# joyecnu/STTODE

Hardware: AMD Instinct MI355X
Metric: predicted-trajectories/sec (20-sample best-of-K) (higher is better)
Workload: dtype f32

## Files before the change

include/sttode_hip.h:

```cpp
#ifndef STTODE_HIP_H
#define STTODE_HIP_H
#ifdef __cplusplus
extern "C" {
#endif

#define STTODE_ABI_VERSION 14
int sttode_abi_version(void);
const char* sttode_last_error(void);

int sttode_rotate_scene(float* past, float* fut, int n, int Tp, int Tf, float c, float s, void* stream);

int sttode_frontend_scenes(const float* past, const int* scene_ptr, int n, int S, int Tp, int TPX, int vel_from_norm,
                           float* scene_orig, int* agent_scene, float* xpad, float* enc_in, float* cur, float* orig,
                           int* last_flag, void* stream);

int sttode_frontend_nba(const float* past, int n, int N, int Tp, int TPX, float* xpad, float* enc_in, float* cur, float* orig,
                        int* last_flag, void* stream);

int sttode_frontend_future(const float* future, const float* past_last, int n, int Tf, int mode, int nba_N,
                           const float* scene_orig, const int* agent_scene, const int* scene_ptr, float* enc_in, void* stream);

int sttode_embed_qkv(const float* fc1P, const float* fc1b, const float* posP, const float* peb, const float* fc2P,
                     const float* fc2b, const float* fc3P, const float* fc3b, const float* fc3last, const float* inP,
                     const float* inb, const float* enc_in, const int* last_flag, float* g, float* qkv, int n, int Tlen,
// ... 162 lines not shown
} SttodeOdeCombine;
int sttode_ode_combine(const void* jobs, int count, int width, void* stream);
typedef struct SttodeOdeProgram {
    int stages;
    int steps;
    float h;
    float a[16];
    float b[4];
} SttodeOdeProgram;
int sttode_ttrunk_ode_fwd(const void* const* ptrs, int count, int trunks, const int* n, const int* T, const long* ld_feat, float* const* ys,
                          float* const* yT, const void* prog, void* stream);
typedef struct SttodeOdeStageBwd {
    const float* w[16];
    const float* y;
    SttodeOdeCombine kb;
    float* dy;
    SttodeOdeCombine next;
    float* attn;
    float* ao;
    float* h;
    float* f1;
    float* dsum2;
    float* df1;
    float* du;
    float* dv;
    float* dao;
    float* dattn;
    float* ln;
    int n;
} SttodeOdeStageBwd;
int sttode_ode_stage_bwd(const void* jobs, int count, void* stream);

int sttode_loss_objective(const float* pred, const float* rec, const float* fut, const float* past, const float* qzp,
                          const int* scene_ptr, const int* agent_scene, int S, int n, int K1, int D, int Dp, int zd, float scale_mse,
                          float scale_rec, float kl_denom, float min_clip, float* out, float* dpred, float* drec, float* dqzp,
                          float* scratch, long scratch_floats, void* stream);
int sttode_loss_objective_live(const float* pred, const float* rec, const float* fut, const float* past, const float* qzp,
                               const int* scene_ptr, const int* agent_scene, int S, int n, int K1, int D, int Dp, int zd, float scale_mse,
                               float scale_rec, float kl_denom, float min_clip, float* out, float* dpred2, float* drec2, float* dqzp,
                               int* best, float* scratch, long scratch_floats, void* stream);
int sttode_live_rows_gather(const void* items, int count, const int* best, int n, int K1, void* stream);
int sttode_publish_values(const float* vals, int n, float* host_vals, unsigned* dev_seq, unsigned* host_seq, void* stream);
int sttode_wait_value(const unsigned* host_seq, long want, double timeout_s);

int sttode_pmath_rowop(int op, const float* x, const float* y, float* out, float* out2, int rows, int d, float c, void* stream);
int sttode_pmath_scalar(int which, const float* x, float* out, long n, void* stream);
int sttode_pmath_riemannian_grad(const float* x, const float* g, float* out, int rows, int d, float c, void* stream);
int sttode_pmath_matvec(const float* m, const float* x, float* mx_ws, float* xnorm_ws, float* out, int rows, int d, int O, float c,
                        void* stream);
int sttode_pmath_pair(int which, const float* x, const float* y, const float* A, float* out, int P, int R, int d, float c,
                      void* stream);
int sttode_pmath_mean(const float* x, float* yl_ws, float* lam_ws, float* out, int rows, int d, float c, void* stream);
int sttode_pmath_rowop_bwd(int op, const float* x, const float* y, const float* g, float* gx, float* gy, int rows, int d, float c, void* stream);
int sttode_pmath_matvec_bwd(const float* m, const float* x, const float* g, float* mx_ws, float* gmx_ws, float* gxn_ws, float* gx, float* gm,
                            int rows, int d, int O, float c, void* stream);
int sttode_pmath_dist_matrix_bwd(const float* x, const float* y, const float* g, float* gx, float* gy, int P, int R, int d, float c,
                                 void* stream);
int sttode_pmath_hsoftmax_bwd(const float* X, const float* A, const float* P, const float* g, double* coef_ws, float* gX, float* gA, float* gP,
                              int B, int C, int d, float c, void* stream);
int sttode_pmath_clip(const float* x, float* out, int rows, int d, float r, void* stream);
int sttode_pmath_clip_bwd(const float* x, const float* g, float* gx, int rows, int d, float r, void* stream);
int sttode_oblique_dist(const float* p1, const float* p2, float* out, int nb, int n1, int n2, int d, void* stream);

int sttode_delta_dist(const float* X, int rows, int d, const int* idx, int T, int n, float* dist, long dist_floats, float* diam, void* stream);
int sttode_delta_workspace(int T, int n, long* floats);
int sttode_delta_hyp(const float* dist, int T, int n, long dist_floats, int symmetric, float* ws, long ws_floats, float* delta, void* stream);

int sttode_reduce_samples(const float* pred, int n, int R, int K_in, int Tf, int K, int iters, int from_frame, int init_mode,
                          const float* init, float* centroids, int* labels, int* counts, void* stream);

typedef struct SttodeModel SttodeModel;

enum SttodeWeight {
    STT_W_FC1P, STT_W_FC1B, STT_W_POSP, STT_W_PEB, STT_W_FC2P, STT_W_FC2B, STT_W_FC3P, STT_W_FC3B, STT_W_FC3LAST, STT_W_INP,
    STT_W_INB, STT_W_OUTP, STT_W_OUTB, STT_W_INFOP, STT_W_INFOB, STT_W_GATEP, STT_W_GATEB, STT_W_LN1W, STT_W_LN1B, STT_W_L1P,
    STT_W_L1B, STT_W_L2P, STT_W_L2B, STT_W_LN2W, STT_W_LN2B,
    STT_W_B0_CONVP, STT_W_B0_CONVB, STT_W_B0_WIHP, STT_W_B0_WHHP, STT_W_B0_GBIAS, STT_W_B0_XWA, STT_W_B0_XB1, STT_W_B0_YWA,
    STT_W_B0_YB1, STT_W_B0_STREAM,
    STT_W_B1_CONVP, STT_W_B1_CONVB, STT_W_B1_WIHP, STT_W_B1_WHHP, STT_W_B1_GBIAS, STT_W_B1_YWA, STT_W_B1_YB1, STT_W_B1_STREAM,
    STT_W_CHAIN_POOL, STT_W_CHAIN_PROG, STT_W_CHAIN_CONSTS, STT_W_G0_POOL, STT_W_G0_PROG, STT_W_G0_CONSTS,
    STT_W_CHAINB3_POOL, STT_W_CHAINB3_PROG,
    STT_W_ROLE32_POOL, STT_W_ROLE32_PROG_SCENES, STT_W_ROLE32_PROG_NBA, STT_W_ROLE32_CONSTS_SCENES,
    STT_W_ROLE32_CONSTS_NBA,
    STT_W_COUNT
};

enum SttodeBuffer {
    STT_B_SCENE_ORIG, STT_B_AGENT_SCENE, STT_B_XPAD, STT_B_ENC_IN, STT_B_CUR, STT_B_ORIG, STT_B_LAST, STT_B_G, STT_B_QKV,
    STT_B_ATTN, STT_B_PF, STT_B_STATE0, STT_B_A0X, STT_B_A0Y, STT_B_A1Y, STT_B_DBUF, STT_B_YBUF, STT_B_STATE1, STT_B_QUEUE, STT_B_FLAGS ,
    STT_B_ODE , STT_B_COUNT
};

enum SttodeStage {
    STT_STAGE_FRONTEND, STT_STAGE_EMBED, STT_STAGE_ATTN, STT_STAGE_POST, STT_STAGE_GRU0, STT_STAGE_LINEAR, STT_STAGE_MLP0,
    STT_STAGE_GRU1, STT_STAGE_MLP1, STT_STAGE_CHAIN, STT_STAGE_AGENTS ,
    STT_STAGE_FUSED , STT_STAGE_COUNT
};

int sttode_model_create(SttodeModel** out, const void* const* weights, int count, int Tp, int Tf, int K, int n_chunks0,
                        int n_chunks1);
int sttode_model_set_weight(SttodeModel* m, int index, const void* ptr);
int sttode_model_destroy(SttodeModel* m);
int sttode_workspace_layout(const SttodeModel* m, int n, int S, long* offsets , long* total_floats);
int sttode_workspace_init(SttodeModel* m, float* workspace, int n, int S, void* stream);
int sttode_set_chain(SttodeModel* m, int mode);
int sttode_set_fused(SttodeModel* m, int mode);
int sttode_set_mfma_mode(SttodeModel* m, int mode);
int sttode_debug_drop_role_flag(SttodeModel* m, int tile);
int sttode_stage_scene(const float* pre, const float* fut, int N, int Tp, int Tf, float* dev, void* stream);
int sttode_stage_rows(const float* a, long na, const float* b, long nb, float* dev, void* stream);
int sttode_async_next_stream(SttodeModel* m, int n, void** stream);
int sttode_async_best_of_k(SttodeModel* m, int slot, const float* pred, const float* gt, int n, int K, int Tf, float scale, float* ade,
                           float* fde);
int sttode_set_scene_launch(SttodeModel* m, int max_tiles);
int sttode_fused_block_of(long block, long tiles, long groups, long K, long lead);
int sttode_set_ode(SttodeModel* m, int method, int steps);
int sttode_timing_enable(SttodeModel* m, int every);
int sttode_timing_read(SttodeModel* m, double* total_ms , int* launches ,
                       double* busy_ms );

int sttode_inference_scenes(SttodeModel* m, const float* past, const int* scene_ptr, int n, int S, const float* z,
                            float* workspace, float* pred, void* stream);
int sttode_inference_nba(SttodeModel* m, const float* past, int B, int N, const float* z, float* workspace, float* pred,
                         void* stream);
int sttode_inference_nba_groups(SttodeModel* m, const float* past, int G, int B, int N, const float* z, float* workspace, float* pred,
                                void* stream);

int sttode_set_lagged(SttodeModel* m, int streams );
typedef struct SttodeSamplerPlan {
    const float* pool;
    const int* prog;
    int prog_len;
    const float* biases;
    int K;
    int nz;
    int h1;
    int h2;
    int eps_mode;
    const float* eps;
} SttodeSamplerPlan;
typedef struct SttodeAsyncOpts {
    int device_latents;
    unsigned long long zkey;
    const float* metrics_gt;
    float* ade;
    float* fde;
    float metrics_scale;
    int nba_groups;
    const SttodeSamplerPlan* sampler;
} SttodeAsyncOpts;
int sttode_sampler_qnet(const SttodeSamplerPlan* plan, const float* pf, int n, float* z, void* stream);
int sttode_clock_probe(long long* out, void* stream);
int sttode_copy_to_host(void* dst, const void* src, long bytes, int wgs, void* stream);
int sttode_async_enqueue(SttodeModel* m, int slot);
int sttode_async_flush(SttodeModel* m);
int sttode_inference_scenes_async(SttodeModel* m, const float* past, const int* scene_ptr, int n, int S, const float* z,
                                  float* workspace, float* pred, int slot, const SttodeAsyncOpts* opts, void* stream);
int sttode_inference_nba_async(SttodeModel* m, const float* past, int B, int N, const float* z, float* workspace, float* pred,
                               int slot, const SttodeAsyncOpts* opts, void* stream);
int sttode_async_horizon_metrics(SttodeModel* m, int slot, const float* pred, const float* gt, int n, int K, int Tf, float scale, float* out);
int sttode_async_best_of_k_select(SttodeModel* m, int slot, const float* pred, const float* gt, int n, int K, int Tf, float scale,
                                  float miss_threshold, const int* seg_ptr, int S, float* ade, float* fde, int* best_ade_idx, int* best_fde_idx,
                                  unsigned char* miss, float* best, float* seg_ade, float* seg_fde, int* seg_miss);
int sttode_async_joint_select(SttodeModel* m, int slot, const float* pred, const float* gt, int n, int K, int Tf, float scale,
                              const int* seg_ptr, int S, float radius, float* seg_jade, float* seg_jfde, int* seg_jade_idx, int* seg_jfde_idx,
                              int* seg_col, int* seg_gt_col);
int sttode_async_kde_nll(SttodeModel* m, int slot, const float* pred, const float* gt, int n, int K, int Tf, float scale, double* nll);
int sttode_async_sample_spread(SttodeModel* m, int slot, const float* pred, const float* gt, int n, int K, int Tf, float scale,
                               double div_scale, double* apd, double* fpd, double* pade, double* dlow, double* es_ade, double* es_fde,
                               float* ade_at_k, float* fde_at_k);
int sttode_wait(SttodeModel* m, int slot, void* stream);
int sttode_async_is_lagged(SttodeModel* m, int n);
int sttode_wait_host(SttodeModel* m, int slot);
int sttode_timeout_word(SttodeModel* m, const unsigned** word);
int sttode_timeout_clear(SttodeModel* m);
int sttode_check(SttodeModel* m, const float* workspace, int n, int S, void* stream);

#ifdef __cplusplus
}
#endif
#endif
```

sttode_amd/capi.py:

```python
import ctypes
import os

_LIB = None
LIB_PATH = os.environ.get('STTODE_HIP_LIB') or os.path.join(os.path.dirname(os.path.abspath(__file__)), 'lib', 'libsttode_hip.so')

_P, _I, _L, _F, _D = ctypes.c_void_p, ctypes.c_int, ctypes.c_long, ctypes.c_float, ctypes.c_double
ABI_VERSION = 14

SIGNATURES = {
    'sttode_abi_version': [],
    'sttode_rotate_scene': [_P, _P, _I, _I, _I, _F, _F, _P],
    'sttode_frontend_scenes': [_P, _P, _I, _I, _I, _I, _I, _P, _P, _P, _P, _P, _P, _P, _P],
    'sttode_frontend_nba': [_P, _I, _I, _I, _I, _P, _P, _P, _P, _P, _P],
    'sttode_frontend_future': [_P, _P, _I, _I, _I, _I, _P, _P, _P, _P, _P],
    'sttode_embed_qkv': [_P] * 11 + [_P, _P, _P, _P, _I, _I, _P],
    'sttode_mhgsa_attn': [_P, _P, _P, _P, _P, _P, _I, _I, _I] + [_L] * 8 + [_F, _F, _P],
    'sttode_mhgsa_attn_groups': [_P, _P, _P, _P, _I, _L, _L, _L, _L, _I, _I, _I] + [_L] * 8 + [_F, _F, _I, _P],
    'sttode_post_attn': [_P] * 14 + [_P, _P, _I, _P, _I, _F, _P],
    'sttode_post_attn_ode': [_P] * 16 + [_P, _P, _I, _F, _I, _I, _P],
    'sttode_post_attn_rhs': [_P] * 14 + [_P, _P, _I, _P, _I, _P],
    'sttode_ode_state_to_pf': [_P, _P, _P, _I, _P],
    'sttode_gru_cols': [_P, _P, _P, _P, _P, _P, _P, _I, _I, _I, _P],
    'sttode_set_latency_tiles': [_I, _I, _I],
    'sttode_linear_cols': [_P, _I, _I, _P, _I, _I, _P, _P, _P, _I, _I, _I, _I, _P],
    'sttode_agent_preact': [_P] * 11 + [_I, _P],
    'sttode_mlp_block0': [_P, _P, _P, _I, _P, _P, _P, _P, _I, _I, _I, _I, _P],
    'sttode_mlp_block1': [_P, _P, _I, _P, _P, _P, _P, _P, _P, _I, _I, _I, _I, _P],
    'sttode_mlp_cols': [_P, _P, _I, _P, _P, _P, _I, _I, _I, _P],
    'sttode_traj_chain': [_P, _P, _P, _P, _P, _I, _P, _P, _P, _I, _P, _P, _P, _P, _I, _I, _I, _I, _I, _P],
    'sttode_chain_prog_len': [_I, _I],
    'sttode_gru_cols32': [_P, _I, _P, _P, _I, _P, _P, _I, _I, _P],
    'sttode_best_of_k': [_P, _P, _I, _I, _I, _F, _P, _P, _P],
    'sttode_horizon_metrics': [_P, _P, _I, _I, _I, _F, _P, _P],
    'sttode_best_of_k_select': [_P, _P, _I, _I, _I, _F, _F, _P, _I] + [_P] * 10,
    'sttode_joint_select': [_P, _P, _I, _I, _I, _F, _P, _I, _F] + [_P] * 7,
    'sttode_kde_nll': [_P, _P, _I, _I, _I, _F, _P, _P],
    'sttode_sample_spread': [_P, _P, _I, _I, _I, _F, _D] + [_P] * 9,
    'sttode_sampler_latent': [_P, _P, _P, _I, _P, _P, _I, _I, _I, _P],
    'sttode_sampler_loss': [_P, _P, _P, _P, _P, _I, _I, _I, _I, _F, _P, _P, _P],
    'sttode_sampler_loss_bwd': [_P, _P, _P, _P, _P, _P, _P, _I, _I, _I, _I, _F, _P, _P, _P, _P],
    'sttode_sampler_qnet': [_P, _P, _I, _P, _P],
    'sttode_tlinear': [_P, _L, _I, _P, _L, _I, _P, _P, _L, _P, _L, _I, _I, _I, _I, _I, _P],
    'sttode_tlinear_tab': [_P, _L, _P, _L, _P, _P, _L, _I, _P, _L, _I, _I, _I, _I, _P],
    'sttode_twgrad': [_P, _L, _P, _L, _I, _P, _L, _P, _I, _I, _I, _P, _L, _P],
    'sttode_twgrad_defer': [_I, _P, _L],
    'sttode_twgrad_flush': [],
    'sttode_tgemm_group': [_I],
    'sttode_tlinear_bwd': [_P, _L, _P, _L, _P, _L, _P, _L, _I, _I, _P, _L, _I, _P, _L, _P, _I, _I, _I, _P, _L, _P],
    'sttode_decoder_inputs': [_P, _P, _L, _P, _L, _P, _P, _I, _I, _I, _I, _P],
    'sttode_rows_copy': [_P, _L, _P, _L, _I, _I, _I, _I, _P],
    'sttode_rows_reduce': [_P, _L, _P, _L, _I, _I, _I, _I, _P],
    'sttode_train_ewise': [_I, _P, _P, _P, _P, _P, _L, _I, _F, _P],
    'sttode_add_ln_fwd': [_P, _P, _P, _P, _P, _P, _P, _I, _I, _P],
    'sttode_ln_bwd': [_P, _P, _P, _P, _P, _P, _P, _I, _I, _P, _L, _P],
    'sttode_gru_cell_fwd': [_P, _L, _P, _P, _P, _P, _I, _P],
    'sttode_gru_cell_bwd': [_P, _P, _P, _P, _L, _P, _P, _I, _P],
    'sttode_gru_seq_fwd': [_P, _P, _P, _P, _P, _P, _L, _I, _I, _P],
    'sttode_gru_seq_bwd': [_P, _L, _P, _P, _P, _P, _P, _I, _I, _P],
    'sttode_conv_fwd': [_P, _I, _P, _P, _P, _P, _P, _I, _I, _P],
    'sttode_conv_bwd': [_P, _P, _P, _P, _P, _P, _I, _I, _P, _L, _P],
    'sttode_mhgsa_attn_bwd': [_P, _P, _P, _I, _I, _I, _P],
    'sttode_mhgsa_attn_rc_bwd': [_P] * 7 + [_I, _I, _I] + [_L] * 8 + [_F, _F, _P],
    'sttode_adam_step': [_P, _I, _L, _P, _D, _D, _D, _D, _D, _L, _P],
    'sttode_grad_norm': [_P, _I, _P, _L, _D, _I, _P, _P],
    'sttode_adam_step_guarded': [_P, _I, _L, _P, _D, _D, _D, _D, _P, _I, _P],
    'sttode_grad_scale': [_P, _I, _L, _P, _P, _P],
    'sttode_loss_sqerr': [_P, _P, _L, _F, _P, _P, _P],
    'sttode_loss_kl': [_P, _P, _I, _I, _I, _F, _F, _P, _P, _P, _P],
    'sttode_loss_diverse': [_P, _P, _P, _P, _I, _I, _I, _P, _P, _P, _P],
    'sttode_ttrunk_fwd': [_P, _I, _I, _I, _L, _F, _I, _P],
    'sttode_ode_combine': [_P, _I, _I, _P],
    'sttode_ttrunk_ode_fwd': [_P, _I, _I, _P, _P, _P, _P, _P, _P, _P],
    'sttode_ode_stage_bwd': [_P, _I, _P],
    'sttode_loss_objective': [_P, _P, _P, _P, _P, _P, _P, _I, _I, _I, _I, _I, _I, _F, _F, _F, _F, _P, _P, _P, _P, _P, _L, _P],
    'sttode_pmath_rowop': [_I, _P, _P, _P, _P, _I, _I, _F, _P],
    'sttode_pmath_scalar': [_I, _P, _P, _L, _P],
    'sttode_pmath_riemannian_grad': [_P, _P, _P, _I, _I, _F, _P],
    'sttode_pmath_matvec': [_P, _P, _P, _P, _P, _I, _I, _I, _F, _P],
    'sttode_pmath_pair': [_I, _P, _P, _P, _P, _I, _I, _I, _F, _P],
    'sttode_pmath_mean': [_P, _P, _P, _P, _I, _I, _F, _P],
    'sttode_oblique_dist': [_P, _P, _P, _I, _I, _I, _I, _P],
    'sttode_pmath_rowop_bwd': [_I, _P, _P, _P, _P, _P, _I, _I, _F, _P],
    'sttode_pmath_matvec_bwd': [_P, _P, _P, _P, _P, _P, _P, _P, _I, _I, _I, _F, _P],
    'sttode_pmath_dist_matrix_bwd': [_P, _P, _P, _P, _P, _I, _I, _I, _F, _P],
    'sttode_pmath_hsoftmax_bwd': [_P, _P, _P, _P, _P, _P, _P, _P, _I, _I, _I, _F, _P],
    'sttode_pmath_clip': [_P, _P, _I, _I, _F, _P],
    'sttode_pmath_clip_bwd': [_P, _P, _P, _I, _I, _F, _P],
    'sttode_delta_dist': [_P, _I, _I, _P, _I, _I, _P, _L, _P, _P],
    'sttode_delta_workspace': [_I, _I, ctypes.POINTER(ctypes.c_long)],
    'sttode_delta_hyp': [_P, _I, _I, _L, _I, _P, _L, _P, _P],
    'sttode_reduce_samples': [_P, _I, _I, _I, _I, _I, _I, _I, _I, _P, _P, _P, _P, _P],
    'sttode_attn_core': [_P, _P, _P, _P, _L, _P, _P, _P, _P, _I, _I, _I] + [_L] * 8 + [_F, _F, _I, _P],
    'sttode_attn_core_bwd': [_P, _P, _P, _P, _L, _P, _P, _P, _P, _I, _I, _I] + [_L] * 8 + [_F, _F, _I, _P],
    'sttode_model_create': [ctypes.POINTER(ctypes.c_void_p), ctypes.POINTER(ctypes.c_void_p), _I, _I, _I, _I, _I, _I],
    'sttode_model_destroy': [_P],
    'sttode_model_set_weight': [_P, _I, _P],
    'sttode_workspace_layout': [_P, _I, _I, ctypes.POINTER(ctypes.c_long), ctypes.POINTER(ctypes.c_long)],
    'sttode_workspace_init': [_P, _P, _I, _I, _P],
    'sttode_timeout_word': [_P, ctypes.POINTER(ctypes.c_void_p)],
    'sttode_timeout_clear': [_P],
    'sttode_set_chain': [_P, _I],
    'sttode_set_fused': [_P, _I],
    'sttode_set_mfma_mode': [_P, _I],
    'sttode_debug_drop_role_flag': [_P, _I],
    'sttode_set_scene_launch': [_P, _I],
    'sttode_stage_scene': [_P, _P, _I, _I, _I, _P, _P],
    'sttode_stage_rows': [_P, _L, _P, _L, _P, _P],
    'sttode_loss_objective_live': [_P, _P, _P, _P, _P, _P, _P, _I, _I, _I, _I, _I, _I, _F, _F, _F, _F, _P, _P, _P, _P, _P, _P, _L, _P],
    'sttode_live_rows_gather': [_P, _I, _P, _I, _I, _P],
    'sttode_publish_values': [_P, _I, _P, _P, _P, _P],
    'sttode_wait_value': [_P, _L, _D],
    'sttode_async_next_stream': [_P, _I, _P],
    'sttode_async_best_of_k': [_P, _I, _P, _P, _I, _I, _I, _F, _P, _P],
    'sttode_fused_block_of': [_L, _L, _L, _L, _L],
    'sttode_set_ode': [_P, _I, _I],
    'sttode_timing_enable': [_P, _I],
    'sttode_timing_read': [_P, ctypes.POINTER(ctypes.c_double), ctypes.POINTER(ctypes.c_int), ctypes.POINTER(ctypes.c_double)],
    'sttode_inference_scenes': [_P, _P, _P, _I, _I, _P, _P, _P, _P],
    'sttode_inference_nba': [_P, _P, _I, _I, _P, _P, _P, _P],
    'sttode_inference_nba_groups': [_P, _P, _I, _I, _I, _P, _P, _P, _P],
    'sttode_inference_scenes_async': [_P, _P, _P, _I, _I, _P, _P, _P, _I, _P, _P],
    'sttode_inference_nba_async': [_P, _P, _I, _I, _P, _P, _P, _I, _P, _P],
    'sttode_async_horizon_metrics': [_P, _I, _P, _P, _I, _I, _I, _F, _P],
    'sttode_async_best_of_k_select': [_P, _I, _P, _P, _I, _I, _I, _F, _F, _P, _I] + [_P] * 9,
    'sttode_async_joint_select': [_P, _I, _P, _P, _I, _I, _I, _F, _P, _I, _F] + [_P] * 6,
    'sttode_async_kde_nll': [_P, _I, _P, _P, _I, _I, _I, _F, _P],
    'sttode_async_sample_spread': [_P, _I, _P, _P, _I, _I, _I, _F, _D] + [_P] * 8,
    'sttode_wait': [_P, _I, _P],
    'sttode_async_is_lagged': [_P, _I],
    'sttode_wait_host': [_P, _I],
    'sttode_set_lagged': [_P, _I],
    'sttode_async_flush': [_P],
    'sttode_clock_probe': [_P, _P],
    'sttode_copy_to_host': [_P, _P, _L, _I, _P],
    'sttode_async_enqueue': [_P, _I],
    'sttode_check': [_P, _P, _I, _I, _P],
}

WEIGHT_ORDER = ([('past', k) for k in ('fc1P', 'fc1b', 'posP', 'peb', 'fc2P', 'fc2b', 'fc3P', 'fc3b', 'fc3last', 'inP', 'inb', 'outP',
                                       'outb', 'infoP', 'infob', 'gateP', 'gateb', 'ln1w', 'ln1b', 'l1P', 'l1b', 'l2P', 'l2b', 'ln2w',
                                       'ln2b')]
                + [('blk0', k) for k in ('convP', 'convB', 'wihP', 'whhP', 'gbias', 'x_WA', 'x_b1', 'y_WA', 'y_b1', 'stream')]
                + [('blk1', k) for k in ('convP', 'convB', 'wihP', 'whhP', 'gbias', 'y_WA', 'y_b1', 'stream')]
                + [('chain', k) for k in ('pool', 'prog', 'consts')] + [('gru0s', k) for k in ('pool', 'prog', 'consts')]
                + [('chain_b3', k) for k in ('pool', 'prog')]
                + [('role32', k) for k in ('pool', 'prog_scenes', 'prog_nba', 'consts_scenes', 'consts_nba')])
TRUNK_PTRS = ('fc1_w', 'fc1_b', 'pos_w', 'pos_b', 'fc2_w', 'fc2_b', 'fc3_w', 'fc3_b', 'inproj_w', 'inproj_b', 'out_w', 'out_b', 'info_w', 'info_b',
              'gate_w', 'gate_b', 'ln1_w', 'ln1_b', 'l1_w', 'l1_b', 'l2_w', 'l2_b', 'ln2_w', 'ln2_b', 'enc_in', 'last', 'pe', 'drop', 'posin', 'tp',
              'h3in', 'feat', 'xc', 'qkv', 'ao', 'tt', 'ss', 'h', 'xh1', 'rs1', 'f1', 'xh2', 'rs2', 'ode', 'attn')
BUFFERS = ('scene_orig', 'agent_scene', 'xpad', 'enc_in', 'cur', 'orig', 'last', 'g', 'qkv', 'attn', 'pf', 'state0', 'A0x', 'A0y',
           'A1y', 'dbuf', 'ybuf', 'state1', 'queue', 'flags', 'ode')
STAGES = ('frontend', 'embed_qkv', 'mhgsa_attn', 'post_attn', 'gru_cols[block0,agents]', 'agent_preact', 'mlp_block0',
          'gru_cols[block1,trajectories]', 'mlp_block1', 'trajectory_chain', 'agents_fused[encoder+block0 GRU]', 'agents+trajectory_chain[fused launch]')


class AsyncOpts(ctypes.Structure):
    _fields_ = [('device_latents', ctypes.c_int), ('zkey', ctypes.c_ulonglong), ('metrics_gt', ctypes.c_void_p), ('ade', ctypes.c_void_p),
                ('fde', ctypes.c_void_p), ('metrics_scale', ctypes.c_float), ('nba_groups', ctypes.c_int), ('sampler', ctypes.c_void_p)]


class GradGroup(ctypes.Structure):
    _fields_ = [('items', ctypes.c_void_p), ('n', ctypes.c_int), ('chunks', ctypes.c_long), ('gbase', ctypes.c_void_p),
                ('lr', ctypes.c_double), ('beta1', ctypes.c_double), ('beta2', ctypes.c_double), ('step', ctypes.c_long)]


GRAD_MAX_GROUPS = 16
GRAD_STATE_WORDS = 40


class SamplerPlan(ctypes.Structure):
    _fields_ = [('pool', ctypes.c_void_p), ('prog', ctypes.c_void_p), ('prog_len', ctypes.c_int), ('biases', ctypes.c_void_p),
                ('K', ctypes.c_int), ('nz', ctypes.c_int), ('h1', ctypes.c_int), ('h2', ctypes.c_int), ('eps_mode', ctypes.c_int),
                ('eps', ctypes.c_void_p)]


class NativeModel:

    def __init__(self, packed, Tp, Tf, K):
        self.packed = packed
        tbl = (ctypes.c_void_p * len(WEIGHT_ORDER))(*[(packed[g][k].data_ptr() if g in packed else None) for g, k in WEIGHT_ORDER])
        h = ctypes.c_void_p()
        rc = lib().sttode_model_create(ctypes.byref(h), tbl, len(WEIGHT_ORDER), Tp, Tf, K, int(packed['blk0']['n_chunks']),
                                       int(packed['blk1']['n_chunks']))
        if rc != 0:
            raise SttodeError('sttode_model_create failed: ' + lib().sttode_last_error().decode())
        self.h = h
        self._layouts = {}
        w = ctypes.c_void_p()
        if lib().sttode_timeout_word(h, ctypes.byref(w)) != 0 or not w.value:
            raise SttodeError('sttode_timeout_word failed: ' + lib().sttode_last_error().decode())
        self.timeout_word = ctypes.c_uint.from_address(w.value)

    def raise_if_timed_out(self):
        v = self.timeout_word.value
        if v:
            lib().sttode_timeout_clear(self.h)
            raise SttodeError('a trajectory group of an earlier launch gave up waiting for its per-agent role (time-out word %d): the '
                              'predictions of that call are NaN-poisoned, not valid' % v if v != 2 else
                              'an earlier launch ran on a workspace that was never initialised (sttode_workspace_init): its predictions are NaN')

    def init_workspace(self, buf, n, S):
        call('sttode_workspace_init', self.h, buf, int(n), int(S), stream_ptr())

    def layout(self, n, S):
        key = (n, S)
        if key not in self._layouts:
            off = (ctypes.c_long * len(BUFFERS))()
            tot = ctypes.c_long()
            rc = lib().sttode_workspace_layout(self.h, n, S, off, ctypes.byref(tot))
            if rc != 0:
                raise SttodeError('sttode_workspace_layout failed: ' + lib().sttode_last_error().decode())
            self._layouts[key] = (dict(zip(BUFFERS, list(off))), int(tot.value))
        return self._layouts[key]

    def set_chain(self, mode):
        if lib().sttode_set_chain(self.h, int(mode)) != 0:
            raise SttodeError('sttode_set_chain failed: ' + lib().sttode_last_error().decode())

    def set_scene_launch(self, max_tiles):
        call('sttode_set_scene_launch', self.h, int(max_tiles))

    def set_fused(self, mode):
        if lib().sttode_set_fused(self.h, int(mode)) != 0:
            raise SttodeError('sttode_set_fused failed: ' + lib().sttode_last_error().decode())

    def set_lagged(self, streams):
        call('sttode_set_lagged', self.h, int(streams))
        self._lagged = int(streams)

    def check(self, workspace, n, S):
        call('sttode_check', self.h, workspace, int(n), int(S), stream_ptr())

    def set_weights(self, group, tensors):
        self.packed[group] = tensors
        for i, (g, k) in enumerate(WEIGHT_ORDER):
            if g == group:
                call('sttode_model_set_weight', self.h, i, tensors[k])

    def set_mfma_mode(self, mode):
        if lib().sttode_set_mfma_mode(self.h, int(mode)) != 0:
            raise SttodeError('sttode_set_mfma_mode failed: ' + lib().sttode_last_error().decode())

    def set_ode(self, method, steps):
        if lib().sttode_set_ode(self.h, int(method), int(steps)) != 0:
            raise SttodeError('sttode_set_ode failed: ' + lib().sttode_last_error().decode())

    def timing(self, every):
        lib().sttode_timing_enable(self.h, int(every))

    def read_timing(self):
        ms = (ctypes.c_double * len(STAGES))()
        cnt = (ctypes.c_int * len(STAGES))()
        busy = (ctypes.c_double * len(STAGES))()
        rc = lib().sttode_timing_read(self.h, ms, cnt, busy)
        if rc != 0:
            raise SttodeError('sttode_timing_read failed: ' + lib().sttode_last_error().decode())
        self.busy_ms = {STAGES[i]: busy[i] for i in range(len(STAGES)) if cnt[i]}
        return {STAGES[i]: (ms[i], cnt[i]) for i in range(len(STAGES)) if cnt[i]}

    def __del__(self):
        try:
            if self.h:
                lib().sttode_model_destroy(self.h)
                self.h = None
        except Exception:
            pass



class SttodeError(RuntimeError):
    pass


def lib():
    global _LIB
    if _LIB is None:
        if not os.path.exists(LIB_PATH):
            raise SttodeError(f'{LIB_PATH} not found: build it with `python -c "import __graft_entry__ as g; g.build()"` '
                              f'or `make -C sttode_amd/csrc`. There is no CPU fallback.')
        L = ctypes.CDLL(LIB_PATH)
        L.sttode_last_error.restype = ctypes.c_char_p
        L.sttode_last_error.argtypes = []
        try:
            got = int(L.sttode_abi_version())
        except AttributeError:
            got = None
        if got != ABI_VERSION:
            raise SttodeError(f'{LIB_PATH}: ABI version {got}, this binding needs {ABI_VERSION}; rebuild with `make -C sttode_amd/csrc`')
# ... 40 lines not shown
```

sttode_amd/csrc/api_util.hpp:

```cpp
#pragma once
#include <hip/hip_runtime.h>
#include <cstdio>

void stt_set_error(const char* msg);
int stt_gru_cols_form(const float* xin, const float* convP, const float* convB, const float* wihP, const float* whhP, const float* gbias,
                      float* state, int ncols, int Tp, int TPX, int lat_max_tiles, void* stream);
int stt_agents_fused(const float* const* W, const float* enc_in, const int* last, float* g, float* qkv, float* pf, const float* xpad,
                     float* state0, int n, int Tp, int TPX, float ode_time, void* stream);
bool stt_agents_fused_covers(int Tp, int TPX);
int stt_chain_fused(const float* const* W, float* ws, const long* off, int n, int K, int Tp, int Tf, int prog_len, const float* z, float* pred,
                    float ode_time, const float* attn, int ld_attn, const float* past, const int* scene_ptr, int S, int wgs_per_cu, int b3, int lead, int drop_tile,
                    unsigned* tmo_host, void* stream);
bool stt_chain_fused_covers(int Tp);
int stt_scene_lat(const float* const* W, float* ws, const long* off, int n, int K, int Tp, int Tf, int TPX, int NOY, int n_chunks0, int n_chunks1,
                  const float* z, float* pred, float ode_time, const float* past, const int* scene_ptr, int S, int drop_tile, unsigned* tmo_host,
                  void* stream);
static inline int stt_scene_flags_offset(int n) { return 5 * ((n + 15) / 16) + 4; }
int stt_scene_flags_init(float* ws, const long* off, int n, int K, void* stream);
bool stt_scene_lat_covers(int Tp, int TPX, int NOY);
int stt_traj_chain_b3(const float* A0x, const float* A0y, const float* A1y, const float* pool, const int* prog, int prog_len,
                      const float* consts, const float* z, const float* xpad, int ldx, const float* cur, const float* orig,
                      float* pred, int* counter, int ncols, int K, int Tp, int Tf, int wgs_per_cu, void* stream);
int stt_gru_lat_tiles();
int stt_enc_lat_tiles();

#define STT_REQUIRE(cond, msg)      \
    do {                            \
        if (!(cond)) {              \
            stt_set_error(msg);     \
            return 1;               \
        }                           \
    } while (0)

#define STT_HIP(expr)                                                                       \
    do {                                                                                    \
        hipError_t _e = (expr);                                                             \
        if (_e != hipSuccess) {                                                             \
            char _b[512];                                                                   \
            snprintf(_b, sizeof(_b), "%s failed: %s (%s:%d)", #expr, hipGetErrorString(_e), __FILE__, __LINE__); \
            stt_set_error(_b);                                                              \
            return 2;                                                                       \
        }                                                                                   \
    } while (0)

#define STT_ATTR_DEVICES 64
#define STT_SET_LDS_ONCE(kernel, bytes)                                                                         \
    do {                                                                                                        \
        static bool _done[STT_ATTR_DEVICES] = {};                                                               \
        int _dev = 0;                                                                                           \
        STT_HIP(hipGetDevice(&_dev));                                                                           \
        if (_dev < 0 || _dev >= STT_ATTR_DEVICES || !_done[_dev]) {                                             \
            STT_HIP(hipFuncSetAttribute((const void*)(kernel), hipFuncAttributeMaxDynamicSharedMemorySize, (bytes))); \
            if (_dev >= 0 && _dev < STT_ATTR_DEVICES) _done[_dev] = true;                                       \
        }                                                                                                       \
    } while (0)

struct LagRoles {
    float* ws; const long* off; int n;
    const float* attn; int ld_attn; float ode_time;
    float* zgen; unsigned long long zkey;
    const float* past; const int* scene_ptr; int S;
    float* ade; float* fde;
};
struct LagGroups {
    float* ws; const long* off; int n; const float* z; float* pred;
    const float* gt; float* ade; float* fde; float scale;
    int workers;
};
int stt_chain_lagged(const float* const* W, const LagRoles& r, const LagGroups& g, int K, int Tp, int Tf, int prog_len, int b3, void* stream);
bool stt_chain_lagged_covers(int Tp);
struct SttodeSamplerPlan;
const char* stt_sampler_plan_check(const SttodeSamplerPlan* plan, int K);
int stt_sampler_qnet(const SttodeSamplerPlan* plan, const float* pf, int n, float* z, void* stream);
int stt_joint_check(const char* who, const float* pred, const float* gt, int n, int K, int Tf, const int* seg_ptr, int S, float radius,
                    const float* seg_jade, const float* seg_jfde, const int* seg_jade_idx, const int* seg_jfde_idx, const int* seg_col,
                    const int* seg_gt_col);
int stt_kde_check(const char* who, const float* pred, const float* gt, int n, int K, int Tf, const double* nll);
int stt_spread_check(const char* who, const float* pred, const float* gt, int n, int K, int Tf, double div_scale, const double* apd,
                     const double* fpd, const double* pade, const double* dlow, const double* es_ade, const double* es_fde,
                     const float* ade_at_k, const float* fde_at_k);
```

sttode_amd/csrc/chain32.hip:

```cpp
#include "chain.hpp"
#include "latency_bodies.hpp"
#include "frontend_body.hpp"
#include "api_util.hpp"
#include "../../include/sttode_hip.h"
#include <cstdlib>
#include <cstddef>

#ifdef C32_DIAG_TRACE
__shared__ long long g_tr_ph[4];
#define C32_TRACE_BEGIN() long long _tr_t0 = 0, _tr_c0 = 0; if (threadIdx.x == 0 && A.dbg) { _tr_t0 = __builtin_amdgcn_s_memrealtime(); _tr_c0 = __builtin_amdgcn_s_memtime(); }
#define C32_TRACE_END(kind) do { if (threadIdx.x == 0 && A.dbg) { \
        const long long _t1 = __builtin_amdgcn_s_memrealtime(); unsigned _hw, _xcc; \
        asm volatile("s_getreg_b32 %0, hwreg(HW_REG_HW_ID)" : "=s"(_hw)); asm volatile("s_getreg_b32 %0, hwreg(HW_REG_XCC_ID)" : "=s"(_xcc)); \
        const unsigned long long _r = atomicAdd((unsigned long long*)A.dbg, 1ull); if ((long long)_r >= A.dbg[1]) break;  \
        long long* _p = A.dbg + 8 + _r * 12; _p[0] = A.trace_tag; _p[1] = blockIdx.x; _p[2] = (kind); _p[3] = _tr_t0; _p[4] = _t1; _p[5] = _hw; _p[6] = _xcc; \
        _p[8] = g_tr_ph[0]; _p[9] = g_tr_ph[1]; _p[10] = g_tr_ph[2]; _p[7] = __builtin_amdgcn_s_memtime() - _tr_c0; _p[11] = g_tr_ph[3]; } } while (0)
#define C32_TRACE_PHASE(i) do { if (threadIdx.x == 0) g_tr_ph[i] = __builtin_amdgcn_s_memrealtime(); } while (0)
#else
#define C32_TRACE_PHASE(i) do { } while (0)
#define C32_TRACE_BEGIN() do { } while (0)
#define C32_TRACE_END(kind) do { } while (0)
#endif

#include "role_body.hpp"

typedef float f32x16 __attribute__((ext_vector_type(16)));

#ifdef C32_DIAG_NOGATES
#define C32_SIG(x) ((x) * 1e-3f)
#define C32_TANH(x) ((x) * 1e-3f)
#else
#define C32_SIG(x) sigmoid_prescaled(x)
#define C32_TANH(x) tanh_prescaled(x)
#endif

#define C32_TILE 256
#define C32_CMAX 3
#define C32_RING (2 * C32_CMAX * C32_TILE)
#define C32_SLOT 256

struct Role32Args {
    const f32x4* pool; const int2* prog; int prog_len; const float* consts;
    const float* enc_in; const int* last;
    const float* g_in; const float* attn; int ld_attn;
    const float* xpad; int ldx;
    float* pf; float* state0; float* A0x; float* A0y; float* A1y;
    int n, Tp, kte, nwg;
    float ode_time;
    int prio;
    int* counter;
    float* zgen; unsigned zkey0, zkey1; int K;
    const float* past; const int* scene_ptr; int S; float* scene_orig; int* agent_scene;
    float* enc_in_w; float* xpad_w; float* cur_w; float* orig_w; int* last_w;
    float* m_ade; float* m_fde;
};

struct ChainArgs {
    const float* A0x; const float* A0y; const float* A1y;
    const f32x4* pool;
    const int2* prog; int prog_len;
    const float* consts;
    const float* z;
    const float* xpad; int ldx;
    const float* cur; const float* orig;
    float* pred;
    float* park;
    int* counter;
    int ncols, K, Tp, Tf2;
    int persistent;
    const float* m_gt; float* m_ade; float* m_fde; float m_scale;
    int nworkers;
    long long* dbg;
    int trace_tag;
    int xcd_map;
    RoleArgs R;
    Role32Args R32;
};

template <int NY> struct C32Const {
    static constexpr int b2x = 0, b3x = 256, b2y = 288, b3y = 544, gb = 544 + 32 * NY, cb = gb + 384, b2m = cb + 32,
                         b3m = b2m + 256, total = b3m + 32 * NY;
};

__device__ __forceinline__ f32x16 splat16(float v) {
    f32x16 r;
#pragma unroll
    for (int e = 0; e < 16; ++e) r[e] = v;
    return r;
}
__device__ __forceinline__ f32x16 relu16(f32x16 v) {
#pragma unroll
    for (int e = 0; e < 16; ++e) v[e] = fmaxf(v[e], 0.f);
    return v;
}
__device__ __forceinline__ f32x16 ldrows(const float* p, int h) {
    f32x16 r;
#pragma unroll
    for (int a = 0; a < 4; ++a) {
        const f32x4 v = ld4(p + 8 * a + 4 * h);
        r[4 * a + 0] = v[0]; r[4 * a + 1] = v[1]; r[4 * a + 2] = v[2]; r[4 * a + 3] = v[3];
    }
    return r;
}

typedef const __attribute__((address_space(4))) int KProg;

template <int BUF, bool GEN, bool DYN = false>
struct ChainStreamT {
    static constexpr int kBuf = BUF;
    static constexpr int kPieces = (BUF / 64 + 3) / 4, kPairs = (kPieces + 1) / 2;
    const char* pool; KProg* prog; f32x4* ring;
    unsigned ring_addr, loff;
    unsigned qoff, qend;
    int par, lane, wave;
    int2 ld_v, ld_w;
    bool fetched;
    int cnt;
    const char* nsrc[kPairs]; unsigned nm0[kPairs]; int ncnt, npc;
#ifdef C32_DIAG_STAMPS
    long long t_bar, gap_cyc, gap_n, gap_cal;
#endif
    __device__ __forceinline__ int2 entry_at(unsigned off) const {
        const KProg* e = reinterpret_cast<const KProg*>(reinterpret_cast<const __attribute__((address_space(4))) char*>(prog) + off);
        return make_int2(e[0], e[1]);
    }
    __device__ __forceinline__ unsigned next_off(unsigned off) const { return off + 8 >= qend ? 0u : off + 8; }
    __device__ __forceinline__ void stage(int2 ev, int buf) {
        ncnt = __builtin_amdgcn_readfirstlane(ev.y);
        npc = GEN ? (ncnt - wave + 3) >> 2 : ncnt;
        const size_t src = (size_t)(unsigned)__builtin_amdgcn_readfirstlane(ev.x) * (GEN ? 16u : C32_TILE * 16u) + (unsigned)wave * 1024u;
        const unsigned dst = __builtin_amdgcn_readfirstlane(ring_addr + (unsigned)buf * (BUF * 16) + (unsigned)wave * 1024u);
#pragma unroll
        for (int k = 0; k < kPairs; ++k) {
            nsrc[k] = pool + (src + 4096u * (2 * k + 1));
            nm0[k] = dst + 4096u * (2 * k + 1);
            asm volatile("" : "+s"(nsrc[k]), "+s"(nm0[k]));
        }
        asm volatile("" : "+s"(npc));
    }
    __device__ __forceinline__ void issue(int N) {
#ifndef C32_DIAG_NODMA
#pragma unroll
        for (int k = 0; k < kPairs; ++k) {
            if (N > 0 ? 2 * k < N : 2 * k < npc) {
                glds16_sv<-4096>(nsrc[k], loff, nm0[k] - 4096u);
                if (2 * k + 1 < kPieces && (N > 0 ? 2 * k + 1 < N : 2 * k + 1 < npc)) glds16_m0<0>(nsrc[k], loff);
            }
        }
#endif
    }
    __device__ __forceinline__ void init(const f32x4* pool_, const int2* prog_, int len_, f32x4* ring_) {
        pool = reinterpret_cast<const char*>(pool_); prog = (KProg*)prog_; ring = ring_;
        ring_addr = __builtin_amdgcn_readfirstlane(lds_addr(ring_));
        lane = threadIdx.x & 63;
        loff = (unsigned)lane * 16;
        wave = __builtin_amdgcn_readfirstlane(threadIdx.x >> 6);
        par = 0;
        qend = (unsigned)len_ * 8u;
        const int2 e0 = entry_at(0);
        stage(e0, 0);
        issue(0);
        cnt = e0.y;
        qoff = next_off(0);
        stage(entry_at(qoff), 1);
        qoff = next_off(qoff);
        fetched = false;
#ifdef C32_DIAG_STAMPS
        gap_cyc = 0; gap_n = 0;
        const long long c0 = __builtin_amdgcn_s_memtime();
        asm volatile("s_waitcnt lgkmcnt(0)" ::: "memory");
        gap_cal = __builtin_amdgcn_s_memtime() - c0;
        t_bar = 0;
#endif
    }
    __device__ __forceinline__ void fetch() { ld_v = entry_at(qoff); qoff = next_off(qoff); fetched = true; }
    __device__ __forceinline__ void fetch_more() { ld_w = entry_at(qoff); qoff = next_off(qoff); }
    __device__ __forceinline__ void take_prefetched() { ld_v = ld_w; fetched = true; }
    __device__ __forceinline__ void stamp_gap() {
#ifdef C32_DIAG_STAMPS
        asm volatile("s_waitcnt lgkmcnt(0)" ::: "memory");
        const long long c1 = __builtin_amdgcn_s_memtime();
        asm volatile("s_waitcnt lgkmcnt(0)" ::: "memory");
        if (t_bar) { gap_cyc += c1 - t_bar; ++gap_n; }
#endif
    }
    __device__ __forceinline__ void begin(int N = 0) {
        __builtin_amdgcn_sched_barrier(0);
#ifdef C32_DIAG_CHECK
        if (!GEN && N > 0 && ncnt != N) __builtin_trap();
#endif
        cnt = ncnt;
        issue(GEN || DYN ? 0 : N);
        stamp_gap();
        __builtin_amdgcn_sched_barrier(0);
    }
    __device__ __forceinline__ const f32x4* cur() const { return ring + par * BUF + lane; }
    __device__ __forceinline__ void end(bool has_entry = false) {
        __builtin_amdgcn_sched_barrier(0);
#ifdef C32_DIAG_CHECK
        if (has_entry && !fetched) __builtin_trap();
#endif
        if (!has_entry && !fetched) fetch();
        stage(ld_v, par);
        __builtin_amdgcn_sched_barrier(0);
#ifndef C32_DIAG_NOBARRIER
        asm volatile("s_waitcnt vmcnt(0)" ::: "memory");
        __syncthreads();
#endif
#ifdef C32_DIAG_STAMPS
        t_bar = __builtin_amdgcn_s_memtime();
        asm volatile("s_waitcnt lgkmcnt(0)" ::: "memory");
#endif
        par ^= 1;
        fetched = false;
        __builtin_amdgcn_sched_barrier(0);
    }
};
typedef ChainStreamT<C32_CMAX * C32_TILE, false> ChainStream;

__device__ __forceinline__ void tile_mma(f32x16& acc, const f32x4* __restrict__ t, const f32x16& B) {
#pragma unroll
    for (int g = 0; g < 4; ++g) {
        const f32x4 a = t[g * 64];
#pragma unroll
        for (int r = 0; r < 4; ++r) acc = __builtin_amdgcn_mfma_f32_32x32x2f32(a[r], B[4 * g + r], acc, 0, 0, 0);
    }
}

__device__ __forceinline__ void gather_rows(const void* base, unsigned voff, unsigned slot_addr) {
// ... 366 lines not shown
    f32x16 e = ldrows(cb, h);
    Frag fa, fb;
    if (ZS) {
        const int k0 = 2 * t - 2, k1 = 2 * t + 3;
        const int g0 = (k0 > 0 ? k0 : 0) >> 3, g1 = (k1 < 2 * Tp - 1 ? k1 : 2 * Tp - 1) >> 3;
        const f32x4* tc = st.cur();
#pragma unroll
        for (int g = 0; g < 4; ++g)
            if (g >= g0 && g <= g1) fa.a[g] = tc[g * 64];
        st.begin(3);
#pragma unroll
        for (int g = 0; g < 4; ++g)
            if (g >= g0 && g <= g1)
#pragma unroll
                for (int r = 0; r < 4; ++r) e = __builtin_amdgcn_mfma_f32_32x32x2f32(fa.a[g][r], d[4 * g + r], e, 0, 0, 0);
        __builtin_amdgcn_sched_barrier(0);
        if (pre) st.take_prefetched();
        else st.fetch();
    } else {
        ldfrag(fa, st.cur());
        st.begin(3);
        tile_mma2f(st, e, fa, d, fb, nullptr, pre ? 0 : 1);
        if (pre) st.take_prefetched();
    }
    e = relu16(e);
    st.end();
    return e;
}

template <bool ZS, class ST>
__device__ __forceinline__ void gru32_steps(ST& st, const float* gb, const float* cb, const f32x16& d, f32x16 (&hs)[3], int Tp, int h) {
    if (ZS) {
        const f32x16 e = gru32_conv<ZS>(st, cb, d, 0, Tp, h, false);
        Frag fa, fb;
#pragma unroll
        for (int j = 0; j < 3; ++j) {
            STT_FENCE();
            f32x16 ar = ldrows(gb + 0 * 96 + 32 * j, h);
            ldfrag(fa, st.cur()); st.begin(3);
            tile_mma2f(st, ar, fa, e, fb, nullptr);
            st.end(); ldfrag(fa, st.cur() + 1 * C32_TILE); st.begin(3);
#pragma unroll
            for (int r = 0; r < 16; ++r) ar[r] = C32_SIG(ar[r]);
            STT_FENCE();
            f32x16 az = ldrows(gb + 1 * 96 + 32 * j, h);
            tile_mma2f(st, az, fa, e, fb, nullptr, 2);
            st.end(); st.begin(3);
            st.take_prefetched();
#pragma unroll
            for (int r = 0; r < 16; ++r) az[r] = C32_SIG(az[r]);
            STT_FENCE();
            f32x16 an = ldrows(gb + 3 * 96 + 32 * j, h);
            {
                const f32x16 bi = ldrows(gb + 2 * 96 + 32 * j, h);
#pragma unroll
                for (int r = 0; r < 16; ++r) an[r] = fmaf(ar[r], an[r], bi[r]);
            }
            st.end(); ldfrag(fa, st.cur() + 2 * C32_TILE);
            if (j < 2) st.begin(3); else st.begin();
            STT_FENCE();
            tile_mma2f(st, an, fa, e, fb, nullptr, (j == 2 && 1 < Tp) ? 2 : 1);
            st.end();
#pragma unroll
            for (int r = 0; r < 16; ++r) {
                const float ng = C32_TANH(an[r]);
                hs[j][r] = fmaf(az[r], 0.f - ng, ng);
            }
        }
    }
#pragma unroll 1
    for (int t = ZS ? 1 : 0; t < Tp; ++t) {
        const f32x16 e = gru32_conv<ZS>(st, cb, d, t, Tp, h, ZS);
        Frag fa, fb;
        f32x16 hn[3];
#pragma unroll
        for (int j = 0; j < 3; ++j) {
            STT_FENCE();
            f32x16 ar = ldrows(gb + 0 * 96 + 32 * j, h);
            ldfrag(fa, st.cur()); st.begin(3);
            tile_mma2f(st, ar, fa, e, fb, st.cur() + 1 * C32_TILE);
            tile_mma2(ar, fb, hs[0], fa, st.cur() + 2 * C32_TILE);
            tile_mma2(ar, fa, hs[1], fb, nullptr);
            st.end(); ldfrag(fa, st.cur()); st.begin(3);
            tile_mma2f(st, ar, fa, hs[2], fb, st.cur() + 1 * C32_TILE);
#pragma unroll
            for (int r = 0; r < 16; ++r) ar[r] = C32_SIG(ar[r]);
            STT_FENCE();
            f32x16 az = ldrows(gb + 1 * 96 + 32 * j, h);
            tile_mma2(az, fb, e, fa, st.cur() + 2 * C32_TILE);
            tile_mma2(az, fa, hs[0], fb, nullptr);
            st.end(); ldfrag(fa, st.cur()); st.begin(3);
            tile_mma2f(st, az, fa, hs[1], fb, st.cur() + 1 * C32_TILE);
            tile_mma2(az, fb, hs[2], fa, st.cur() + 2 * C32_TILE);
#pragma unroll
            for (int r = 0; r < 16; ++r) az[r] = C32_SIG(az[r]);
            STT_FENCE();
            f32x16 an = ldrows(gb + 3 * 96 + 32 * j, h);
            tile_mma2(an, fa, hs[0], fb, nullptr);
            st.end(); ldfrag(fa, st.cur());
            if (j < 2) st.begin(3); else st.begin();
            tile_mma2f(st, an, fa, hs[1], fb, st.cur() + 1 * C32_TILE, (ZS && j == 2 && t + 1 < Tp) ? 2 : 1);
            tile_mma2(an, fb, hs[2], fa, st.cur() + 2 * C32_TILE);
            {
                const f32x16 bi = ldrows(gb + 2 * 96 + 32 * j, h);
#pragma unroll
                for (int r = 0; r < 16; ++r) an[r] = fmaf(ar[r], an[r], bi[r]);
            }
            STT_FENCE();
            tile_mma2(an, fa, e, fb, nullptr);
            st.end();
#pragma unroll
            for (int r = 0; r < 16; ++r) {
                const float ng = C32_TANH(an[r]);
                hn[j][r] = fmaf(az[r], hs[j][r] - ng, ng);
            }
        }
#pragma unroll
        for (int j = 0; j < 3; ++j) hs[j] = hn[j];
    }

}

#include "role32.hpp"

__device__ __forceinline__ int opaque(int v) { asm volatile("" : "+v"(v)); return v; }

#ifdef C32_DIAG_STAMPS
#define C32_STAMP(k) do { if (threadIdx.x == 0 && A.dbg && gi < 4) { A.dbg[((size_t)blockIdx.x * 4 + gi) * 16 + 2 * (k)] = __builtin_amdgcn_s_memtime(); \
                                                                    A.dbg[((size_t)blockIdx.x * 4 + gi) * 16 + 2 * (k) + 1] = __builtin_amdgcn_s_memrealtime(); } } while (0)
#else
#define C32_STAMP(k) do { } while (0)
#endif

__host__ __device__ __forceinline__ int fused_block_of(long b, long T, long G, long K, long lead) {
    auto roles_upto = [&](long x) { const long c = (8 * (x + lead + 1) + K - 1) / K; return c < T ? c : T; };
    long lo = -1, hi = G - 1;
    while (lo < hi) {
        const long mid = (lo + hi + 1) >> 1;
        if (mid + roles_upto(mid) <= b) lo = mid; else hi = mid - 1;
    }
    if (lo >= 0 && lo + roles_upto(lo) == b) return (int)lo;
    return -1 - (int)(b - (lo + 1));
}

__host__ __device__ __forceinline__ int xcd_group(int b, int G) {
    const int x = b & 7, i = b >> 3, q = G >> 3, r = G & 7;
    return x * q + (x < r ? x : r) + i;
}

template <int NY, int FUSE, bool B3M, bool ZS>
__global__ __launch_bounds__(256, 2) void traj_chain_kernel(ChainArgs A) {
    constexpr bool kDynCount = !B3M && ((NY == 1 && FUSE == 2 && !ZS) || (NY == 2 && FUSE == 1 && ZS));
    typedef ChainStreamT<B3M ? C32_BUF_B3 : C32_CMAX * C32_TILE, B3M, kDynCount> Stream;
    extern __shared__ __attribute__((aligned(16))) char smem[];
    f32x4* ring = reinterpret_cast<f32x4*>(smem);
    f32x4* slots = ring + 2 * Stream::kBuf;
    f32x4* zslots = slots + 4 * C32_SLOT;
    float* cst = reinterpret_cast<float*>(zslots + 4 * C32_SLOT);
    int* sq = reinterpret_cast<int*>(cst + C32Const<NY>::total);
    typedef C32Const<NY> CO;

    const int lane = threadIdx.x & 63, c = lane & 31, h = lane >> 5;
    const int wave = __builtin_amdgcn_readfirstlane(threadIdx.x >> 6);
    const f32x4* slot = slots + wave * C32_SLOT;
    const f32x4* zslot = zslots + wave * C32_SLOT;
    const unsigned slot_addr = __builtin_amdgcn_readfirstlane(lds_addr(slot));
    const unsigned zslot_addr = __builtin_amdgcn_readfirstlane(lds_addr(zslot));
    const int ngroups = (A.ncols + 127) >> 7;

    C32_TRACE_BEGIN();
    if (FUSE == 2 && (int)blockIdx.x < A.R32.nwg) {
        role32_body<ZS>(*(KRole32Args*)((const __attribute__((address_space(4))) char*)__builtin_amdgcn_kernarg_segment_ptr() + offsetof(ChainArgs, R32)),
                    blockIdx.x, smem);
        C32_TRACE_END(1);
        return;
    }
    if (FUSE == 1 && A.R.split && (int)blockIdx.x < 5 * A.R.ntiles) {
        split_role(A.R, (A.ncols + A.K - 1) / A.K, A.Tp, A.ldx, A.xpad, blockIdx.x, smem);
        C32_TRACE_END(1);
        return;
    }
    int fb = FUSE == 0 ? (int)blockIdx.x : FUSE == 2 ? (int)blockIdx.x - A.R32.nwg : A.R.split ? (int)blockIdx.x - 5 * A.R.ntiles
                                                : fused_block_of(blockIdx.x, A.R.ntiles, ngroups, A.K, A.R.lead);
    if (FUSE && A.xcd_map && fb >= 0) fb = xcd_group(fb, ngroups);
    if (FUSE == 1 && fb < 0) {
        agent_role(A.R, (A.ncols + A.K - 1) / A.K, A.Tp, A.ldx, A.xpad, -1 - fb, smem);
        C32_TRACE_END(1);
        return;
    }
    for (int i = threadIdx.x; i < CO::total; i += blockDim.x) cst[i] = A.consts[i];
    if (threadIdx.x == 0) sq[0] = FUSE == 2 ? fb : (FUSE == 0 && A.persistent) ? atomicAdd(A.counter, 1) : FUSE ? fb : (int)blockIdx.x;
    if (FUSE == 1) {
        const int g0 = fb;
        const int c_lo = g0 * 128, c_hi = (c_lo + 127 < A.ncols ? c_lo + 127 : A.ncols - 1);
        const int t_lo = (c_lo / A.K) >> 4, t_hi = (c_hi / A.K) >> 4;
        if (wave == 0) {
            const bool ok = A.R.split ? wait_tiles(A.R.pflags, 3 * t_lo, 3 * t_hi + 2, A.R.flags + A.R.ntiles, lane, A.R.tmo_host)
                                      : wait_tiles(A.R.flags, t_lo, t_hi, A.R.flags + A.R.ntiles, lane, A.R.tmo_host);
            if (!ok && lane == 0) sq[0] = -1;
        }
    }
    __syncthreads();
    C32_TRACE_PHASE(3);
    int g = sq[0];
    if (FUSE == 1 && g < 0) {
        for (int i = threadIdx.x; i < 128 * A.Tf2; i += blockDim.x) {
            const size_t o = (size_t)fb * 128 * A.Tf2 + i;
            if (o < (size_t)A.ncols * A.Tf2) A.pred[o] = __builtin_nanf("");
        }
        return;
    }
    if (g >= ngroups) return;
    Stream st;
    st.init(A.pool, A.prog, A.prog_len, ring);

    auto col_of = [&](int gg) { int col = gg * 128 + wave * 32 + c; return col < A.ncols ? col : A.ncols - 1; };
    {
        const int c0 = col_of(g);
        gather_rows(A.A0x, row_off(c0 / A.K, 512, h), slot_addr);
        gather_rows(A.z, row_off(c0, 32, h), zslot_addr);
    }
    asm volatile("s_waitcnt vmcnt(0)" ::: "memory");
    __syncthreads();

    int gi = 0;
    (void)gi;
    while (true) {
        C32_STAMP(0);
        const int col = g * 128 + wave * 32 + c;
        int colc = col < A.ncols ? col : A.ncols - 1;
        int agent = colc / A.K;
        const bool live = col < A.ncols;
        __syncthreads();
        if (threadIdx.x == 0)
            sq[1] = (FUSE == 2 && A.persistent && ngroups > A.nworkers) ? A.nworkers + atomicAdd(A.counter, 1)
                    : (FUSE == 0 && A.persistent) ? atomicAdd(A.counter, 1) : ngroups;

        f32x16 acc2[8];
        f32x16 d;
        {
            agent = opaque(agent);
            f32x16 xo[1];
            const unsigned ao = row_off(agent, 512, h);
            if (B3M) {
                mlp_l12_b3<0, true>(st, slot, zslot, nullptr, A.A0x, ao, A.A0y, ao, acc2, lane);
                mlp_l3_b3<1>(st, acc2, cst + CO::b2x, cst + CO::b3x, xo, h);
            } else {
                mlp_l12<0>(st, slot, zslot, nullptr, A.A0x, ao, A.A0y, ao, acc2, lane);
                mlp_l3<1, 3>(st, acc2, cst + CO::b2x, cst + CO::b3x, xo, h);
            }
            agent = opaque(agent);
            const float* xp = A.xpad + (size_t)agent * A.ldx;
#pragma unroll
            for (int a = 0; a < 4; ++a) {
                f32x4 v = splat4(0.f);
                if (8 * a + 4 * h < A.ldx) v = ld4(xp + 8 * a + 4 * h);
#pragma unroll
                for (int b = 0; b < 4; ++b) d[4 * a + b] = v[b] - xo[0][4 * a + b];
            }
        }
        STT_FENCE();
        C32_STAMP(1);
        {
            agent = opaque(agent);
            f32x16 yo[NY];
            const unsigned ao = row_off(agent, 512, h);
            if (B3M) {
                mlp_l12_b3<0, true>(st, slot, zslot, nullptr, A.A0y, ao, A.A1y, ao, acc2, lane);
                mlp_l3_b3<NY>(st, acc2, cst + CO::b2y, cst + CO::b3y, yo, h);
            } else {
                mlp_l12<0>(st, slot, zslot, nullptr, A.A0y, ao, A.A1y, ao, acc2, lane);
                mlp_l3<NY, 1>(st, acc2, cst + CO::b2y, cst + CO::b3y, yo, h);
            }
            if (live) {
                float* prow = A.park + (size_t)opaque(col) * A.Tf2;
#pragma unroll
                for (int o = 0; o < NY; ++o)
#pragma unroll
                    for (int a = 0; a < 4; ++a) {
                        const int row0 = 32 * o + 8 * a + 4 * h;
                        float* p = prow + row0;
                        if (row0 + 3 < A.Tf2 && (A.Tf2 & 3) == 0) {
                            f32x4 v = {yo[o][4 * a], yo[o][4 * a + 1], yo[o][4 * a + 2], yo[o][4 * a + 3]};
                            st4(p, v);
                        } else {
#pragma unroll
                            for (int b = 0; b < 4; ++b)
                                if (row0 + b < A.Tf2) p[b] = yo[o][4 * a + b];
                        }
                    }
            }
        }
        STT_FENCE();
        C32_STAMP(2);
        f32x16 hs[3];
        {
#pragma unroll
            for (int j = 0; j < 3; ++j) hs[j] = splat16(0.f);
            if (B3M) gru32_steps_b3(st, cst + CO::gb, cst + CO::cb, d, hs, A.Tp, h);
            else gru32_steps<ZS>(st, cst + CO::gb, cst + CO::cb, d, hs, A.Tp, h);
        }
        STT_FENCE();
        C32_STAMP(3);
        const int gnext = sq[1];
        {
            agent = opaque(agent);
            const int cnx = col_of(gnext < ngroups ? gnext : g);
            const unsigned ao = row_off(agent, 512, h), an = row_off(cnx / A.K, 512, h);
            if (B3M) mlp_l12_b3<3, false>(st, slot, zslot, hs, A.A1y, ao, A.A0x, an, acc2, lane);
            else mlp_l12<3>(st, slot, zslot, hs, A.A1y, ao, A.A0x, an, acc2, lane);
            gather_rows(A.z, row_off(opaque(cnx), 32, h), zslot_addr);
            f32x16 yo[NY];
            if (B3M) mlp_l3_b3<NY>(st, acc2, cst + CO::b2m, cst + CO::b3m, yo, h);
            else mlp_l3<NY, 3>(st, acc2, cst + CO::b2m, cst + CO::b3m, yo, h);
            {
                agent = opaque(agent);
                const float cx = A.cur[2 * agent], cy = A.cur[2 * agent + 1];
                const float ox = A.orig[2 * agent], oy = A.orig[2 * agent + 1];
                const bool vec = (A.Tf2 & 3) == 0;
                const float* yrow = A.park + (size_t)opaque(colc) * A.Tf2;
                float* prow = A.pred + (size_t)opaque(col) * A.Tf2;
                const float* grow = FUSE == 2 && A.m_gt ? A.m_gt + (size_t)agent * A.Tf2 : nullptr;
                float dd[NY][4][2];
#pragma unroll
                for (int o = 0; o < NY; ++o)
#pragma unroll
                    for (int a = 0; a < 4; ++a) {
                        const int row0 = 32 * o + 8 * a + 4 * h;
                        const bool whole = vec && row0 + 3 < A.Tf2;
                        f32x4 y0 = splat4(0.f);
                        if (whole) y0 = ld4(yrow + row0);
                        else {
#pragma unroll
                            for (int b = 0; b < 4; ++b)
                                if (row0 + b < A.Tf2) y0[b] = yrow[row0 + b];
                        }
                        f32x4 v;
                        v[0] = ((y0[0] + yo[o][4 * a + 0]) + cx) + ox;
                        v[1] = ((y0[1] + yo[o][4 * a + 1]) + cy) + oy;
                        v[2] = ((y0[2] + yo[o][4 * a + 2]) + cx) + ox;
                        v[3] = ((y0[3] + yo[o][4 * a + 3]) + cy) + oy;
                        if (live) {
                            if (whole) st4(prow + row0, v);
                            else {
#pragma unroll
                                for (int b = 0; b < 4; ++b)
                                    if (row0 + b < A.Tf2) prow[row0 + b] = v[b];
                            }
                        }
                        dd[o][a][0] = dd[o][a][1] = 0.f;
                        if (FUSE == 2 && grow) {
                            if (row0 < A.Tf2) { const float2 g = *reinterpret_cast<const float2*>(grow + row0); dd[o][a][0] = bok_dist(v[0], v[1], g.x, g.y, A.m_scale); }
                            if (row0 + 2 < A.Tf2) { const float2 g = *reinterpret_cast<const float2*>(grow + row0 + 2); dd[o][a][1] = bok_dist(v[2], v[3], g.x, g.y, A.m_scale); }
                        }
                    }
                if (FUSE == 2 && grow) {
                    const int Tf = A.Tf2 >> 1;
                    float acc = 0.f, fdl = -1.f;
#pragma unroll
                    for (int o = 0; o < NY; ++o)
#pragma unroll
                        for (int a = 0; a < 4; ++a) {
                            const int t0 = (32 * o + 8 * a + 4 * h) >> 1;
                            float mine = acc;
                            if (h == 0) { if (t0 < Tf) mine += dd[o][a][0]; if (t0 + 1 < Tf) mine += dd[o][a][1]; }
                            float mine1 = __shfl(mine, c, 64);
                            if (h == 1) { if (t0 < Tf) mine1 += dd[o][a][0]; if (t0 + 1 < Tf) mine1 += dd[o][a][1]; }
                            acc = __shfl(mine1, c + 32, 64);
                            if (t0 == Tf - 1) fdl = dd[o][a][0];
                            if (t0 + 1 == Tf - 1) fdl = dd[o][a][1];
                        }
                    fdl = fmaxf(fdl, __shfl_xor(fdl, 32, 64));
                    const float adev = acc / (float)Tf;
                    if (live && h == 0) {
                        atomicMin(reinterpret_cast<unsigned*>(A.m_ade) + agent, __float_as_uint(adev));
                        atomicMin(reinterpret_cast<unsigned*>(A.m_fde) + agent, __float_as_uint(fdl));
                    }
                }
            }
        }
        C32_STAMP(4);
#ifdef C32_DIAG_STAMPS
        if (threadIdx.x == 0 && A.dbg && gi < 4) {
            long long* o = A.dbg + ((size_t)blockIdx.x * 4 + gi) * 16 + 10;
            o[0] = st.gap_cyc; o[1] = st.gap_n; o[2] = st.gap_cal;
        }
        st.gap_cyc = 0; st.gap_n = 0;
#endif
        ++gi;
        g = gnext;
        if (g >= ngroups) break;
    }
    C32_TRACE_END(0);
}

struct Gru32Args {
    const float* xin; int ldx;
    const f32x4* pool; const int2* prog; int prog_len;
    const float* consts;
    float* state;
    int ncols, Tp;
};
template <bool ZS>
__global__ __launch_bounds__(256, 2) void gru32_kernel(Gru32Args A) {
    extern __shared__ __attribute__((aligned(16))) char smem[];
    f32x4* ring = reinterpret_cast<f32x4*>(smem);
    float* cst = reinterpret_cast<float*>(ring + C32_RING);
    const int lane = threadIdx.x & 63, c = lane & 31, h = lane >> 5;
    const int wave = __builtin_amdgcn_readfirstlane(threadIdx.x >> 6);
    for (int i = threadIdx.x; i < 416; i += blockDim.x) cst[i] = A.consts[i];
    __syncthreads();
    ChainStream st;
    st.init(A.pool, A.prog, A.prog_len, ring);
    const int col = blockIdx.x * 128 + wave * 32 + c;
    const int colc = col < A.ncols ? col : A.ncols - 1;
    f32x16 d;
    {
        const float* xp = A.xin + (size_t)colc * A.ldx;
#pragma unroll
        for (int a = 0; a < 4; ++a) {
            f32x4 v = splat4(0.f);
            if (8 * a + 4 * h < A.ldx) v = ld4(xp + 8 * a + 4 * h);
#pragma unroll
            for (int b = 0; b < 4; ++b) d[4 * a + b] = v[b];
        }
    }
    asm volatile("s_waitcnt vmcnt(0)" ::: "memory");
    __syncthreads();
    f32x16 hs[3];
#pragma unroll
    for (int j = 0; j < 3; ++j) hs[j] = splat16(0.f);
    gru32_steps<ZS>(st, cst, cst + 384, d, hs, A.Tp, h);
    if (col < A.ncols) {
#pragma unroll
        for (int j = 0; j < 3; ++j)
#pragma unroll
            for (int a = 0; a < 4; ++a) {
                const f32x4 v = {hs[j][4 * a], hs[j][4 * a + 1], hs[j][4 * a + 2], hs[j][4 * a + 3]};
                st4(A.state + (size_t)col * 96 + 32 * j + 8 * a + 4 * h, v);
            }
    }
}

static int chain_cus() {
    static int n = 0;
    if (!n) {
        int dev = 0;
        hipDeviceProp_t p;
        if (hipGetDevice(&dev) == hipSuccess && hipGetDeviceProperties(&p, dev) == hipSuccess) n = p.multiProcessorCount;
        if (n <= 0) n = 256;
    }
    return n;
}
static int gru_zero_skip() {
    static const int v = getenv("STTODE_GRU_ZERO_SKIP") ? atoi(getenv("STTODE_GRU_ZERO_SKIP")) != 0 : 1;
    return v;
}
static int chain_lds(int NY, bool b3 = false) { return ((b3 ? 2 * C32_BUF_B3 : C32_RING) + 8 * C32_SLOT) * 16 + (1216 + 64 * NY) * 4 + 16; }

static int role_lds(int Tp) {
    const int e = (Tp * 256 + 512) * 16, g = (2 * 6 * 64 + 2 * 24 * 64 + 2 * 4 * 64) * 16;
    return e > g ? e : g;
}

static int role32_lds() { return C32_RING * 16 + R32C::total * 4; }

template <int NY, int FUSE, bool B3M = false> static int chain_launch(ChainArgs a, int wgs_per_cu, hipStream_t s) {
    void (*kern)(ChainArgs) = gru_zero_skip() ? traj_chain_kernel<NY, FUSE, B3M, true> : traj_chain_kernel<NY, FUSE, B3M, false>;
    STT_SET_LDS_ONCE(kern, 96 * 1024);
    const int ngroups = (a.ncols + 127) / 128;
    int grid = ngroups;
    if (FUSE == 1) grid = (a.R.split ? 5 : 1) * a.R.ntiles + ngroups;
    else if (FUSE == 2) {
        int workers = ngroups;
        if (a.persistent && workers > 2 * chain_cus()) workers = 2 * chain_cus();
        grid = a.R32.nwg + (a.ncols > 0 ? workers : 0);
        a.nworkers = workers;
        if (workers < ngroups) a.xcd_map = 0;
    }
    int lds = chain_lds(NY, B3M);
    if (FUSE == 1 && lds < role_lds(a.Tp)) lds = role_lds(a.Tp);
    if (FUSE == 2 && a.R32.nwg > 0 && lds < role32_lds()) lds = role32_lds();
    if (wgs_per_cu == 1 && lds < 84 * 1024) lds = 84 * 1024;
    STT_REQUIRE(lds <= 96 * 1024, "sttode_traj_chain: dynamic LDS beyond the 96 KiB the kernel is registered for");
    STT_REQUIRE((long)a.ncols * 128 <= 0xffffffffL && (long)((a.ncols + a.K - 1) / a.K) * 2048 <= 0xffffffffL,
                "sttode_traj_chain: z / per-agent table rows beyond the 32-bit byte offsets of the gathers");
    if (FUSE == 1) STT_HIP(hipMemsetAsync(a.R.flags, 0, (((size_t)(a.R.split ? 5 : 1) * a.R.ntiles + 1) * 4 + 15) / 16 * 16, s));
    hipLaunchKernelGGL(kern, dim3(grid), dim3(256), lds, s, a);
    STT_HIP(hipGetLastError());
    return 0;
}

extern "C" int sttode_gru_cols32(const float* xin, int ldx, const float* pool, const int* prog, int prog_len, const float* consts,
                                 float* state, int ncols, int Tp, void* stream) {
    STT_REQUIRE(xin && pool && prog && consts && state, "sttode_gru_cols32: null pointer");
    STT_REQUIRE(ncols > 0 && Tp >= 1 && (ldx == 16 || ldx == 32) && 2 * Tp <= ldx, "sttode_gru_cols32: bad ncols/Tp/ldx");
    STT_REQUIRE(prog_len == 13 * Tp, "sttode_gru_cols32: chunk program must hold 13 entries per step");
    Gru32Args a;
    a.xin = xin; a.ldx = ldx; a.pool = (const f32x4*)pool; a.prog = (const int2*)prog; a.prog_len = prog_len; a.consts = consts;
    a.state = state; a.ncols = ncols; a.Tp = Tp;
    const int lds = C32_RING * 16 + 416 * 4;
    hipLaunchKernelGGL(gru_zero_skip() ? gru32_kernel<true> : gru32_kernel<false>, dim3((ncols + 127) / 128), dim3(256), lds, (hipStream_t)stream, a);
    STT_HIP(hipGetLastError());
    return 0;
}

__global__ __launch_bounds__(256, 2) void sampler_qnet32_kernel(QNet32Args Q) {
    extern __shared__ __attribute__((aligned(16))) char smem[];
    f32x4* ring = reinterpret_cast<f32x4*>(smem);
    const int lane = threadIdx.x & 63, c = lane & 31, h = lane >> 5;
    const int wave = __builtin_amdgcn_readfirstlane(threadIdx.x >> 6);
    ChainStream st;
    st.init(Q.pool, Q.prog, Q.prog_len, ring);
    const int col = blockIdx.x * 128 + wave * 32 + c;
    const bool live = col < Q.n;
    const int colc = live ? col : Q.n - 1;
    f32x16 P[4];
#pragma unroll
    for (int kt = 0; kt < 4; ++kt) P[kt] = ldrows(Q.pf + (size_t)colc * 128 + 32 * kt, h);
    asm volatile("s_waitcnt vmcnt(0)" ::: "memory");
    __syncthreads();
    TileFeed<ChainStream> fd(st);
    fd.open();
    qnet32(fd, Q, P, col, colc, live, h);
    fd.close();
}

static long sampler_tiles(const SttodeSamplerPlan* p) {
    const long h1t = p->h1 / 32, h2t = p->h2 / 32;
    return 8 + h1t * (2 + h2t) + (long)p->K * h2t * (p->eps_mode ? 2 : 1);
}
const char* stt_sampler_plan_check(const SttodeSamplerPlan* p, int K) {
    if (!p || !p->pool || !p->prog || !p->biases) return "sampler plan: null pool / program / biases";
    if (p->nz != 32) return "sampler plan: nz must be 32 (one MFMA tile of rows per sample)";
    if (p->K <= 0 || (K > 0 && p->K != K)) return "sampler plan: K must be positive and equal the model's sample_k";
    if (p->h1 <= 0 || p->h1 % 32 || p->h2 <= 0 || p->h2 % 32 || p->h2 > 256) return "sampler plan: hidden widths must be multiples of 32, h2 <= 256";
    if (p->eps_mode < 0 || p->eps_mode > 2 || (p->eps_mode != 0 && !p->eps)) return "sampler plan: eps_mode 0 (mean) | 1 (shared [nz]) | 2 (per agent [n][nz]); eps required unless 0";
    if (p->prog_len <= 0 || p->prog_len > 4096) return "sampler plan: prog_len must be in [1, 4096]";
    if (3L * p->prog_len < sampler_tiles(p)) return "sampler plan: chunk program too short for the widths (<= 3 tiles per chunk)";
    return nullptr;
}
int stt_sampler_qnet(const SttodeSamplerPlan* p, const float* pf, int n, float* z, void* stream) {
    QNet32Args q;
    q.pool = (const f32x4*)p->pool; q.prog = (const int2*)p->prog; q.prog_len = p->prog_len; q.bias = p->biases;
    q.pf = pf; q.z = z; q.eps = p->eps; q.n = n; q.K = p->K; q.h1t = p->h1 / 32; q.h2t = p->h2 / 32; q.eps_mode = p->eps_mode;
    const int lds = C32_RING * 16;
    hipLaunchKernelGGL(sampler_qnet32_kernel, dim3((n + 127) / 128), dim3(256), lds, (hipStream_t)stream, q);
    STT_HIP(hipGetLastError());
    return 0;
}
extern "C" int sttode_sampler_qnet(const SttodeSamplerPlan* plan, const float* pf, int n, float* z, void* stream) {
    STT_REQUIRE(plan && pf && z, "sttode_sampler_qnet: null pointer");
    STT_REQUIRE(n > 0 && (long)n * plan->K <= 0x7fffffffL / 32, "sttode_sampler_qnet: n must be positive (and n K 32 within int range)");
    if (const char* why = stt_sampler_plan_check(plan, 0)) {
        char b[256];
        snprintf(b, sizeof(b), "sttode_sampler_qnet: %s", why);
        stt_set_error(b);
        return 1;
    }
    return stt_sampler_qnet(plan, pf, n, z, stream);
}

#if defined(C32_DIAG_STAMPS) || defined(C32_DIAG_TRACE)
static long long* g_chain_dbg = nullptr;
static int g_trace_tag = 0;
extern "C" int sttode_chain_debug_buffer(void* p) { g_chain_dbg = (long long*)p; return 0; }
#endif

extern "C" int sttode_fused_block_of(long block, long tiles, long groups, long K, long lead) {
    return fused_block_of(block, tiles, groups, K, lead);
}

extern "C" int sttode_chain_prog_len(int Tp, int Tf) {
    const int NY = (2 * Tf + 31) / 32;
    const int l3y = (8 * NY + 2) / 3;
    return (48 + 3) + (48 + l3y) + 13 * Tp + (64 + l3y);
}

static int traj_chain_impl(const float* A0x, const float* A0y, const float* A1y, const float* pool, const int* prog, int prog_len,
                           const float* consts, const float* z, const float* xpad, int ldx, const float* cur, const float* orig,
                           float* pred, int* counter, int ncols, int K, int Tp, int Tf, int wgs_per_cu, bool b3, void* stream) {
    STT_REQUIRE(A0x && A0y && A1y && pool && prog && consts && z && xpad && cur && orig && pred && counter, "sttode_traj_chain: null pointer");
    STT_REQUIRE(ncols > 0 && K > 0 && Tp >= 1 && 2 * Tp <= 32 && Tf >= 1, "sttode_traj_chain: bad ncols/K/Tp/Tf");
    STT_REQUIRE(ldx == 16 || ldx == 32, "sttode_traj_chain: ldx must be 16 or 32");
    STT_REQUIRE(wgs_per_cu == 1 || wgs_per_cu == 2, "sttode_traj_chain: wgs_per_cu must be 1 or 2");
    STT_REQUIRE(2 * Tp <= ldx, "sttode_traj_chain: xpad rows shorter than 2*Tp");
    STT_REQUIRE(prog_len == sttode_chain_prog_len(Tp, Tf), "sttode_traj_chain: chunk program length does not match (Tp, Tf)");
    ChainArgs a;
    a.A0x = A0x; a.A0y = A0y; a.A1y = A1y; a.pool = (const f32x4*)pool; a.prog = (const int2*)prog; a.prog_len = prog_len;
    a.consts = consts; a.z = z; a.xpad = xpad; a.ldx = ldx; a.cur = cur; a.orig = orig; a.pred = pred; a.park = pred; a.counter = counter;
    a.ncols = ncols; a.K = K; a.Tp = Tp; a.Tf2 = 2 * Tf;
    a.dbg = nullptr; a.trace_tag = 0; a.xcd_map = 0; a.nworkers = 0; a.m_gt = nullptr; a.m_ade = a.m_fde = nullptr; a.m_scale = 1.0f;
    a.R = RoleArgs();
    a.persistent = 0;
#if defined(C32_DIAG_STAMPS) || defined(C32_DIAG_TRACE)
    a.dbg = g_chain_dbg;
    a.trace_tag = g_trace_tag++;
#endif
    const int NY = (2 * Tf + 31) / 32;
    hipStream_t s = (hipStream_t)stream;
    if (b3) {
        switch (NY) {
            case 1: return chain_launch<1, 0, true>(a, wgs_per_cu, s);
            case 2: return chain_launch<2, 0, true>(a, wgs_per_cu, s);
            case 3: return chain_launch<3, 0, true>(a, wgs_per_cu, s);
            default: STT_REQUIRE(false, "sttode_traj_chain: future length beyond the built instantiations (2*Tf <= 96)");
        }
    }
    switch (NY) {
        case 1: return chain_launch<1, 0>(a, wgs_per_cu, s);
        case 2: return chain_launch<2, 0>(a, wgs_per_cu, s);
        case 3: return chain_launch<3, 0>(a, wgs_per_cu, s);
        default: STT_REQUIRE(false, "sttode_traj_chain: future length beyond the built instantiations (2*Tf <= 96)");
    }
    return 0;
}
extern "C" int sttode_traj_chain(const float* A0x, const float* A0y, const float* A1y, const float* pool, const int* prog, int prog_len,
                                 const float* consts, const float* z, const float* xpad, int ldx, const float* cur, const float* orig,
                                 float* pred, int* counter, int ncols, int K, int Tp, int Tf, int wgs_per_cu, void* stream) {
    return traj_chain_impl(A0x, A0y, A1y, pool, prog, prog_len, consts, z, xpad, ldx, cur, orig, pred, counter, ncols, K, Tp, Tf, wgs_per_cu, false, stream);
}
int stt_traj_chain_b3(const float* A0x, const float* A0y, const float* A1y, const float* pool, const int* prog, int prog_len,
                      const float* consts, const float* z, const float* xpad, int ldx, const float* cur, const float* orig,
                      float* pred, int* counter, int ncols, int K, int Tp, int Tf, int wgs_per_cu, void* stream) {
    return traj_chain_impl(A0x, A0y, A1y, pool, prog, prog_len, consts, z, xpad, ldx, cur, orig, pred, counter, ncols, K, Tp, Tf, wgs_per_cu, true, stream);
}

bool stt_chain_fused_covers(int Tp) { return Tp >= 2 && 2 * Tp <= 32 && role_lds(Tp) <= 80 * 1024; }
int stt_chain_fused(const float* const* W, float* ws, const long* off, int n, int K, int Tp, int Tf, int prog_len, const float* z, float* pred,
                    float ode_time, const float* attn, int ld_attn, const float* past, const int* scene_ptr, int S, int wgs_per_cu, int b3,
                    int lead, int drop_tile, unsigned* tmo_host, void* stream) {
    STT_REQUIRE(W && ws && off && z && pred, "stt_chain_fused: null pointer");
    STT_REQUIRE(n > 0 && K > 0 && stt_chain_fused_covers(Tp) && Tf >= 1, "stt_chain_fused: shape outside the fused launch");
    STT_REQUIRE(!attn || (ld_attn >= 64 && ld_attn % 4 == 0), "stt_chain_fused: bad attention leading dimension");
    STT_REQUIRE(prog_len == sttode_chain_prog_len(Tp, Tf), "stt_chain_fused: chunk program length does not match (Tp, Tf)");
    STT_REQUIRE((long)n * K <= 0x7fffffffL, "stt_chain_fused: too many trajectories");
    ChainArgs a;
    a.A0x = ws + off[STT_B_A0X]; a.A0y = ws + off[STT_B_A0Y]; a.A1y = ws + off[STT_B_A1Y];
    a.pool = (const f32x4*)W[b3 ? STT_W_CHAINB3_POOL : STT_W_CHAIN_POOL]; a.prog = (const int2*)W[b3 ? STT_W_CHAINB3_PROG : STT_W_CHAIN_PROG];
    a.prog_len = prog_len;
    a.consts = W[STT_W_CHAIN_CONSTS]; a.z = z; a.xpad = ws + off[STT_B_XPAD]; a.ldx = 2 * Tp <= 16 ? 16 : 32; a.cur = ws + off[STT_B_CUR];
    a.orig = ws + off[STT_B_ORIG]; a.pred = pred; a.park = pred; a.counter = (int*)(ws + off[STT_B_QUEUE]);
    a.ncols = n * K; a.K = K; a.Tp = Tp; a.Tf2 = 2 * Tf; a.persistent = 0; a.dbg = nullptr; a.trace_tag = 0; a.xcd_map = 0; a.nworkers = 0;
    a.m_gt = nullptr; a.m_ade = a.m_fde = nullptr; a.m_scale = 1.0f;
#if defined(C32_DIAG_STAMPS) || defined(C32_DIAG_TRACE)
    a.dbg = g_chain_dbg;
    a.trace_tag = g_trace_tag++;
#endif
    RoleArgs& r = a.R;
    role_args_fill(r, W, ws, off);
    r.attn = attn; r.ld_attn = ld_attn;
    STT_REQUIRE(!past || (scene_ptr && S > 0 && !attn), "stt_chain_fused: the in-role front-end needs scene_ptr, S > 0 and attention length 1");
    r.past = past; r.scene_ptr = scene_ptr; r.S = S;
    r.flags = (unsigned*)(ws + off[STT_B_FLAGS]); r.ntiles = (n + 15) / 16; r.ode_time = ode_time;
    r.tmo_host = tmo_host;
    r.lead = lead < 0 ? (1 << 28) : lead;
    a.xcd_map = lead < 0;
    r.split = lead == -2;
    r.gflags = r.flags + r.ntiles + 1; r.pflags = r.gflags + r.ntiles;
    r.drop_tile = drop_tile;
    const int NY = (2 * Tf + 31) / 32;
    hipStream_t s = (hipStream_t)stream;
    switch (NY) {
        case 1: return b3 ? chain_launch<1, 1, true>(a, wgs_per_cu, s) : chain_launch<1, 1>(a, wgs_per_cu, s);
        case 2: return b3 ? chain_launch<2, 1, true>(a, wgs_per_cu, s) : chain_launch<2, 1>(a, wgs_per_cu, s);
        case 3: return b3 ? chain_launch<3, 1, true>(a, wgs_per_cu, s) : chain_launch<3, 1>(a, wgs_per_cu, s);
        default: STT_REQUIRE(false, "stt_chain_fused: future length beyond the built instantiations (2*Tf <= 96)");
    }
    return 0;
}

bool stt_chain_lagged_covers(int Tp) { return Tp >= 2 && 2 * Tp <= 32; }
int stt_chain_lagged(const float* const* W, const LagRoles& lr, const LagGroups& lg, int K, int Tp, int Tf, int prog_len, int b3, void* stream) {
    float* ws_r = lr.ws; const long* off_r = lr.off; const int n_r = lr.n; const float* attn = lr.attn; const int ld_attn = lr.ld_attn;
    const float ode_time = lr.ode_time; float* zgen = lr.zgen; const unsigned long long zkey = lr.zkey; const float* past = lr.past;
    const int* scene_ptr = lr.scene_ptr; const int S = lr.S; float* r_ade = lr.ade; float* r_fde = lr.fde;
    float* ws_g = lg.ws; const long* off_g = lg.off; const int n_g = lg.n; const float* z = lg.z; float* pred = lg.pred;
    const float* g_gt = lg.gt; float* g_ade = lg.ade; float* g_fde = lg.fde; const float g_scale = lg.scale; const int lag_workers_ok = lg.workers;
    STT_REQUIRE(W && (ws_r || ws_g), "stt_chain_lagged: nothing to launch");
    STT_REQUIRE(K > 0 && stt_chain_lagged_covers(Tp) && Tf >= 1, "stt_chain_lagged: shape outside the lagged launch");
    ChainArgs a;
    a.R = RoleArgs();
    a.R32 = Role32Args();
    a.dbg = nullptr; a.trace_tag = 0; a.xcd_map = 0; a.persistent = 0; a.counter = nullptr; a.nworkers = 0;
    a.K = K; a.Tp = Tp; a.Tf2 = 2 * Tf; a.ldx = 2 * Tp <= 16 ? 16 : 32; a.ncols = 0;
    a.pool = (const f32x4*)W[b3 ? STT_W_CHAINB3_POOL : STT_W_CHAIN_POOL]; a.prog = (const int2*)W[b3 ? STT_W_CHAINB3_PROG : STT_W_CHAIN_PROG];
    a.prog_len = prog_len; a.consts = W[STT_W_CHAIN_CONSTS];
    a.A0x = a.A0y = a.A1y = nullptr; a.z = nullptr; a.xpad = nullptr; a.cur = a.orig = nullptr; a.pred = nullptr; a.park = nullptr;
    a.m_gt = nullptr; a.m_ade = a.m_fde = nullptr; a.m_scale = 1.0f;
    if (ws_g && g_gt) {
        STT_REQUIRE(g_ade && g_fde, "stt_chain_lagged: fused metrics need ade and fde");
        a.m_gt = g_gt; a.m_ade = g_ade; a.m_fde = g_fde; a.m_scale = g_scale;
    }
    if (ws_g) {
        STT_REQUIRE(off_g && z && pred && n_g > 0 && (long)n_g * K <= 0x7fffffffL, "stt_chain_lagged: bad group arguments");
        STT_REQUIRE(prog_len == sttode_chain_prog_len(Tp, Tf), "stt_chain_lagged: chunk program length does not match (Tp, Tf)");
        a.A0x = ws_g + off_g[STT_B_A0X]; a.A0y = ws_g + off_g[STT_B_A0Y]; a.A1y = ws_g + off_g[STT_B_A1Y];
        a.z = z; a.xpad = ws_g + off_g[STT_B_XPAD]; a.cur = ws_g + off_g[STT_B_CUR]; a.orig = ws_g + off_g[STT_B_ORIG]; a.pred = pred;
        a.park = ws_g + off_g[STT_B_YBUF];
        a.ncols = n_g * K;
        a.persistent = lag_workers_ok ? 1 : 0;
        a.counter = (int*)(ws_g + off_g[STT_B_QUEUE]);
        a.xcd_map = 1;
    }
    if (ws_r) {
        STT_REQUIRE(off_r && n_r > 0, "stt_chain_lagged: bad role arguments");
        STT_REQUIRE(!attn || (ld_attn >= 64 && ld_attn % 4 == 0), "stt_chain_lagged: bad attention leading dimension");
        Role32Args& r = a.R32;
        r.pool = (const f32x4*)W[STT_W_ROLE32_POOL];
        r.prog = (const int2*)W[attn ? STT_W_ROLE32_PROG_NBA : STT_W_ROLE32_PROG_SCENES];
        r.consts = W[attn ? STT_W_ROLE32_CONSTS_NBA : STT_W_ROLE32_CONSTS_SCENES];
        r.kte = (4 * Tp + 31) / 32;
        const int e = attn ? 8 : 2 * r.kte + 8;
        r.prog_len = attn ? 13 * Tp + (e + 2) / 3 + (128 + 288 + 2) / 3 : 13 * Tp + (e + 128 + 288 + 2) / 3;
        r.enc_in = ws_r + off_r[STT_B_ENC_IN]; r.last = (const int*)(ws_r + off_r[STT_B_LAST]);
        r.g_in = ws_r + off_r[STT_B_G]; r.attn = attn; r.ld_attn = ld_attn;
        r.xpad = ws_r + off_r[STT_B_XPAD]; r.ldx = a.ldx;
        r.pf = ws_r + off_r[STT_B_PF]; r.state0 = ws_r + off_r[STT_B_STATE0];
        r.A0x = ws_r + off_r[STT_B_A0X]; r.A0y = ws_r + off_r[STT_B_A0Y]; r.A1y = ws_r + off_r[STT_B_A1Y];
        r.n = n_r; r.Tp = Tp; r.nwg = (n_r + 127) / 128; r.ode_time = ode_time;
        r.prio = 3;
        r.counter = (int*)(ws_r + off_r[STT_B_QUEUE]);
        r.zgen = zgen; r.zkey0 = (unsigned)zkey; r.zkey1 = (unsigned)(zkey >> 32); r.K = K;
        STT_REQUIRE(!past || (scene_ptr && S > 0 && !attn), "stt_chain_lagged: the in-role front-end needs scene_ptr, S > 0 and attention length 1");
        r.past = past; r.scene_ptr = scene_ptr; r.S = S;
        r.scene_orig = ws_r + off_r[STT_B_SCENE_ORIG]; r.agent_scene = (int*)(ws_r + off_r[STT_B_AGENT_SCENE]);
        r.enc_in_w = ws_r + off_r[STT_B_ENC_IN]; r.xpad_w = ws_r + off_r[STT_B_XPAD]; r.cur_w = ws_r + off_r[STT_B_CUR];
        r.orig_w = ws_r + off_r[STT_B_ORIG]; r.last_w = (int*)(ws_r + off_r[STT_B_LAST]);
        r.m_ade = r_ade; r.m_fde = r_fde;
    }
#if defined(C32_DIAG_STAMPS) || defined(C32_DIAG_TRACE)
    a.dbg = g_chain_dbg;
    a.trace_tag = g_trace_tag++;
#endif
    const int NY = (2 * Tf + 31) / 32;
    hipStream_t s = (hipStream_t)stream;
    switch (NY) {
        case 1: return b3 ? chain_launch<1, 2, true>(a, 2, s) : chain_launch<1, 2>(a, 2, s);
        case 2: return b3 ? chain_launch<2, 2, true>(a, 2, s) : chain_launch<2, 2>(a, 2, s);
        case 3: return b3 ? chain_launch<3, 2, true>(a, 2, s) : chain_launch<3, 2>(a, 2, s);
        default: STT_REQUIRE(false, "stt_chain_lagged: future length beyond the built instantiations (2*Tf <= 96)");
    }
    return 0;
}
```

sttode_amd/csrc/pipeline.hip:

```cpp
#include "api_util.hpp"
#include "../../include/sttode_hip.h"
#include <vector>
#include <algorithm>
#include <utility>
#include <cstring>
#include <mutex>
#include <cstdlib>

#define STT_MAX_DEVICES 64
#define STT_MAX_SLOTS 8
#define STT_GRU0_LAT_TILES 4096
struct TimRec { int stage; hipEvent_t e0, e1; };

struct LagPending { bool valid; float* ws; long off[STT_B_COUNT]; int n; const float* z; float* pred; hipStream_t s; int si;
                    const float* gt; float* ade; float* fde; float scale;
                    int one_launch; };

struct SttodeModel {
    int Tp, Tf, TPX, NOY, K;
    const float* w[STT_W_COUNT];
    int n_chunks0, n_chunks1;
    hipStream_t side;
    hipEvent_t ev_fork, ev_join;
    int chain_mode;
    int fused_mode;
    int role_lead;
    hipStream_t slot_stream[STT_MAX_SLOTS];
    int scene_launch;
    int drop_tile;
    int b3;
    bool fe_in_role;
    int ode_method, ode_steps;
    int prog_len;
    hipStream_t sA, sB, sB2;
    std::mutex mu;
    unsigned* tmo_host;
    int lag_streams;
    long lag_calls;
    LagPending lag[STT_MAX_SLOTS];
    int lag_q[4][STT_MAX_SLOTS]; int lag_qn[4];
    hipStream_t sLag4;
    long acalls;
    hipEvent_t ev_call, evA_done[STT_MAX_SLOTS], evB_done[STT_MAX_SLOTS];
    bool timing;
    int timing_every;
    long calls;
    std::vector<TimRec> recs;
    std::vector<hipEvent_t> pool;
};

bool stt_embed_qkv_fe_covers(int n, int Tlen);
int stt_embed_qkv_fe(const float* const* W, const float* past, int n, int N, int Tlen, int TPX, float* xpad, float* enc_in, float* cur,
                     float* orig, int* last, float* g, float* qkv, void* stream);

int stt_post_attn_stage(const float* const* W, const float* state, const float* attn, int ld_attn, const float* base, const float* kA, float cA,
                        const float* kB, float cB, const float* kC, float cC, float cN, float* kout, float* out, float* qkv, const float* g,
                        float* pf, int n, void* stream);

static std::mutex g_stream_mu;

#define STT_TMO_WORDS 4096
static unsigned* g_tmo_pool = nullptr;
static std::vector<int> g_tmo_free;
static unsigned* tmo_word_take() {
    std::lock_guard<std::mutex> lk(g_stream_mu);
    if (!g_tmo_pool) {
        if (hipHostMalloc((void**)&g_tmo_pool, STT_TMO_WORDS * sizeof(unsigned), hipHostMallocDefault) != hipSuccess) { g_tmo_pool = nullptr; return nullptr; }
        memset(g_tmo_pool, 0, STT_TMO_WORDS * sizeof(unsigned));
        for (int i = STT_TMO_WORDS - 1; i >= 0; --i) g_tmo_free.push_back(i);
    }
    if (g_tmo_free.empty()) return nullptr;
    const int i = g_tmo_free.back();
    g_tmo_free.pop_back();
    g_tmo_pool[i] = 0u;
    return g_tmo_pool + i;
}
static void tmo_word_give(unsigned* w) {
    if (!w || !g_tmo_pool) return;
    std::lock_guard<std::mutex> lk(g_stream_mu);
    g_tmo_free.push_back((int)(w - g_tmo_pool));
}

static inline size_t al(size_t x) { return (x + 63) & ~(size_t)63; }

extern "C" int sttode_model_create(SttodeModel** out, const void* const* weights, int count, int Tp, int Tf, int K,
                                   int n_chunks0, int n_chunks1) {
    STT_REQUIRE(out && weights, "sttode_model_create: null pointer");
    STT_REQUIRE(count == STT_W_COUNT, "sttode_model_create: weight table must have STT_W_COUNT entries");
    STT_REQUIRE(Tp >= 2 && 2 * Tp <= 32 && Tf >= 1 && K >= 1, "sttode_model_create: bad Tp/Tf/K");
    for (int i = 0; i < count; ++i)
        STT_REQUIRE(weights[i] != nullptr || i == STT_W_CHAINB3_POOL || i == STT_W_CHAINB3_PROG, "sttode_model_create: null weight pointer");
    SttodeModel* m = new SttodeModel();
    m->Tp = Tp; m->Tf = Tf; m->K = K;
    m->TPX = (2 * Tp <= 16) ? 1 : 2;
    m->NOY = (2 * Tf + 15) / 16;
    for (int i = 0; i < count; ++i) m->w[i] = (const float*)weights[i];
    m->n_chunks0 = n_chunks0; m->n_chunks1 = n_chunks1;
    m->timing = false;
    m->timing_every = 0;
    m->calls = 0;
    m->acalls = 0;
    m->chain_mode = -1;
    m->ode_method = 0; m->ode_steps = 1;
    m->fused_mode = 1;
    m->b3 = 0;
    m->role_lead = -1;
    m->drop_tile = -1;
    for (int p = 0; p < STT_MAX_SLOTS; ++p) { m->slot_stream[p] = nullptr; m->lag[p].valid = false; }
    m->lag_streams = 3;
    m->lag_calls = 0;
    m->tmo_host = nullptr;
    for (int i = 0; i < 4; ++i) m->lag_qn[i] = 0;
    if (const char* e = getenv("STTODE_LAGGED")) m->lag_streams = atoi(e) >= 2 && atoi(e) <= 4 ? atoi(e) : 0;
    m->scene_launch = 128;
    m->fe_in_role = false;
    m->prog_len = sttode_chain_prog_len(Tp, Tf);
    m->side = nullptr;
    bool ok = hipEventCreateWithFlags(&m->ev_fork, hipEventDisableTiming) == hipSuccess &&
              hipEventCreateWithFlags(&m->ev_join, hipEventDisableTiming) == hipSuccess;
    static hipStream_t g_sA[STT_MAX_DEVICES] = {}, g_sB[STT_MAX_DEVICES] = {}, g_sB2[STT_MAX_DEVICES] = {};
    static hipStream_t g_sLag4[STT_MAX_DEVICES] = {};
    int dev = 0;
    ok = ok && hipGetDevice(&dev) == hipSuccess && dev >= 0 && dev < STT_MAX_DEVICES;
    if (ok) {
        std::lock_guard<std::mutex> lk(g_stream_mu);
        if (!g_sA[dev]) {
            ok = hipStreamCreateWithFlags(&g_sA[dev], hipStreamNonBlocking) == hipSuccess &&
                 hipStreamCreateWithFlags(&g_sB[dev], hipStreamNonBlocking) == hipSuccess &&
                 hipStreamCreateWithFlags(&g_sB2[dev], hipStreamNonBlocking) == hipSuccess;
            if (!ok) g_sA[dev] = nullptr;
        }
        if (ok) { m->sA = g_sA[dev]; m->sB = g_sB[dev]; m->sB2 = g_sB2[dev]; }
        if (ok && !g_sLag4[dev]) ok = hipStreamCreateWithFlags(&g_sLag4[dev], hipStreamNonBlocking) == hipSuccess;
        m->sLag4 = g_sLag4[dev];
    }
    ok = ok && hipEventCreateWithFlags(&m->ev_call, hipEventDisableTiming) == hipSuccess;
    if (ok) { m->tmo_host = tmo_word_take(); ok = m->tmo_host != nullptr; }
    for (int p = 0; p < STT_MAX_SLOTS && ok; ++p)
        ok = hipEventCreateWithFlags(&m->evA_done[p], hipEventDisableTiming) == hipSuccess &&
             hipEventCreateWithFlags(&m->evB_done[p], hipEventDisableTiming) == hipSuccess;
    if (!ok) {
        tmo_word_give(m->tmo_host);
        delete m;
        stt_set_error("sttode_model_create: could not create streams / events");
        return 2;
    }
    *out = m;
    return 0;
}

extern "C" int sttode_model_set_weight(SttodeModel* m, int index, const void* ptr) {
    STT_REQUIRE(m && ptr && index >= 0 && index < STT_W_COUNT, "sttode_model_set_weight: bad arguments");
    m->w[index] = (const float*)ptr;
    return 0;
}

extern "C" int sttode_model_destroy(SttodeModel* m) {
    if (!m) return 0;
    hipStreamCaptureMode mode = hipStreamCaptureModeRelaxed;
    const bool exchanged = hipThreadExchangeStreamCaptureMode(&mode) == hipSuccess;
    if (!exchanged) (void)hipGetLastError();
    for (auto& r : m->recs) { (void)hipEventDestroy(r.e0); (void)hipEventDestroy(r.e1); }
    for (auto e : m->pool) (void)hipEventDestroy(e);
    (void)hipEventDestroy(m->ev_fork); (void)hipEventDestroy(m->ev_join);
    (void)hipEventDestroy(m->ev_call);
    for (int p = 0; p < STT_MAX_SLOTS; ++p) { (void)hipEventDestroy(m->evA_done[p]); (void)hipEventDestroy(m->evB_done[p]); }
    tmo_word_give(m->tmo_host);
    delete m;
    if (exchanged) (void)hipThreadExchangeStreamCaptureMode(&mode);
    return 0;
}

extern "C" int sttode_workspace_layout(const SttodeModel* m, int n, int S, long* offsets, long* total_floats) {
    STT_REQUIRE(m && offsets && total_floats, "sttode_workspace_layout: null pointer");
    STT_REQUIRE(n > 0 && S >= 0, "sttode_workspace_layout: bad n/S");
    const size_t mm = (size_t)n * m->K;
    size_t o = 0;
    auto put = [&](int id, size_t cnt) { offsets[id] = (long)o; o += al(cnt); };
    put(STT_B_SCENE_ORIG, (size_t)(S > 0 ? S : 1) * 2);
    put(STT_B_AGENT_SCENE, n);
    put(STT_B_XPAD, (size_t)n * 16 * m->TPX);
    put(STT_B_ENC_IN, (size_t)n * m->Tp * 4);
    put(STT_B_CUR, (size_t)n * 2);
    put(STT_B_ORIG, (size_t)n * 2);
    put(STT_B_LAST, n);
    put(STT_B_G, (size_t)n * 64);
    put(STT_B_QKV, (size_t)n * 192);
    put(STT_B_ATTN, (size_t)n * 64);
    put(STT_B_PF, (size_t)n * 128);
    put(STT_B_STATE0, (size_t)n * 96);
    put(STT_B_A0X, (size_t)n * 512);
    put(STT_B_A0Y, (size_t)n * 512);
    put(STT_B_A1Y, (size_t)n * 512);
    put(STT_B_DBUF, mm * 16 * m->TPX);
    put(STT_B_YBUF, mm * 16 * m->NOY);
    put(STT_B_STATE1, mm * 96);
    put(STT_B_QUEUE, 64);
    put(STT_B_FLAGS, (size_t)8 * ((n + 15) / 16) + 8 + (mm + 15) / 16);
    put(STT_B_ODE, (size_t)6 * n * 64);
    *total_floats = (long)o;
    return 0;
}

extern "C" int sttode_set_chain(SttodeModel* m, int mode) {
    STT_REQUIRE(m, "sttode_set_chain: null model");
    STT_REQUIRE(mode >= -1 && mode <= 1, "sttode_set_chain: mode must be -1 (auto), 0 or 1");
    m->chain_mode = mode;
    return 0;
}

extern "C" int sttode_set_fused(SttodeModel* m, int mode) {
    STT_REQUIRE(m, "sttode_set_fused: null model");
    STT_REQUIRE(mode >= 0 && mode <= 4, "sttode_set_fused: mode must be 0 .. 4");
    m->fused_mode = mode ? 1 : 0;
    m->fe_in_role = mode == 2;
    m->role_lead = mode == 3 ? 160 : mode == 4 ? -2 : -1;
    return 0;
}

static int lag_flush_all(SttodeModel* m);
extern "C" int sttode_set_lagged(SttodeModel* m, int streams) {
    STT_REQUIRE(m, "sttode_set_lagged: null model");
    STT_REQUIRE(streams == 0 || (streams >= 2 && streams <= 4), "sttode_set_lagged: streams must be 0 (off), 2, 3 or 4");
    std::lock_guard<std::mutex> lk(m->mu);
    if (int rc = lag_flush_all(m)) return rc;
    m->lag_streams = streams;
    m->lag_calls = 0;
    return 0;
}

extern "C" int sttode_debug_drop_role_flag(SttodeModel* m, int tile) {
    STT_REQUIRE(m && tile >= -1, "sttode_debug_drop_role_flag: bad arguments");
    m->drop_tile = tile;
    return 0;
}

extern "C" int sttode_set_scene_launch(SttodeModel* m, int max_tiles) {
    STT_REQUIRE(m, "sttode_set_scene_launch: null model");
    STT_REQUIRE(max_tiles >= -1, "sttode_set_scene_launch: max_tiles must be -1 (default), 0 (off) or a tile count");
    m->scene_launch = max_tiles < 0 ? 128 : max_tiles;
    return 0;
}

extern "C" int sttode_set_mfma_mode(SttodeModel* m, int mode) {
    STT_REQUIRE(m, "sttode_set_mfma_mode: null model");
    STT_REQUIRE(mode == 0 || mode == 1, "sttode_set_mfma_mode: mode must be 0 (fp32) or 1 (three-way bf16 split, exploratory)");
    STT_REQUIRE(mode == 0 || (m->w[STT_W_CHAINB3_POOL] && m->w[STT_W_CHAINB3_PROG]),
                "sttode_set_mfma_mode: the bf16-split weight stream has not been handed over (sttode_model_set_weight)");
    m->b3 = mode;
    return 0;
}

extern "C" int sttode_set_ode(SttodeModel* m, int method, int steps) {
    STT_REQUIRE(m, "sttode_set_ode: null model");
    STT_REQUIRE(method >= 0 && method <= 2 && steps >= 1 && steps <= 1024, "sttode_set_ode: method in {0,1,2}, 1 <= steps <= 1024");
    m->ode_method = method; m->ode_steps = steps;
    return 0;
}

extern "C" int sttode_timing_enable(SttodeModel* m, int every) {
    STT_REQUIRE(m && every >= 0, "sttode_timing_enable: bad arguments");
    m->timing_every = every;
    m->timing = false;
    m->calls = 0;
    return 0;
}

static hipEvent_t get_event(SttodeModel* m) {
    if (!m->pool.empty()) { hipEvent_t e = m->pool.back(); m->pool.pop_back(); return e; }
    hipEvent_t e = nullptr;
    (void)hipEventCreate(&e);
    return e;
}

extern "C" int sttode_timing_read(SttodeModel* m, double* total_ms, int* launches, double* busy_ms) {
    STT_REQUIRE(m && total_ms && launches, "sttode_timing_read: null pointer");
    for (int i = 0; i < STT_STAGE_COUNT; ++i) { total_ms[i] = 0.0; launches[i] = 0; if (busy_ms) busy_ms[i] = 0.0; }
    std::vector<std::pair<double, double>> iv[STT_STAGE_COUNT];
    hipEvent_t ref = m->recs.empty() ? nullptr : m->recs.front().e0;
    for (auto& r : m->recs) {
        STT_HIP(hipEventSynchronize(r.e1));
        float ms = 0.f, t0 = 0.f;
        STT_HIP(hipEventElapsedTime(&ms, r.e0, r.e1));
        total_ms[r.stage] += ms;
        launches[r.stage] += 1;
        if (busy_ms && r.e0 != ref) {
            STT_HIP(hipEventSynchronize(r.e0));
            STT_HIP(hipEventElapsedTime(&t0, ref, r.e0));
        }
        iv[r.stage].push_back({(double)t0, (double)t0 + (double)ms});
    }
    if (busy_ms)
        for (int st = 0; st < STT_STAGE_COUNT; ++st) {
            std::sort(iv[st].begin(), iv[st].end());
            double cur0 = 0, cur1 = 0;
            bool open = false;
            for (auto& p : iv[st]) {
                if (!open) { cur0 = p.first; cur1 = p.second; open = true; }
                else if (p.first <= cur1) { if (p.second > cur1) cur1 = p.second; }
                else { busy_ms[st] += cur1 - cur0; cur0 = p.first; cur1 = p.second; }
            }
            if (open) busy_ms[st] += cur1 - cur0;
        }
    for (auto& r : m->recs) { m->pool.push_back(r.e0); m->pool.push_back(r.e1); }
    m->recs.clear();
    return 0;
}

struct StageTimer {
    SttodeModel* m; int stage; hipStream_t s; hipEvent_t e0 = nullptr, e1 = nullptr; bool on = false;
    StageTimer(SttodeModel* m_, int st, hipStream_t s_) : m(m_), stage(st), s(s_) {
        on = m->timing || (m->timing_every > 0 && ((stage >= STT_STAGE_MLP0 && stage <= STT_STAGE_CHAIN) || stage == STT_STAGE_FUSED));
        if (on) { e0 = get_event(m); e1 = get_event(m); (void)hipEventRecord(e0, s); }
    }
    ~StageTimer() {
        if (on) { (void)hipEventRecord(e1, s); m->recs.push_back({stage, e0, e1}); }
    }
};

// ... 83 lines not shown
            return last ? 0 : attention_of_state();
        };
#define ODE_DO(call) do { if (int _rc = (call)) return _rc; } while (0)
        const double h = 12.0 / (double)m->ode_steps;
        for (int st = 0; st < m->ode_steps; ++st) {
            const bool fin = st + 1 == m->ode_steps;
            const float* y0 = st == 0 ? g : y;
            if (m->ode_method == 0) { ODE_DO(stage(y0, y0, nullptr, 0, nullptr, 0, nullptr, 0, h, nullptr, y, fin)); continue; }
            if (m->ode_method == 1) {
                ODE_DO(stage(y0, y0, nullptr, 0, nullptr, 0, nullptr, 0, h / 3, k1, t, false));
                ODE_DO(stage(t, y0, k1, -h / 3, nullptr, 0, nullptr, 0, h, k2, t, false));
                ODE_DO(stage(t, y0, k1, h, k2, -h, nullptr, 0, h, k3, t, false));
                ODE_DO(stage(t, y0, k1, h / 8, k2, 3 * h / 8, k3, 3 * h / 8, h / 8, nullptr, y, fin));
            } else {
                ODE_DO(stage(y0, y0, nullptr, 0, nullptr, 0, nullptr, 0, h / 2, k1, t, false));
                ODE_DO(stage(t, y0, nullptr, 0, nullptr, 0, nullptr, 0, h / 2, k2, t, false));
                ODE_DO(stage(t, y0, nullptr, 0, nullptr, 0, nullptr, 0, h, k3, t, false));
                ODE_DO(stage(t, y0, k1, h / 6, k2, h / 3, k3, h / 3, h / 6, nullptr, y, fin));
            }
        }
#undef ODE_DO
    } else if (m->ode_method != 0 || m->ode_steps != 1) {
        RUN(STT_STAGE_POST, s,
            sttode_post_attn_ode(W[STT_W_OUTP], W[STT_W_OUTB], W[STT_W_INFOP], W[STT_W_INFOB], W[STT_W_GATEP], W[STT_W_GATEB], W[STT_W_LN1W],
                                 W[STT_W_LN1B], W[STT_W_L1P], W[STT_W_L1B], W[STT_W_L2P], W[STT_W_L2B], W[STT_W_LN2W], W[STT_W_LN2B],
                                 W[STT_W_INP], W[STT_W_INB], g, pf, n, 12.0f, m->ode_method, m->ode_steps, s));
    } else
    RUN(STT_STAGE_POST, s,
        sttode_post_attn(W[STT_W_OUTP], W[STT_W_OUTB], W[STT_W_INFOP], W[STT_W_INFOB], W[STT_W_GATEP], W[STT_W_GATEB], W[STT_W_LN1W],
                         W[STT_W_LN1B], W[STT_W_L1P], W[STT_W_L1B], W[STT_W_L2P], W[STT_W_L2B], W[STT_W_LN2W], W[STT_W_LN2B], g,
                         attn_src, ld_attn, pf, n, 12.0f, s));
    if (use_side) STT_HIP(hipStreamWaitEvent(s, m->ev_join, 0));
    RUN(STT_STAGE_LINEAR, s,
        sttode_agent_preact(pf, state0, W[STT_W_B0_XWA], W[STT_W_B0_XB1], W[STT_W_B0_YWA], W[STT_W_B0_YB1], W[STT_W_B1_YWA], W[STT_W_B1_YB1],
                            A0x, A0y, A1y, n, s));
    return 0;
}

static int stage_trajectories(SttodeModel* m, float* ws, const long* off, int n, const float* z, float* pred, hipStream_t s, bool pipelined) {
    const float* const* W = m->w;
    const int K = m->K, Tp = m->Tp, Tf = m->Tf, TPX = m->TPX, NOY = m->NOY;
    const float* xpad = ws + off[STT_B_XPAD];
    const float *A0x = ws + off[STT_B_A0X], *A0y = ws + off[STT_B_A0Y], *A1y = ws + off[STT_B_A1Y];
    float *dbuf = ws + off[STT_B_DBUF], *ybuf = ws + off[STT_B_YBUF], *state1 = ws + off[STT_B_STATE1];
    const long ncols_all = (long)n * K;
    const bool fused = m->chain_mode == 1 || (m->chain_mode < 0 && ncols_all >= 16384);
    if (fused) {
        if (m->b3) {
            RUN(STT_STAGE_CHAIN, s,
                stt_traj_chain_b3(A0x, A0y, A1y, W[STT_W_CHAINB3_POOL], (const int*)W[STT_W_CHAINB3_PROG], m->prog_len, W[STT_W_CHAIN_CONSTS], z,
                                  xpad, 16 * TPX, ws + off[STT_B_CUR], ws + off[STT_B_ORIG], pred, (int*)(ws + off[STT_B_QUEUE]), (int)ncols_all, K,
                                  Tp, Tf, pipelined ? 1 : 2, s));
            return 0;
        }
        RUN(STT_STAGE_CHAIN, s,
            sttode_traj_chain(A0x, A0y, A1y, W[STT_W_CHAIN_POOL], (const int*)W[STT_W_CHAIN_PROG], m->prog_len, W[STT_W_CHAIN_CONSTS], z,
                              xpad, 16 * TPX, ws + off[STT_B_CUR], ws + off[STT_B_ORIG], pred, (int*)(ws + off[STT_B_QUEUE]), (int)ncols_all, K,
                              Tp, Tf, pipelined ? 1 : 2, s));
        return 0;
    }
    const int nc = (int)ncols_all;
    RUN(STT_STAGE_MLP0, s,
        sttode_mlp_block0(A0x, A0y, W[STT_W_B0_STREAM], m->n_chunks0, z, xpad, dbuf, ybuf, nc, K, TPX, NOY, s));
    RUN(STT_STAGE_GRU1, s,
        sttode_gru_cols(dbuf, W[STT_W_B1_CONVP], W[STT_W_B1_CONVB], W[STT_W_B1_WIHP], W[STT_W_B1_WHHP], W[STT_W_B1_GBIAS], state1, nc, Tp, TPX, s));
    RUN(STT_STAGE_MLP1, s,
        sttode_mlp_block1(A1y, W[STT_W_B1_STREAM], m->n_chunks1, z, state1, ybuf, ws + off[STT_B_CUR], ws + off[STT_B_ORIG], pred, nc, K, Tf,
                          NOY, s));
    return 0;
}

static int frontend(SttodeModel* m, float* ws, const long* off, const float* past, const int* scene_ptr, int n, int S, int nbaN,
                    hipStream_t s) {
    if (scene_ptr) {
        RUN(STT_STAGE_FRONTEND, s,
            sttode_frontend_scenes(past, scene_ptr, n, S, m->Tp, m->TPX, 1, ws + off[STT_B_SCENE_ORIG],
                                   (int*)(ws + off[STT_B_AGENT_SCENE]), ws + off[STT_B_XPAD], ws + off[STT_B_ENC_IN], ws + off[STT_B_CUR],
                                   ws + off[STT_B_ORIG], (int*)(ws + off[STT_B_LAST]), s));
    } else {
        RUN(STT_STAGE_FRONTEND, s,
            sttode_frontend_nba(past, n, nbaN, m->Tp, m->TPX, ws + off[STT_B_XPAD], ws + off[STT_B_ENC_IN], ws + off[STT_B_CUR],
                                ws + off[STT_B_ORIG], (int*)(ws + off[STT_B_LAST]), s));
    }
    return 0;
}

static bool use_fused(const SttodeModel* m, int n) {
    const long ncols_all = (long)n * m->K;
    const bool chain = m->chain_mode == 1 || (m->chain_mode < 0 && ncols_all >= 16384);
    return m->fused_mode == 1 && chain && m->ode_method == 0 && m->ode_steps == 1 && stt_chain_fused_covers(m->Tp);
}
static bool use_scene_launch(const SttodeModel* m, int n, const int* scene_ptr) {
    const long ncols_all = (long)n * m->K;
    const bool chain = m->chain_mode == 1 || (m->chain_mode < 0 && ncols_all >= 16384);
    return scene_ptr != nullptr && !chain && m->scene_launch > 0 && (ncols_all + 15) / 16 <= m->scene_launch && m->ode_method == 0 &&
           m->ode_steps == 1 && stt_scene_lat_covers(m->Tp, m->TPX, m->NOY);
}
static int stage_fused(SttodeModel* m, float* ws, const long* off, int n, int groups, int attn_len, int attn_slots, const float* z, float* pred,
                       const float* past, const int* scene_ptr, int S, hipStream_t s) {
    const float* const* W = m->w;
    const float* attn = nullptr;
    if (attn_len > 1) {
        float* qkv = ws + off[STT_B_QKV];
        RUN(STT_STAGE_EMBED, s,
            sttode_embed_qkv(W[STT_W_FC1P], W[STT_W_FC1B], W[STT_W_POSP], W[STT_W_PEB], W[STT_W_FC2P], W[STT_W_FC2B], W[STT_W_FC3P],
                             W[STT_W_FC3B], W[STT_W_FC3LAST], W[STT_W_INP], W[STT_W_INB], ws + off[STT_B_ENC_IN],
                             (const int*)(ws + off[STT_B_LAST]), ws + off[STT_B_G], qkv, n, m->Tp, s));
        RUN(STT_STAGE_ATTN, s, attention(qkv, ws + off[STT_B_ATTN], groups, attn_len, attn_slots, s));
        attn = ws + off[STT_B_ATTN];
    }
    RUN(STT_STAGE_FUSED, s, stt_chain_fused(W, ws, off, n, m->K, m->Tp, m->Tf, m->prog_len, z, pred, 12.0f, attn, 64, past, scene_ptr, S, 2, m->b3, m->role_lead, m->drop_tile,
                                            m->tmo_host, s));
    return 0;
}

static inline void arm_timing(SttodeModel* m) {
    m->timing = m->timing_every > 0 && (m->calls % m->timing_every) == 0;
    ++m->calls;
}

static int run_serial(SttodeModel* m, const float* past, const int* scene_ptr, int n, int S, int G, int B, int N, const float* z, float* ws,
                      float* pred, hipStream_t s) {
    arm_timing(m);
    long off[STT_B_COUNT], tot;
    if (int rc = sttode_workspace_layout(m, n, S, off, &tot)) return rc;
    if (use_scene_launch(m, n, scene_ptr)) {
        RUN(STT_STAGE_FUSED, s,
            stt_scene_lat(m->w, ws, off, n, m->K, m->Tp, m->Tf, m->TPX, m->NOY, m->n_chunks0, m->n_chunks1, z, pred, 12.0f, past, scene_ptr, S,
                          m->drop_tile, m->tmo_host, s));
        return 0;
    }
    const bool fe_in_role = use_fused(m, n) && scene_ptr != nullptr && m->fe_in_role;
    if (!fe_in_role)
        if (int rc = frontend(m, ws, off, past, scene_ptr, n, S, N, s)) return rc;
    if (use_fused(m, n))
        return stage_fused(m, ws, off, n, G, scene_ptr ? 1 : B, scene_ptr ? 1 : N, z, pred, fe_in_role ? past : nullptr, scene_ptr, S, s);
    if (int rc = stage_agents(m, ws, off, n, G, scene_ptr ? 1 : B, scene_ptr ? 1 : N, s, true)) return rc;
    return stage_trajectories(m, ws, off, n, z, pred, s, false);
}

static bool use_lagged(const SttodeModel* m, int n) {
    const long ncols_all = (long)n * m->K;
    const bool chain = m->chain_mode == 1 || (m->chain_mode < 0 && ncols_all >= 16384);
    return m->lag_streams > 0 && m->fused_mode == 1 && chain && m->ode_method == 0 && m->ode_steps == 1 && stt_chain_lagged_covers(m->Tp);
}
static hipStream_t lag_stream(const SttodeModel* m, int si) { return si == 0 ? m->sB : si == 1 ? m->sB2 : si == 2 ? m->sA : m->sLag4; }
static void lag_unqueue(SttodeModel* m, int slot) {
    const int si = m->lag[slot].si;
    int w = 0;
    for (int i = 0; i < m->lag_qn[si]; ++i)
        if (m->lag_q[si][i] != slot) m->lag_q[si][w++] = m->lag_q[si][i];
    m->lag_qn[si] = w;
}
static int lag_flush(SttodeModel* m, int slot) {
    LagPending& p = m->lag[slot];
    if (!p.valid) return 0;
    lag_unqueue(m, slot);
    p.valid = false;
    LagRoles none = {};
    LagGroups lg = {p.ws, p.off, p.n, p.z, p.pred, p.gt, p.ade, p.fde, p.scale, p.one_launch};
    RUN(STT_STAGE_FUSED, p.s, stt_chain_lagged(m->w, none, lg, m->K, m->Tp, m->Tf, m->prog_len, m->b3, p.s));
    STT_HIP(hipEventRecord(m->evB_done[slot], p.s));
    return 0;
}
static int lag_flush_all(SttodeModel* m) {
    for (int p = 0; p < STT_MAX_SLOTS; ++p)
        if (int rc = lag_flush(m, p)) return rc;
    return 0;
}
static int run_lagged(SttodeModel* m, const float* past, const int* scene_ptr, int n, int S, int G, int B, int N, const float* z, float* ws,
                      float* pred, int slot, const long* off, const SttodeAsyncOpts& o, hipStream_t s) {
    const float* const* W = m->w;
    const int si = (int)(m->lag_calls % m->lag_streams);
    hipStream_t sf = lag_stream(m, si);
    ++m->lag_calls;
    STT_HIP(hipStreamWaitEvent(sf, m->ev_call, 0));
    STT_HIP(hipStreamWaitEvent(sf, m->evB_done[slot], 0));
    const bool fe_role = scene_ptr != nullptr;
    const bool fe_embed = !scene_ptr && B > 1 && stt_embed_qkv_fe_covers(n, m->Tp);
    if (!fe_role && !fe_embed)
        if (int rc = frontend(m, ws, off, past, scene_ptr, n, S, N, sf)) return rc;
    const float* attn = nullptr;
    if (!scene_ptr && B > 1) {
        float* qkv = ws + off[STT_B_QKV];
        if (fe_embed) {
            RUN(STT_STAGE_EMBED, sf,
                stt_embed_qkv_fe(W, past, n, N, m->Tp, m->TPX, ws + off[STT_B_XPAD], ws + off[STT_B_ENC_IN], ws + off[STT_B_CUR], ws + off[STT_B_ORIG],
                                 (int*)(ws + off[STT_B_LAST]), ws + off[STT_B_G], qkv, sf));
        } else
        RUN(STT_STAGE_EMBED, sf,
            sttode_embed_qkv(W[STT_W_FC1P], W[STT_W_FC1B], W[STT_W_POSP], W[STT_W_PEB], W[STT_W_FC2P], W[STT_W_FC2B], W[STT_W_FC3P],
                             W[STT_W_FC3B], W[STT_W_FC3LAST], W[STT_W_INP], W[STT_W_INB], ws + off[STT_B_ENC_IN],
                             (const int*)(ws + off[STT_B_LAST]), ws + off[STT_B_G], qkv, n, m->Tp, sf));
        RUN(STT_STAGE_ATTN, sf, attention(qkv, ws + off[STT_B_ATTN], G, B, N, sf));
        attn = ws + off[STT_B_ATTN];
    }
    const int gs = m->lag_qn[si] > 0 ? m->lag_q[si][0] : -1;
    LagPending* g = gs >= 0 ? &m->lag[gs] : nullptr;
    float* zgen = o.device_latents ? const_cast<float*>(z) : nullptr;
    const bool met = o.metrics_gt != nullptr;
    LagRoles lr = {ws, off, n, attn, 64, 12.0f, zgen, o.zkey, fe_role ? past : nullptr, fe_role ? scene_ptr : nullptr, fe_role ? S : 0,
                   met ? o.ade : nullptr, met ? o.fde : nullptr};
    LagGroups lg = {};
    if (g) lg = LagGroups{g->ws, g->off, g->n, g->z, g->pred, g->gt, g->ade, g->fde, g->scale, fe_role && g->one_launch};
    RUN(STT_STAGE_FUSED, sf, stt_chain_lagged(W, lr, lg, m->K, m->Tp, m->Tf, m->prog_len, m->b3, sf));
    if (g) {
        lag_unqueue(m, gs);
        g->valid = false;
        STT_HIP(hipEventRecord(m->evB_done[gs], sf));
    }
    if (o.sampler)
        if (int rc = stt_sampler_qnet(o.sampler, ws + off[STT_B_PF], n, const_cast<float*>(z), sf)) return rc;
    LagPending& p = m->lag[slot];
    p.valid = true; p.ws = ws; p.n = n; p.z = z; p.pred = pred; p.s = sf; p.si = si;
    p.one_launch = fe_role;
    p.gt = met ? o.metrics_gt : nullptr; p.ade = met ? o.ade : nullptr; p.fde = met ? o.fde : nullptr; p.scale = met ? o.metrics_scale : 1.0f;
    memcpy(p.off, off, sizeof(p.off));
    m->lag_q[si][m->lag_qn[si]++] = slot;
    m->slot_stream[slot] = sf;
    return 0;
}

static int run_async(SttodeModel* m, const float* past, const int* scene_ptr, int n, int S, int G, int B, int N, const float* z, float* ws,
                     float* pred, int slot, const SttodeAsyncOpts* opts, hipStream_t s) {
    STT_REQUIRE(slot >= 0 && slot < STT_MAX_SLOTS, "sttode_inference_*_async: slot must be in [0, 8)");
    std::lock_guard<std::mutex> lk(m->mu);
    SttodeAsyncOpts o = {};
    if (opts) o = *opts;
    if (o.device_latents || o.metrics_gt) {
        STT_REQUIRE(use_lagged(m, n), "sttode_inference_*_async: device latents / fused metrics need the lagged form (sttode_async_is_lagged)");
        STT_REQUIRE(!o.metrics_gt || (o.ade && o.fde), "sttode_inference_*_async: fused metrics need the ade / fde outputs");
    }
    if (o.sampler) {
        STT_REQUIRE(!o.device_latents, "sttode_inference_*_async: a sampler plan and device_latents both ask to fill z: pass one of them");
        STT_REQUIRE(use_lagged(m, n), "sttode_inference_*_async: a sampler plan needs the lagged form (sttode_async_is_lagged)");
        if (const char* why = stt_sampler_plan_check(o.sampler, m->K)) {
            char b[256];
            snprintf(b, sizeof(b), "sttode_inference_*_async: %s", why);
            stt_set_error(b);
            return 1;
        }
    }
    arm_timing(m);
    long off[STT_B_COUNT], tot;
    if (int rc = sttode_workspace_layout(m, n, S, off, &tot)) return rc;
    if (int rc = lag_flush(m, slot)) return rc;
    STT_HIP(hipEventRecord(m->ev_call, s));
    if (use_lagged(m, n)) return run_lagged(m, past, scene_ptr, n, S, G, B, N, z, ws, pred, slot, off, o, s);
    if (use_fused(m, n)) {
        hipStream_t sf = m->sB;
        ++m->acalls;
        STT_HIP(hipStreamWaitEvent(sf, m->ev_call, 0));
        STT_HIP(hipStreamWaitEvent(sf, m->evB_done[slot], 0));
        const bool fe_in_role = scene_ptr != nullptr && m->fe_in_role;
        if (!fe_in_role)
            if (int rc = frontend(m, ws, off, past, scene_ptr, n, S, N, sf)) return rc;
        if (int rc = stage_fused(m, ws, off, n, G, scene_ptr ? 1 : B, scene_ptr ? 1 : N, z, pred, fe_in_role ? past : nullptr, scene_ptr, S, sf)) return rc;
        STT_HIP(hipEventRecord(m->evB_done[slot], sf));
        m->slot_stream[slot] = sf;
        return 0;
    }
    STT_HIP(hipStreamWaitEvent(m->sA, m->ev_call, 0));
    STT_HIP(hipStreamWaitEvent(m->sA, m->evB_done[slot], 0));
    if (int rc = frontend(m, ws, off, past, scene_ptr, n, S, N, m->sA)) return rc;
    if (int rc = stage_agents(m, ws, off, n, G, scene_ptr ? 1 : B, scene_ptr ? 1 : N, m->sA, false)) return rc;
    STT_HIP(hipEventRecord(m->evA_done[slot], m->sA));
    hipStream_t sb = (m->acalls++ & 1) ? m->sB2 : m->sB;
    STT_HIP(hipStreamWaitEvent(sb, m->ev_call, 0));
    STT_HIP(hipStreamWaitEvent(sb, m->evA_done[slot], 0));
    if (int rc = stage_trajectories(m, ws, off, n, z, pred, sb, true)) return rc;
    STT_HIP(hipEventRecord(m->evB_done[slot], sb));
    m->slot_stream[slot] = sb;
    return 0;
}

extern "C" int sttode_inference_scenes(SttodeModel* m, const float* past, const int* scene_ptr, int n, int S, const float* z,
                                       float* workspace, float* pred, void* stream) {
    STT_REQUIRE(m && past && scene_ptr && z && workspace && pred, "sttode_inference_scenes: null pointer");
    STT_REQUIRE(n > 0 && S > 0, "sttode_inference_scenes: n and S must be positive");
    return run_serial(m, past, scene_ptr, n, S, 1, 1, 1, z, workspace, pred, (hipStream_t)stream);
}

extern "C" int sttode_inference_nba(SttodeModel* m, const float* past, int B, int N, const float* z, float* workspace, float* pred,
                                    void* stream) {
    STT_REQUIRE(m && past && z && workspace && pred, "sttode_inference_nba: null pointer");
    STT_REQUIRE(B > 0 && N > 0, "sttode_inference_nba: B and N must be positive");
    return run_serial(m, past, nullptr, B * N, 0, 1, B, N, z, workspace, pred, (hipStream_t)stream);
}

extern "C" int sttode_inference_nba_groups(SttodeModel* m, const float* past, int G, int B, int N, const float* z, float* workspace,
                                           float* pred, void* stream) {
    STT_REQUIRE(m && past && z && workspace && pred, "sttode_inference_nba_groups: null pointer");
    STT_REQUIRE(G > 0 && B > 0 && N > 0 && (long)G * B * N <= 0x7fffffffL / 64, "sttode_inference_nba_groups: G, B and N must be positive (and G B N small enough)");
    return run_serial(m, past, nullptr, G * B * N, 0, G, B, N, z, workspace, pred, (hipStream_t)stream);
}

extern "C" int sttode_inference_scenes_async(SttodeModel* m, const float* past, const int* scene_ptr, int n, int S, const float* z,
                                             float* workspace, float* pred, int slot, const SttodeAsyncOpts* opts, void* stream) {
    STT_REQUIRE(m && past && scene_ptr && z && workspace && pred, "sttode_inference_scenes_async: null pointer");
    STT_REQUIRE(n > 0 && S > 0, "sttode_inference_scenes_async: n and S must be positive");
    return run_async(m, past, scene_ptr, n, S, 1, 1, 1, z, workspace, pred, slot, opts, (hipStream_t)stream);
}

extern "C" int sttode_inference_nba_async(SttodeModel* m, const float* past, int B, int N, const float* z, float* workspace,
                                          float* pred, int slot, const SttodeAsyncOpts* opts, void* stream) {
    STT_REQUIRE(m && past && z && workspace && pred, "sttode_inference_nba_async: null pointer");
    const int G = opts && opts->nba_groups > 1 ? opts->nba_groups : 1;
    STT_REQUIRE(B > 0 && N > 0 && (long)G * B * N <= 0x7fffffffL / 64, "sttode_inference_nba_async: B and N must be positive (and groups x B x N small enough)");
    return run_async(m, past, nullptr, G * B * N, 0, G, B, N, z, workspace, pred, slot, opts, (hipStream_t)stream);
}

extern "C" int sttode_async_best_of_k(SttodeModel* m, int slot, const float* pred, const float* gt, int n, int K, int Tf, float scale,
                                      float* ade, float* fde) {
    STT_REQUIRE(m && slot >= 0 && slot < STT_MAX_SLOTS, "sttode_async_best_of_k: bad model / slot");
    std::lock_guard<std::mutex> lk(m->mu);
    STT_REQUIRE(m->slot_stream[slot] != nullptr, "sttode_async_best_of_k: no asynchronous call has used this slot");
    if (int rc = lag_flush(m, slot)) return rc;
    if (int rc = sttode_best_of_k(pred, gt, n, K, Tf, scale, ade, fde, m->slot_stream[slot])) return rc;
    STT_HIP(hipEventRecord(m->evB_done[slot], m->slot_stream[slot]));
    return 0;
}

extern "C" int sttode_async_best_of_k_select(SttodeModel* m, int slot, const float* pred, const float* gt, int n, int K, int Tf, float scale,
                                             float miss_threshold, const int* seg_ptr, int S, float* ade, float* fde, int* best_ade_idx,
                                             int* best_fde_idx, unsigned char* miss, float* best, float* seg_ade, float* seg_fde,
                                             int* seg_miss) {
    STT_REQUIRE(m && slot >= 0 && slot < STT_MAX_SLOTS, "sttode_async_best_of_k_select: bad model / slot");
    std::lock_guard<std::mutex> lk(m->mu);
    STT_REQUIRE(m->slot_stream[slot] != nullptr, "sttode_async_best_of_k_select: no asynchronous call has used this slot");
    if (int rc = lag_flush(m, slot)) return rc;
    if (int rc = sttode_best_of_k_select(pred, gt, n, K, Tf, scale, miss_threshold, seg_ptr, S, ade, fde, best_ade_idx, best_fde_idx, miss,
                                         best, seg_ade, seg_fde, seg_miss, m->slot_stream[slot]))
        return rc;
    STT_HIP(hipEventRecord(m->evB_done[slot], m->slot_stream[slot]));
    return 0;
}

extern "C" int sttode_async_joint_select(SttodeModel* m, int slot, const float* pred, const float* gt, int n, int K, int Tf, float scale,
                                         const int* seg_ptr, int S, float radius, float* seg_jade, float* seg_jfde, int* seg_jade_idx,
                                         int* seg_jfde_idx, int* seg_col, int* seg_gt_col) {
    STT_REQUIRE(m && slot >= 0 && slot < STT_MAX_SLOTS, "sttode_async_joint_select: bad model / slot");
    if (stt_joint_check("sttode_async_joint_select", pred, gt, n, K, Tf, seg_ptr, S, radius, seg_jade, seg_jfde, seg_jade_idx, seg_jfde_idx,
                        seg_col, seg_gt_col))
        return 1;
    std::lock_guard<std::mutex> lk(m->mu);
    STT_REQUIRE(m->slot_stream[slot] != nullptr, "sttode_async_joint_select: no asynchronous call has used this slot");
    if (int rc = lag_flush(m, slot)) return rc;
    if (int rc = sttode_joint_select(pred, gt, n, K, Tf, scale, seg_ptr, S, radius, seg_jade, seg_jfde, seg_jade_idx, seg_jfde_idx, seg_col,
                                     seg_gt_col, m->slot_stream[slot]))
        return rc;
    STT_HIP(hipEventRecord(m->evB_done[slot], m->slot_stream[slot]));
    return 0;
}

extern "C" int sttode_async_kde_nll(SttodeModel* m, int slot, const float* pred, const float* gt, int n, int K, int Tf, float scale, double* nll) {
    STT_REQUIRE(m && slot >= 0 && slot < STT_MAX_SLOTS, "sttode_async_kde_nll: bad model / slot");
    if (stt_kde_check("sttode_async_kde_nll", pred, gt, n, K, Tf, nll)) return 1;
    std::lock_guard<std::mutex> lk(m->mu);
    STT_REQUIRE(m->slot_stream[slot] != nullptr, "sttode_async_kde_nll: no asynchronous call has used this slot");
    if (int rc = lag_flush(m, slot)) return rc;
    if (int rc = sttode_kde_nll(pred, gt, n, K, Tf, scale, nll, m->slot_stream[slot])) return rc;
    STT_HIP(hipEventRecord(m->evB_done[slot], m->slot_stream[slot]));
    return 0;
}

extern "C" int sttode_async_sample_spread(SttodeModel* m, int slot, const float* pred, const float* gt, int n, int K, int Tf, float scale,
                                          double div_scale, double* apd, double* fpd, double* pade, double* dlow, double* es_ade,
                                          double* es_fde, float* ade_at_k, float* fde_at_k) {
    STT_REQUIRE(m && slot >= 0 && slot < STT_MAX_SLOTS, "sttode_async_sample_spread: bad model / slot");
    if (stt_spread_check("sttode_async_sample_spread", pred, gt, n, K, Tf, div_scale, apd, fpd, pade, dlow, es_ade, es_fde, ade_at_k, fde_at_k))
        return 1;
    std::lock_guard<std::mutex> lk(m->mu);
    STT_REQUIRE(m->slot_stream[slot] != nullptr, "sttode_async_sample_spread: no asynchronous call has used this slot");
    if (int rc = lag_flush(m, slot)) return rc;
    if (int rc = sttode_sample_spread(pred, gt, n, K, Tf, scale, div_scale, apd, fpd, pade, dlow, es_ade, es_fde, ade_at_k, fde_at_k,
                                      m->slot_stream[slot]))
        return rc;
    STT_HIP(hipEventRecord(m->evB_done[slot], m->slot_stream[slot]));
    return 0;
}

extern "C" int sttode_async_horizon_metrics(SttodeModel* m, int slot, const float* pred, const float* gt, int n, int K, int Tf, float scale,
                                            float* out) {
    STT_REQUIRE(m && slot >= 0 && slot < STT_MAX_SLOTS, "sttode_async_horizon_metrics: bad model / slot");
    std::lock_guard<std::mutex> lk(m->mu);
    STT_REQUIRE(m->slot_stream[slot] != nullptr, "sttode_async_horizon_metrics: no asynchronous call has used this slot");
    if (int rc = lag_flush(m, slot)) return rc;
    if (int rc = sttode_horizon_metrics(pred, gt, n, K, Tf, scale, out, m->slot_stream[slot])) return rc;
    STT_HIP(hipEventRecord(m->evB_done[slot], m->slot_stream[slot]));
    return 0;
}

extern "C" int sttode_async_next_stream(SttodeModel* m, int n, void** stream) {
    STT_REQUIRE(m && stream && n > 0, "sttode_async_next_stream: bad arguments");
    std::lock_guard<std::mutex> lk(m->mu);
    *stream = nullptr;
    if (use_lagged(m, n)) { *stream = lag_stream(m, (int)(m->lag_calls % m->lag_streams)); return 0; }
    if (use_fused(m, n)) *stream = m->sB;
    return 0;
}

extern "C" int sttode_async_is_lagged(SttodeModel* m, int n) { return m && n > 0 && use_lagged(m, n) ? 1 : 0; }

extern "C" int sttode_wait_host(SttodeModel* m, int slot) {
    STT_REQUIRE(m && slot >= 0 && slot < STT_MAX_SLOTS, "sttode_wait_host: bad arguments");
    hipEvent_t ev;
    {
        std::lock_guard<std::mutex> lk(m->mu);
        if (int rc = lag_flush(m, slot)) return rc;
        ev = m->evB_done[slot];
    }
    STT_HIP(hipEventSynchronize(ev));
    return 0;
}

extern "C" int sttode_wait(SttodeModel* m, int slot, void* stream) {
    STT_REQUIRE(m && slot >= 0 && slot < STT_MAX_SLOTS, "sttode_wait: bad arguments");
    std::lock_guard<std::mutex> lk(m->mu);
    if (int rc = lag_flush(m, slot)) return rc;
    STT_HIP(hipStreamWaitEvent((hipStream_t)stream, m->evB_done[slot], 0));
    return 0;
}

extern "C" int sttode_async_enqueue(SttodeModel* m, int slot) {
    STT_REQUIRE(m && slot >= 0 && slot < STT_MAX_SLOTS, "sttode_async_enqueue: bad model / slot");
    std::lock_guard<std::mutex> lk(m->mu);
    return lag_flush(m, slot);
}

extern "C" int sttode_async_flush(SttodeModel* m) {
    STT_REQUIRE(m, "sttode_async_flush: null model");
    std::lock_guard<std::mutex> lk(m->mu);
    return lag_flush_all(m);
}

extern "C" int sttode_workspace_init(SttodeModel* m, float* workspace, int n, int S, void* stream) {
    STT_REQUIRE(m && workspace && n > 0 && S >= 0, "sttode_workspace_init: bad arguments");
    long off[STT_B_COUNT], tot;
    if (int rc = sttode_workspace_layout(m, n, S, off, &tot)) return rc;
    STT_HIP(hipMemsetAsync(workspace + off[STT_B_FLAGS], 0, (size_t)(off[STT_B_ODE] - off[STT_B_FLAGS]) * 4, (hipStream_t)stream));
    return stt_scene_flags_init(workspace, off, n, m->K, stream);
}

extern "C" int sttode_timeout_word(SttodeModel* m, const unsigned** word) {
    STT_REQUIRE(m && word && m->tmo_host, "sttode_timeout_word: bad arguments");
    *word = m->tmo_host;
    return 0;
}
extern "C" int sttode_timeout_clear(SttodeModel* m) {
    STT_REQUIRE(m && m->tmo_host, "sttode_timeout_clear: bad arguments");
    __atomic_store_n(m->tmo_host, 0u, __ATOMIC_RELAXED);
    return 0;
}

extern "C" int sttode_check(SttodeModel* m, const float* workspace, int n, int S, void* stream) {
    STT_REQUIRE(m && workspace && n > 0 && S >= 0, "sttode_check: bad arguments");
    long off[STT_B_COUNT], tot;
    if (int rc = sttode_workspace_layout(m, n, S, off, &tot)) return rc;
    unsigned word[2] = {0, 0};
    const float* f = workspace + off[STT_B_FLAGS];
    STT_HIP(hipMemcpyAsync(&word[0], f + (n + 15) / 16, sizeof(unsigned), hipMemcpyDeviceToHost, (hipStream_t)stream));
    STT_HIP(hipMemcpyAsync(&word[1], f + stt_scene_flags_offset(n) + (n + 15) / 16, sizeof(unsigned), hipMemcpyDeviceToHost, (hipStream_t)stream));
    STT_HIP(hipStreamSynchronize((hipStream_t)stream));
    if (word[1] == 2u) {
        stt_set_error("sttode_check: the workspace was never initialised (sttode_workspace_init): the one-launch scene form refused its flag words; the predictions of that call are not valid");
        return 3;
    }
    if (word[0] != 0 || word[1] != 0) {
        stt_set_error("sttode_check: a trajectory group gave up waiting for its per-agent role (time-out word set): the predictions of that call are not valid");
        return 3;
    }
    return 0;
}
```

sttode_amd/model.py:

```python
import os
import operator

import numpy as np
import torch
from torch import nn

from .dist import Normal
from . import capi, packing
from .weights import sinusoid_table_np

_DEBUG = os.environ.get('STTODE_DEBUG', '0') not in ('', '0')


class _HypMHSA(nn.Module):

    def __init__(self, d, h):
        super().__init__()
        self.embed_dim, self.num_heads = d, h
        self.in_proj_weight = nn.Parameter(torch.empty(3 * d, d))
        self.in_proj_bias = nn.Parameter(torch.zeros(3 * d))
        self.out_proj = nn.Linear(d, d)
        nn.init.xavier_uniform_(self.in_proj_weight)
        nn.init.zeros_(self.out_proj.bias)


class _HypAttention(nn.Module):
    def __init__(self, d, h):
        super().__init__()
        self.temporal_attention_before = _HypMHSA(d, h)
        self.temporal_info = nn.Linear(d, d)
        self.temporal_gate = nn.Linear(d, d)


class _EncoderLayer(nn.Module):
    def __init__(self, d, h, ff):
        super().__init__()
        self.self_attn = _HypAttention(d, h)
        self.linear1 = nn.Linear(d, ff)
        self.linear2 = nn.Linear(ff, d)
        self.norm1 = nn.LayerNorm(d)
        self.norm2 = nn.LayerNorm(d)


class _Named(nn.Module):
    def __init__(self, **children):
        super().__init__()
        for k, v in children.items():
            setattr(self, k, v)


class _PosEnc(nn.Module):
    def __init__(self, d, max_t_len=200):
        super().__init__()
        self.fc = nn.Linear(2 * d, d)
        self.register_buffer('pe', torch.from_numpy(sinusoid_table_np(max_t_len, d)))


class _Trunk(nn.Module):

    def __init__(self, args, length, future=False):
        super().__init__()
        D = args.hidden_dim
        self.input_fc = nn.Linear(4, D)
        self.input_fc2 = nn.Linear(D * length, D)
        self.input_fc3 = nn.Linear(D + 3, D)
        layers = nn.ModuleList([_EncoderLayer(D, 8, 1024)])
        self.ODE_Encoder = _Named(odeblock=_Named(odefunc=_Named(layers=layers)))
        self.pos_encoder = _PosEnc(D)
        if future:
            self.out_mlp = _Named(affine_layers=nn.ModuleList([nn.Linear((2 + len(args.hyper_scales)) * D, 128)]))
            self.qz_layer = nn.Linear(128, 2 * args.zdim)
            for m in (self.out_mlp.affine_layers[0], self.qz_layer):
                nn.init.normal_(m.weight, 0, 0.01)
                nn.init.zeros_(m.bias)


class _MLP(nn.Module):
    def __init__(self, din, dout, hidden=(512, 256)):
        super().__init__()
        dims = [din, *hidden, dout]
        self.layers = nn.ModuleList(nn.Linear(a, b) for a, b in zip(dims[:-1], dims[1:]))


class _DecomposeBlock(nn.Module):
    def __init__(self, past_len, future_len, input_dim):
        super().__init__()
        self.conv_past = nn.Conv1d(2, 32, 3, stride=1, padding=1)
        self.encoder_past = nn.GRU(32, 96, 1, batch_first=True)
        self.decoder_y = _MLP(96 + input_dim, future_len * 2)
        self.decoder_x = _MLP(96 + input_dim, past_len * 2)
        nn.init.kaiming_normal_(self.conv_past.weight)
        nn.init.kaiming_normal_(self.encoder_past.weight_ih_l0)
        nn.init.kaiming_normal_(self.encoder_past.weight_hh_l0)
        nn.init.zeros_(self.conv_past.bias)
        nn.init.zeros_(self.encoder_past.bias_ih_l0)
        nn.init.zeros_(self.encoder_past.bias_hh_l0)


class _Decoder(nn.Module):
    def __init__(self, args):
        super().__init__()
        din = 2 * args.hidden_dim + args.zdim
        self.decompose = nn.ModuleList(_DecomposeBlock(args.past_length, args.future_length, din)
                                       for _ in range(args.num_decompose))


_DATA_PTR = torch.Tensor.data_ptr
_VERSION = operator.attrgetter('_version')


def _on(t, device):
    device = torch.device(device)
    return t.device.type == device.type and (device.index is None or t.device.index == device.index)


def _f32(t, device):
    if isinstance(t, torch.Tensor) and t.dtype == torch.float32 and _on(t, device) and t.is_contiguous():
        return t
    return torch.as_tensor(t, dtype=torch.float32).to(device).contiguous()


class _LazyViews(dict):

    def __init__(self, makers):
        super().__init__()
        self._makers = makers

    def __missing__(self, key):
        if key not in self._makers:
            raise KeyError(key)
        v = self[key] = self._makers[key]()
        return v

    def get(self, key, default=None):
        try:
            return self[key]
        except KeyError:
            return default


class STTODENet(nn.Module):
    ODE_TIME = 12.0
    ODE_METHODS = {'euler': 0, 'rk4': 1, 'rk4_classic': 2}

    def __init__(self, args, device):
        super().__init__()
        from . import generic
        why = generic.unsupported_reason(args)
        if why is not None:
            raise NotImplementedError(why)
        self._generic = generic.uses_generic(args)
        self.device = torch.device(device)
        self.args = args
        self.max_train_agent = args.max_train_agent
        self.rand_rot_scene = args.rand_rot_scene
        self.discrete_rot = args.discrete_rot
        scale_num = 2 + len(args.hyper_scales)
        self.past_encoder = _Trunk(args, args.past_length)
        self.pz_layer = nn.Linear(scale_num * args.hidden_dim, 2 * args.zdim)
        self.future_encoder = _Trunk(args, args.future_length, future=True)
        self.decoder = _Decoder(args)
        self.param_annealers = nn.ModuleList()
        self._packed = None
        self._packed_key = None
        self._mode = None
        self._async_calls = 0
        self.ode_method, self.ode_steps = 'euler', 1
        self.mfma_mode = 'bf16x3' if os.environ.get('STTODE_BF16X3', '0') not in ('', '0') else 'f32'
        self._host_futures = {}
        self.async_depth = 6
        self.device_latents = os.environ.get('STTODE_DEVICE_LATENTS', '1') != '0'
        self._async_bufs = {}
        self._async_metrics = {}
        self._ext_streams = {}
        self._ptr_cache = {}
        self._pf = self._pf_thunk = None
        self.to(self.device)

    @property
    def past_feature(self):
        if self._pf is None and self._pf_thunk is not None:
            self._pf, self._pf_thunk = self._pf_thunk(), None
        return self._pf

    @past_feature.setter
    def past_feature(self, value):
        self._pf, self._pf_thunk = value, None

    _PLAIN = frozenset(('_past', '_future', '_scene_ptr', '_mode', 'batch_size', 'agent_num', '_S', '_N', '_G', 'pre_motion_mask', 'fut_motion_mask',
                        'scene_orig', '_pf', '_pf_thunk', '_ws', '_dbg', 'diverse_pred', '_plist'))

    def __setattr__(self, name, value):
        if name in STTODENet._PLAIN:
            self.__dict__[name] = value
        else:
            super().__setattr__(name, value)

    def set_device(self, device):
        self.device = torch.device(device)
        self.to(self.device)

    def step_annealer(self):
        for anl in self.param_annealers:
            anl.step()

    def _weights_key(self):
        if getattr(self, '_plist', None) is None:
            self._plist = list(self.parameters()) + list(self.buffers())
        return (self.device.index, tuple(map(_DATA_PTR, self._plist)), tuple(map(_VERSION, self._plist)))

    def _apply(self, fn, *a, **k):
        self._plist = None
        return super()._apply(fn, *a, **k)

    def packed(self):
        if self._generic:
            return {}
        key = self._weights_key()
        if self._packed is None or key != self._packed_key:
            if getattr(self, '_native', None) is not None:
                capi.call('sttode_async_flush', self._native.h)
                torch.cuda.synchronize(self.device)
            sd = {k: v.detach().cpu().numpy() for k, v in self.state_dict().items()}
            a = self.args
            host = {'past': packing.pack_trunk(sd, 'past_encoder.', a.past_length),
                    'blk0': packing.pack_block(sd, 0, a.past_length, a.future_length, first=True),
                    'blk1': packing.pack_block(sd, 1, a.past_length, a.future_length, first=False),
                    'future': packing.pack_trunk(sd, 'future_encoder.', a.future_length),
                    'post': packing.pack_posterior(sd),
                    'chain': packing.chain_stream(sd, a.past_length, a.future_length),
                    'gru0s': packing.gru32_stream(sd, 0, a.past_length),
                    'role32': packing.role_stream(sd, a.past_length)}
            self._packed = {g: {k: (torch.from_numpy(np.ascontiguousarray(v)).to(self.device) if isinstance(v, np.ndarray) else v)
                                for k, v in d.items()} for g, d in host.items()}
            self._packed_key = key
            self._native = capi.NativeModel(self._packed, a.past_length, a.future_length, a.sample_k) if self.device.type == 'cuda' else None
            self._wscache = {}
            self._async_bufs = {}
        return self._packed

    def release_native(self):
        if self.device.type == 'cuda':
            if getattr(self, '_native', None) is not None:
                capi.call('sttode_async_flush', self._native.h)
            torch.cuda.synchronize(self.device)
        self._native, self._packed, self._packed_key = None, None, None
        self._wscache, self._async_bufs = {}, {}

    def native(self, check_weights=True):
        if self._generic:
            raise capi.SttodeError('the native pipeline (fused launches, packed weight streams) is built for the reference widths hidden_dim 64, '
                                   'zdim 32, num_decompose 2, 2 Tp <= 32, 2 Tf <= 96; this model runs the generic form (sttode_amd/generic.py)')
        if check_weights or self._packed is None or self._native is None:
            self.packed()
        ode = (self.ODE_METHODS[self.ode_method], int(self.ode_steps))
        if self._native is not None and getattr(self._native, '_ode', (0, 1)) != ode:
            self._native.set_ode(*ode)
            self._native._ode = ode
        if self._native is not None and getattr(self._native, '_mfma', None) != self.mfma_mode:
            if self.mfma_mode not in ('f32', 'bf16x3'):
                raise ValueError("mfma_mode must be 'f32' or 'bf16x3'")
            if self.mfma_mode == 'bf16x3' and 'chain_b3' not in self._packed:
                sd = {k: v.detach().cpu().numpy() for k, v in self.state_dict().items()}
                b3 = packing.chain_stream_b3(sd, self.args.past_length, self.args.future_length)
                self._native.set_weights('chain_b3', {k: (torch.from_numpy(np.ascontiguousarray(v)).to(self.device) if isinstance(v, np.ndarray) else v)
                                                      for k, v in b3.items()})
            self._native.set_mfma_mode(1 if self.mfma_mode == 'bf16x3' else 0)
            self._native._mfma = self.mfma_mode
        return self._native

    def _workspace(self, n, S):
        key = (n, S)
        if key not in self._wscache:
            if len(self._wscache) > 8:
                self._wscache.clear()
            off, tot = self._native.layout(n, S)
            buf = torch.empty(tot, dtype=torch.float32, device=self.device)
            self._native.init_workspace(buf, n, S)
            self._wscache[key] = (buf, off)
        return self._wscache[key]

    def _view(self, buf, off, name, *shape, dtype=torch.float32):
        cnt = int(np.prod(shape))
        v = buf[off[name]: off[name] + cnt]
        if dtype != torch.float32:
            v = v.view(dtype)
        return v.view(*shape)

    def _require_gpu(self):
        if self.device.type != 'cuda':
            raise capi.SttodeError('STTODENet compute runs only on a HIP device (no CPU fallback); got device=%s' % self.device)

    def set_data(self, batch, pre_motion, fut_motion, pre_motion_mask=None, fut_motion_mask=None, theta=None):
        dev = self.device
        if (not self.training and theta is None and type(pre_motion) is torch.Tensor and type(fut_motion) is torch.Tensor
                and pre_motion.dtype is torch.float32 and fut_motion.dtype is torch.float32 and not pre_motion.is_cuda and not fut_motion.is_cuda
                and dev.type == 'cuda' and pre_motion.dim() == 3 and pre_motion.shape[1] == 2 and pre_motion.shape[2] == self.args.past_length
                and pre_motion.shape[0] > 0 and fut_motion.shape == (pre_motion.shape[0], 2, self.args.future_length)):
            N = pre_motion.shape[0]
            past, fut = self._stage_scene(pre_motion, fut_motion)
            ptr = self._ptr_cache.get(N)
            if ptr is None or not _on(ptr, dev):
                ptr = self._ptr_cache[N] = torch.tensor([0, N], dtype=torch.int32).to(dev)
            d = self.__dict__
            d['_past'], d['_future'], d['_scene_ptr'], d['_mode'], d['batch_size'], d['agent_num'], d['_S'], d['_N'] = past, fut, ptr, 'scenes', 1, N, 1, 0
            d['_G'] = 1
            d['pre_motion_mask'], d['fut_motion_mask'] = pre_motion_mask, fut_motion_mask
            return

        def to_dev(x):
            x = torch.as_tensor(x, dtype=torch.float32)
            return x.permute(0, 2, 1).contiguous().to(dev)
        pre_motion = torch.as_tensor(pre_motion, dtype=torch.float32)
        fut_motion = torch.as_tensor(fut_motion, dtype=torch.float32) if fut_motion is not None else None
        if torch.device(dev).type == 'cuda' and not pre_motion.is_cuda and (fut_motion is None or not fut_motion.is_cuda):
            past, fut = self._stage_scene(pre_motion, fut_motion)
        else:
            past = to_dev(pre_motion)
            fut = to_dev(fut_motion) if fut_motion is not None else None
        if self.training and past.shape[0] > self.max_train_agent:
            ind = torch.tensor(np.random.choice(past.shape[0], self.max_train_agent).tolist(), device=dev)
            past = past.index_select(0, ind).contiguous()
# ... 353 lines not shown
            if not late or attempt or self._weights_key() == self._packed_key:
                break
            nat = self.native()
            buf, off = self._workspace(n, S)
        if self._mode == 'scenes':
            so = self._view(buf, off, 'scene_orig', S, 2)
            self.scene_orig = so[0] if S == 1 else so
        m = n * K
        self._pf, self._pf_thunk = None, (lambda: self._view(buf, off, 'pf', n, 128))
        self._ws = _LazyViews({'xpad': lambda: self._view(buf, off, 'xpad', n, 16 * TPX), 'enc_in': lambda: self._view(buf, off, 'enc_in', n, Tp, 4),
                               'cur': lambda: self._view(buf, off, 'cur', n, 2), 'orig': lambda: self._view(buf, off, 'orig', n, 2)})
        self._dbg = _LazyViews({'state0': lambda: self._view(buf, off, 'state0', n, 96), 'dbuf': lambda: self._view(buf, off, 'dbuf', m, 16 * TPX),
                                'ybuf': lambda: self._view(buf, off, 'ybuf', m, 16 * NOY), 'state1': lambda: self._view(buf, off, 'state1', m, 96)})
        self.diverse_pred = pred
        return pred.permute(1, 0, 2, 3)

    def _round_buffer(self, rounds, n):
        bufs = self.__dict__.setdefault('_reduce_bufs', {})
        key = (int(rounds), int(n), self.args.sample_k, self.args.future_length)
        if key not in bufs:
            if len(bufs) > 8:
                bufs.clear()
            bufs[key] = torch.empty(*key, 2, dtype=torch.float32, device=self.device)
        return bufs[key]

    @torch.no_grad()
    def inference_reduced(self, rounds, K=None, iters=10, from_frame=0, init='first', z=None):
        from . import metrics
        self._require_gpu()
        rounds = int(rounds)
        if rounds < 1:
            raise ValueError(f'inference_reduced needs rounds >= 1, got {rounds}')
        if self._mode is None:
            raise capi.SttodeError('call set_data / set_data_nba / set_scene_batch before inference_reduced()')
        if z is not None and (getattr(z, 'ndim', 0) != 3 or z.shape[0] != rounds):
            raise ValueError(f'z must be [rounds = {rounds}, n * sample_k, zdim], got {tuple(getattr(z, "shape", ()))}')
        K = self.args.sample_k if K is None else int(K)
        buf = self._round_buffer(rounds, self._past.shape[0])
        for r in range(rounds):
            self.inference(None, z=None if z is None else z[r])
            buf[r].copy_(self.diverse_pred)
        red = metrics.reduce_samples(buf, K, iters=iters, from_frame=from_frame, init=init)
        self.__dict__['reduction'] = red
        self.diverse_pred = red.centroids
        return red.centroids.permute(1, 0, 2, 3)

    @torch.no_grad()
    def inference_nba_sharded(self, data_local, z=None, gather=None):
        self._require_gpu()
        a, P = self.args, self.packed()
        self.set_data_nba(data_local)
        ws = self._frontend(vel_from_norm=1)
        n, N, W = self._past.shape[0], self._N, P['past']
        st = capi.stream_ptr()
        g, qkv = self._f(n, 64), self._f(n, 192)
        capi.call('sttode_embed_qkv', W['fc1P'], W['fc1b'], W['posP'], W['peb'], W['fc2P'], W['fc2b'], W['fc3P'], W['fc3b'],
                  W['fc3last'], W['inP'], W['inb'], ws['enc_in'], ws['last'], g, qkv, n, a.past_length, st)
        if gather is None:
            from . import parallel
            gather = parallel.gather_futures
        qkv_all = gather(qkv).contiguous()
        L_all, L_loc = qkv_all.shape[0] // N, n // N
        attn = self._f(n, 64)
        e = qkv.element_size()
        capi.call('sttode_mhgsa_attn', qkv.data_ptr() + 64 * e, qkv_all.data_ptr(), qkv_all.data_ptr() + 128 * e, attn, None, None,
                  L_loc, L_all, N, N * 192, 192, N * 192, 192, N * 192, 192, N * 64, 64, 1.0, 8.0 ** -0.5, st)
        pf = self._f(n, 128)
        capi.call('sttode_post_attn', W['outP'], W['outb'], W['infoP'], W['infob'], W['gateP'], W['gateb'], W['ln1w'], W['ln1b'],
                  W['l1P'], W['l1b'], W['l2P'], W['l2b'], W['ln2w'], W['ln2b'], g, attn, 64, pf, n, self.ODE_TIME, st)
        self.past_feature, self._ws = pf, ws
        K = a.sample_k
        if z is None:
            z = torch.randn(n * K, a.zdim, device=self.device)
        pred = self._decode(pf, z, ws, K)
        self._keep = (g, qkv, qkv_all)
        return pred.permute(1, 0, 2, 3)

    @torch.no_grad()
    def inference_async(self, z=None, metrics_gt=None, metrics_scale=1.0, pred_host=False, sampler_plan=None):
        self._require_gpu()
        a = self.args
        if self._mode is None:
            raise capi.SttodeError('call set_data / set_data_nba / set_scene_batch before inference_async()')
        if sampler_plan is not None and (self._generic or z is not None):
            raise capi.SttodeError('inference_async: a sampler plan fills z itself and needs the lagged form of the reference widths')
        if self._generic:
            if pred_host:
                raise capi.SttodeError('pred_host=True needs the lagged pipelined form (reference widths)')
            out = self.inference(None, z=z)
            return {'generic': True, 'fused_metrics': None, 'slot': -1, 'pred': self.diverse_pred, 'z': None, 'metrics': None,
                    'gt_default': self._future, 'stream': None, 'inputs': (self._past, getattr(self, '_scene_ptr', None))}
        nat = self.native()
        nat.raise_if_timed_out()
        K, n = a.sample_k, self._past.shape[0]
        S = self._S if self._mode == 'scenes' else 0
        lagged = bool(capi.lib().sttode_async_is_lagged(nat.h, n))
        if z is not None:
            if not (isinstance(z, torch.Tensor) and z.is_cuda and z.dtype == torch.float32 and z.is_contiguous()):
                z = _f32(z, self.device)
            if tuple(z.shape) != (n * K, a.zdim):
                raise ValueError(f'z must be [{n * K}, {a.zdim}], got {tuple(z.shape)}')
        if metrics_gt is not None and not (isinstance(metrics_gt, torch.Tensor) and metrics_gt.is_cuda and metrics_gt.dtype == torch.float32
                                           and metrics_gt.is_contiguous() and tuple(metrics_gt.shape) == (n, a.future_length, 2)):
            raise ValueError(f'metrics_gt must be a contiguous float32 device tensor [{n}, {a.future_length}, 2]')
        if pred_host and not lagged:
            raise capi.SttodeError('pred_host=True needs the lagged pipelined form (a chain-sized batch, reference integrator)')
        if sampler_plan is not None and not lagged:
            raise capi.SttodeError('inference_async: a sampler plan needs the lagged pipelined form (a chain-sized batch, reference integrator)')
        slot = self._async_calls % max(2, min(8, int(self.async_depth)))
        key = (n, S, slot)
        if key not in self._async_bufs:
            if len(self._async_bufs) > 16:
                raise capi.SttodeError('too many distinct batch shapes in flight for the async pipeline; call reset_async()')
            _, tot = nat.layout(n, S)
            ws = torch.empty(tot, dtype=torch.float32, device=self.device)
            nat.init_workspace(ws, n, S)
            self._async_bufs[key] = (ws, torch.empty(n, K, a.future_length, 2, dtype=torch.float32, device=self.device),
                                     torch.empty(n * K, a.zdim, dtype=torch.float32, device=self.device))
        self._async_calls += 1
        opts = capi.AsyncOpts()
        if sampler_plan is not None:
            import ctypes
            opts.sampler = ctypes.addressof(sampler_plan)
            z = self._async_bufs[key][2]
        elif z is None:
            if self.device_latents and lagged:
                opts.device_latents, opts.zkey = 1, int(torch.empty((), dtype=torch.int64).random_()) & 0x7fffffffffffffff
                z = self._async_bufs[key][2]
            else:
                z = torch.randn(n * K, a.zdim, device=self.device)
        buf, pred = self._async_bufs[key][:2]
        if pred_host:
            hk = ('host',) + key
            if hk not in self._async_bufs:
                self._async_bufs[hk] = torch.empty(n, K, a.future_length, 2, dtype=torch.float32).pin_memory()
            pred = self._async_bufs[hk]
        st = capi.stream_ptr()
        pstream = self.next_async_stream(n)
        mb = self._async_metrics.get(key)
        if mb is None:
            t = torch.empty(2, n, dtype=torch.float32, device=self.device)
            mb = self._async_metrics[key] = (t[0], t[1])
        fused = None
        if metrics_gt is not None and lagged:
            opts.metrics_gt, opts.ade, opts.fde, opts.metrics_scale = metrics_gt.data_ptr(), mb[0].data_ptr(), mb[1].data_ptr(), float(metrics_scale)
            fused = (metrics_gt, float(metrics_scale))
        import ctypes
        if self._mode == 'scenes':
            capi.call('sttode_inference_scenes_async', nat.h, self._past, self._scene_ptr, n, S, z, buf, pred, slot, ctypes.addressof(opts), st)
        else:
            opts.nba_groups = getattr(self, '_G', 1)
            capi.call('sttode_inference_nba_async', nat.h, self._past, self.batch_size, self._N, z, buf, pred, slot, ctypes.addressof(opts), st)
        return {'fused_metrics': fused, 'slot': slot, 'pred': pred, 'z': z, 'inputs': (self._past, getattr(self, '_scene_ptr', None)), 'metrics': mb,
                'gt_default': self._future, 'stream': pstream}

    def wait(self, handle):
        if handle.get('generic'):
            return handle['pred'].permute(1, 0, 2, 3)
        nat = self.native()
        nat.raise_if_timed_out()
        capi.call('sttode_wait', nat.h, handle['slot'], capi.stream_ptr())
        return handle['pred'].permute(1, 0, 2, 3)

    def wait_host(self, handle):
        nat = self.native()
        capi.call('sttode_wait_host', nat.h, handle['slot'])
        nat.raise_if_timed_out()
        return handle['pred'].permute(1, 0, 2, 3)

    def futures_to_host_async(self, handle, out=None, workgroups=8):
        pred = handle['pred']
        if out is None:
            out = self._host_futures.get(handle['slot'])
            if out is None or out.shape != pred.shape:
                out = self._host_futures[handle['slot']] = torch.empty(pred.shape, dtype=torch.float32).pin_memory()
        elif not (out.is_pinned() and out.dtype == torch.float32 and out.is_contiguous() and out.shape == pred.shape):
            raise ValueError('futures_to_host_async: out must be a pinned contiguous float32 tensor of shape %s' % (tuple(pred.shape),))
        nat = self.native()
        capi.call('sttode_async_enqueue', nat.h, handle['slot'])
        st = handle['stream']
        raw = st.cuda_stream if st is not None else capi.stream_ptr()
        if st is None:
            capi.call('sttode_wait', nat.h, handle['slot'], raw)
        if (pred.numel() * 4) % 16 == 0:
            capi.call('sttode_copy_to_host', out, pred, pred.numel() * 4, int(workgroups), raw)
        else:
            with torch.cuda.stream(st if st is not None else torch.cuda.current_stream(self.device)):
                out.copy_(pred, non_blocking=True)
        ev = handle.get('host_event')
        if ev is None:
            ev = handle['host_event'] = torch.cuda.Event()
        ev.record(st if st is not None else torch.cuda.current_stream(self.device))
        handle['host'] = out
        return out

    def wait_host_copy(self, handle):
        handle['host_event'].synchronize()
        self.native().raise_if_timed_out()
        return handle['host'].permute(1, 0, 2, 3)

    def next_async_stream(self, n):
        if self._generic:
            return None
        return self._next_async_stream(n)

    def _next_async_stream(self, n):
        import ctypes
        out = ctypes.c_void_p(0)
        capi.call('sttode_async_next_stream', self.native().h, int(n), ctypes.addressof(out))
        if not out.value:
            return None
        st = self._ext_streams.get(out.value)
        if st is None:
            st = self._ext_streams[out.value] = torch.cuda.ExternalStream(out.value, device=self.device)
        return st

    def best_of_k_async(self, handle, gt=None, scale=1.0):
        if handle.get('generic'):
            return self.best_of_k(handle['pred'], gt=handle.get('gt_default') if gt is None else gt, scale=scale)
        fm = handle.get('fused_metrics')
        if fm is not None and (gt is None or gt.data_ptr() == fm[0].data_ptr()) and float(scale) == fm[1]:
            capi.call('sttode_async_enqueue', self.native().h, handle['slot'])
            return handle['metrics']
        gt = handle.get('gt_default') if gt is None else gt
        if not (isinstance(gt, torch.Tensor) and gt.is_cuda and gt.dtype == torch.float32 and gt.is_contiguous()):
            raise ValueError('best_of_k_async needs a contiguous float32 device tensor gt [n, Tf, 2] that was written before the call')
        pred = handle['pred']
        n, K, Tf = pred.shape[:3]
        mb = handle['metrics']
        capi.call('sttode_async_best_of_k', self.native().h, handle['slot'], pred, gt, n, K, Tf, float(scale), mb[0], mb[1])
        return mb[0], mb[1]

    @torch.no_grad()
    def select_best_of_k(self, pred_nk, gt=None, scale=1.0, miss_threshold=1.0, seg_ptr=None, gather=False):
        from . import metrics
        gt = self._future if gt is None else _f32(gt, self.device)
        return metrics.select(pred_nk, gt, scale=scale, miss_threshold=miss_threshold, seg_ptr=seg_ptr, gather=gather)

    def select_best_of_k_async(self, handle, gt=None, scale=1.0, miss_threshold=1.0, seg_ptr=None, gather=False):
        from . import metrics
        if isinstance(seg_ptr, str):
            if seg_ptr != 'scenes' or handle['inputs'][1] is None:
                raise ValueError("seg_ptr='scenes' needs a call made on a scene batch (set_scene_batch / set_data)")
            seg_ptr = handle['inputs'][1]
        gt = handle.get('gt_default') if gt is None else gt
        if handle.get('generic'):
            sel = self.select_best_of_k(handle['pred'], gt=gt, scale=scale, miss_threshold=miss_threshold, seg_ptr=seg_ptr, gather=gather)
            handle['selection'] = sel
            return sel
        if not (isinstance(gt, torch.Tensor) and gt.is_cuda and gt.dtype == torch.float32 and gt.is_contiguous()):
            raise ValueError('select_best_of_k_async needs a contiguous float32 device tensor gt [n, Tf, 2] that was written before the call')
        if seg_ptr is not None and not (isinstance(seg_ptr, torch.Tensor) and seg_ptr.is_cuda and seg_ptr.dtype == torch.int32
                                        and seg_ptr.is_contiguous()):
            raise ValueError('select_best_of_k_async needs seg_ptr as a contiguous int32 device tensor written before the call')
        pred = handle['pred']
        n, K, Tf = pred.shape[:3]
        metrics.check_k(K)
        if tuple(gt.shape) != (n, Tf, 2):
            raise ValueError(f'gt must be [{n}, {Tf}, 2], got {tuple(gt.shape)}')
        S = int(seg_ptr.numel()) - 1 if seg_ptr is not None else 0
        sel = metrics.Selection(n, S, Tf, self.device, gather)
        capi.call('sttode_async_best_of_k_select', self.native().h, handle['slot'], pred, gt, n, K, Tf, float(scale), float(miss_threshold),
                  seg_ptr, S, *sel.args())
        if handle.get('stream') is not None:
            sel.record_stream(handle['stream'])
        handle['selection'] = sel
        return sel

    @torch.no_grad()
    def select_joint(self, pred_nk, gt=None, seg_ptr=None, scale=1.0, collision_radius=None):
        from . import metrics
        gt = self._future if gt is None else _f32(gt, self.device)
        if seg_ptr is None:
            seg_ptr = getattr(self, '_scene_ptr', None)
            if seg_ptr is None:
                raise ValueError('select_joint needs seg_ptr (no scene batch is set)')
        return metrics.joint_select(pred_nk, gt, seg_ptr, scale=scale, collision_radius=collision_radius)

    @torch.no_grad()
    def kde_nll(self, pred_nk, gt=None, scale=1.0):
        from . import metrics
        gt = self._future if gt is None else _f32(gt, self.device)
        return metrics.kde_nll(pred_nk, gt, scale=scale)

    def _async_metric_inputs(self, handle, gt, what):
        gt = handle.get('gt_default') if gt is None else gt
        if not (isinstance(gt, torch.Tensor) and gt.is_cuda and gt.dtype == torch.float32 and gt.is_contiguous()):
            raise ValueError(f'{what} needs a contiguous float32 device tensor gt [n, Tf, 2] that was written before the call')
        pred = handle['pred']
        n, K, Tf = pred.shape[:3]
        if tuple(gt.shape) != (n, Tf, 2):
            raise ValueError(f'gt must be [{n}, {Tf}, 2], got {tuple(gt.shape)}')
        return pred, gt, n, K, Tf

    def select_joint_async(self, handle, gt=None, seg_ptr='scenes', scale=1.0, collision_radius=None):
        from . import metrics
        if isinstance(seg_ptr, str):
            if seg_ptr != 'scenes' or handle['inputs'][1] is None:
                raise ValueError("seg_ptr='scenes' needs a call made on a scene batch (set_scene_batch / set_data)")
            seg_ptr = handle['inputs'][1]
        if handle.get('generic'):
            js = self.select_joint(handle['pred'], gt=handle.get('gt_default') if gt is None else gt, seg_ptr=seg_ptr, scale=scale,
                                   collision_radius=collision_radius)
            handle['joint'] = js
            return js
        if not (isinstance(seg_ptr, torch.Tensor) and seg_ptr.is_cuda and seg_ptr.dtype == torch.int32 and seg_ptr.is_contiguous()):
            raise ValueError('select_joint_async needs seg_ptr as a contiguous int32 device tensor written before the call')
        pred, gt, n, K, Tf = self._async_metric_inputs(handle, gt, 'select_joint_async')
        metrics.check_k(K)
        r = metrics.check_radius(collision_radius)
        metrics.check_seg_ptr(seg_ptr, n)
        S = int(seg_ptr.numel()) - 1
        js = metrics.JointSelection(S, self.device, r)
        capi.call('sttode_async_joint_select', self.native().h, handle['slot'], pred, gt, n, K, Tf, float(scale), seg_ptr, S, *js.args())
        if handle.get('stream') is not None:
            js.record_stream(handle['stream'])
        handle['joint'] = js
        return js

    def kde_nll_async(self, handle, gt=None, scale=1.0):
        from . import metrics
        if handle.get('generic'):
            out = self.kde_nll(handle['pred'], gt=handle.get('gt_default') if gt is None else gt, scale=scale)
            handle['kde_nll'] = out
            return out
        pred, gt, n, K, Tf = self._async_metric_inputs(handle, gt, 'kde_nll_async')
        metrics.check_kde_k(K)
        out = torch.empty(n, dtype=torch.float64, device=self.device)
        capi.call('sttode_async_kde_nll', self.native().h, handle['slot'], pred, gt, n, K, Tf, float(scale), out)
        if handle.get('stream') is not None:
            out.record_stream(handle['stream'])
        handle['kde_nll'] = out
        return out

    @torch.no_grad()
    def sample_spread(self, pred_nk, gt=None, scale=1.0, div_scale=1.0):
        from . import metrics
        gt = self._future if gt is None else _f32(gt, self.device)
        return metrics.sample_spread(pred_nk, gt, scale=scale, div_scale=div_scale)

    def sample_spread_async(self, handle, gt=None, scale=1.0, div_scale=1.0):
        from . import metrics
        if handle.get('generic'):
            out = self.sample_spread(handle['pred'], gt=handle.get('gt_default') if gt is None else gt, scale=scale, div_scale=div_scale)
            handle['spread'] = out
            return out
        pred, gt, n, K, Tf = self._async_metric_inputs(handle, gt, 'sample_spread_async')
        out = metrics.SampleSpread(n, K, self.device, metrics.check_spread(K, div_scale), True)
        capi.call('sttode_async_sample_spread', self.native().h, handle['slot'], pred, gt, n, K, Tf, float(scale), *out.args())
        if handle.get('stream') is not None:
            out.record_stream(handle['stream'])
        handle['spread'] = out
# ... 41 lines not shown
```

Baseline: 86.86 million.

## Fold device-to-host future copies into the next lagged chain launch

Instead of launching a separate host_copy_kernel on the lane stream after each lagged call, the pinned-memory copy is deferred and carried by the next traj_chain_kernel launch on the same lane. That launch reserves extra leading workgroups that do nontemporal 16-byte loads and stores. Per-slot copy bookkeeping, events, guards and flush paths handle slots that get reused or waited on. The aim is to remove one kernel launch and its gap per step, at the cost of more host-side state, and the copy now finishes later because it waits for the following launch.

```diff
diff --git a/include/sttode_hip.h b/include/sttode_hip.h
--- a/include/sttode_hip.h
+++ b/include/sttode_hip.h
@@ -338,6 +338,9 @@
 int sttode_sampler_qnet(const SttodeSamplerPlan* plan, const float* pf, int n, float* z, void* stream);
 int sttode_clock_probe(long long* out, void* stream);
 int sttode_copy_to_host(void* dst, const void* src, long bytes, int wgs, void* stream);
+int sttode_async_copy_to_host(SttodeModel* m, int slot, void* dst, const void* src, long bytes, int wgs);
+int sttode_wait_host_copy(SttodeModel* m, int slot);
+int sttode_async_copy_stats(SttodeModel* m, long* rode, long* own_launch, int* pending);
 int sttode_async_enqueue(SttodeModel* m, int slot);
 int sttode_async_flush(SttodeModel* m);
 int sttode_inference_scenes_async(SttodeModel* m, const float* past, const int* scene_ptr, int n, int S, const float* z,
diff --git a/profiles/d2h_ride/lane_intervals.py b/profiles/d2h_ride/lane_intervals.py
--- /dev/null
+++ b/profiles/d2h_ride/lane_intervals.py
@@ -0,0 +1,68 @@
+import csv
+import statistics
+import sys
+
+
+def col(row, *names):
+    for n in names:
+        if n in row:
+            return row[n]
+    raise KeyError(names)
+
+
+def main(path, launches=26):
+    rows = []
+    with open(path) as f:
+        for r in csv.DictReader(f):
+            name = col(r, 'Kernel_Name', 'KernelName')
+            lane = r.get('Stream_Id') or r.get('Queue_Id') or '0'
+            rows.append((int(col(r, 'Start_Timestamp', 'BeginNs')), int(col(r, 'End_Timestamp', 'EndNs')), lane, name))
+    rows.sort()
+    copies = [r for r in rows if 'host_copy_kernel' in r[3]]
+    if not copies:
+        print('no host_copy_kernel in the trace')
+        return
+    t1 = copies[-1][1]
+    chains = [r for r in rows if 'traj_chain_kernel' in r[3] and r[0] <= t1][-launches:]
+    t0 = chains[0][0]
+    in_region = [r for r in rows if t0 <= r[0] <= t1]
+    copies = [r for r in in_region if 'host_copy_kernel' in r[3]]
+    print('region: %.3f ms, %d chain launches, %d host_copy_kernel calls, %d other kernels'
+          % ((t1 - t0) / 1e6, len(chains), len(copies), len(in_region) - len(chains) - len(copies)))
+    if len(chains) > 1:
+        print('chain launches: start to start %.1f us median over the region, i.e. per step'
+              % statistics.median((b[0] - a[0]) / 1e3 for a, b in zip(chains, chains[1:])))
+    print('host_copy_kernel duration: median %.1f us' % statistics.median((c[1] - c[0]) / 1e3 for c in copies))
+    lanes = sorted({r[2] for r in chains})
+    tot = []
+    for lane in lanes:
+        seq = [r for r in in_region if r[2] == lane and ('traj_chain_kernel' in r[3] or 'host_copy_kernel' in r[3])]
+        gaps, before, after, dur = [], [], [], []
+        prev, cp = None, None
+        for r in seq:
+            if 'host_copy_kernel' in r[3]:
+                cp = r
+                continue
+            if prev is not None:
+                gaps.append((r[0] - prev[1]) / 1e3)
+                if cp is not None and cp[0] >= prev[1]:
+                    before.append((cp[0] - prev[1]) / 1e3)
+                    dur.append((cp[1] - cp[0]) / 1e3)
+                    after.append((r[0] - cp[1]) / 1e3)
+            prev, cp = r, None
+        if not gaps:
+            continue
+        tot += gaps
+        line = 'lane %s: %d intervals end of chain launch -> start of next: median %.1f us, mean %.1f us' % (lane, len(gaps), statistics.median(gaps), statistics.mean(gaps))
+        if before:
+            line += '; with a copy kernel inside (%d): chain end -> copy start %.1f, copy %.1f, copy end -> next chain start %.1f us (medians)' % (
+                len(before), statistics.median(before), statistics.median(dur), statistics.median(after))
+        print(line)
+    if tot:
+        print('all lanes: median interval %.1f us, mean %.1f us (one interval per step: three lanes in rotation)' % (statistics.median(tot), statistics.mean(tot)))
+        durs = [(c[1] - c[0]) / 1e3 for c in chains]
+        print('chain launch duration: median %.1f us, mean %.1f us' % (statistics.median(durs), statistics.mean(durs)))
+
+
+if __name__ == '__main__':
+    main(sys.argv[1], int(sys.argv[2]) if len(sys.argv) > 2 else 26)
diff --git a/sttode_amd/capi.py b/sttode_amd/capi.py
--- a/sttode_amd/capi.py
+++ b/sttode_amd/capi.py
@@ -134,6 +134,9 @@
     'sttode_clock_probe': [_P, _P],
     'sttode_copy_to_host': [_P, _P, _L, _I, _P],
     'sttode_async_enqueue': [_P, _I],
+    'sttode_async_copy_to_host': [_P, _I, _P, _P, _L, _I],
+    'sttode_wait_host_copy': [_P, _I],
+    'sttode_async_copy_stats': [_P, _P, _P, _P],
     'sttode_check': [_P, _P, _I, _I, _P],
 }
 
diff --git a/sttode_amd/csrc/api_util.hpp b/sttode_amd/csrc/api_util.hpp
--- a/sttode_amd/csrc/api_util.hpp
+++ b/sttode_amd/csrc/api_util.hpp
@@ -67,7 +67,9 @@
     const float* gt; float* ade; float* fde; float scale;
     int workers;
 };
-int stt_chain_lagged(const float* const* W, const LagRoles& r, const LagGroups& g, int K, int Tp, int Tf, int prog_len, int b3, void* stream);
+struct LagCopy { void* dst; const void* src; long bytes; int wgs; };
+int stt_chain_lagged(const float* const* W, const LagRoles& r, const LagGroups& g, const LagCopy& cp, int K, int Tp, int Tf, int prog_len, int b3,
+                     void* stream);
 bool stt_chain_lagged_covers(int Tp);
 struct SttodeSamplerPlan;
 const char* stt_sampler_plan_check(const SttodeSamplerPlan* plan, int K);
diff --git a/sttode_amd/csrc/chain32.hip b/sttode_amd/csrc/chain32.hip
--- a/sttode_amd/csrc/chain32.hip
+++ b/sttode_amd/csrc/chain32.hip
@@ -75,6 +75,8 @@
     int xcd_map;
     RoleArgs R;
     Role32Args R32;
+    int ncopy, front; long cp_n16;
+    const f32x4* cp_src; f32x4* cp_dst;
 };
 
 template <int NY> struct C32Const {
@@ -747,6 +749,14 @@
 __global__ __launch_bounds__(256, 2) void traj_chain_kernel(ChainArgs A) {
     constexpr bool kDynCount = !B3M && ((NY == 1 && FUSE == 2 && !ZS) || (NY == 2 && FUSE == 1 && ZS));
     typedef ChainStreamT<B3M ? C32_BUF_B3 : C32_CMAX * C32_TILE, B3M, kDynCount> Stream;
+    constexpr bool kCopy = FUSE == 2 && !B3M;
+    if (kCopy && (int)blockIdx.x < A.ncopy) {
+        for (long i = (long)blockIdx.x * 256 + threadIdx.x; i < A.cp_n16; i += (long)A.ncopy * 256) {
+            const f32x4 v = __builtin_nontemporal_load(A.cp_src + i);
+            __builtin_nontemporal_store(v, A.cp_dst + i);
+        }
+        return;
+    }
     extern __shared__ __attribute__((aligned(16))) char smem[];
     f32x4* ring = reinterpret_cast<f32x4*>(smem);
     f32x4* slots = ring + 2 * Stream::kBuf;
@@ -764,9 +774,9 @@
     const int ngroups = (A.ncols + 127) >> 7;
 
     C32_TRACE_BEGIN();
-    if (FUSE == 2 && (int)blockIdx.x < A.R32.nwg) {
+    if (FUSE == 2 && (int)blockIdx.x < (kCopy ? A.front : A.R32.nwg)) {
         role32_body<ZS>(*(KRole32Args*)((const __attribute__((address_space(4))) char*)__builtin_amdgcn_kernarg_segment_ptr() + offsetof(ChainArgs, R32)),
-                    blockIdx.x, smem);
+                    kCopy ? (int)blockIdx.x - A.ncopy : (int)blockIdx.x, smem);
         C32_TRACE_END(1);
         return;
     }
@@ -775,7 +785,7 @@
         C32_TRACE_END(1);
         return;
     }
-    int fb = FUSE == 0 ? (int)blockIdx.x : FUSE == 2 ? (int)blockIdx.x - A.R32.nwg : A.R.split ? (int)blockIdx.x - 5 * A.R.ntiles
+    int fb = FUSE == 0 ? (int)blockIdx.x : FUSE == 2 ? (int)blockIdx.x - (kCopy ? A.front : A.R32.nwg) : A.R.split ? (int)blockIdx.x - 5 * A.R.ntiles
                                                 : fused_block_of(blockIdx.x, A.R.ntiles, ngroups, A.K, A.R.lead);
     if (FUSE && A.xcd_map && fb >= 0) fb = xcd_group(fb, ngroups);
     if (FUSE == 1 && fb < 0) {
@@ -1069,7 +1079,8 @@
     else if (FUSE == 2) {
         int workers = ngroups;
         if (a.persistent && workers > 2 * chain_cus()) workers = 2 * chain_cus();
-        grid = a.R32.nwg + (a.ncols > 0 ? workers : 0);
+        a.front = a.ncopy + a.R32.nwg;
+        grid = a.front + (a.ncols > 0 ? workers : 0);
         a.nworkers = workers;
         if (workers < ngroups) a.xcd_map = 0;
     }
@@ -1185,7 +1196,7 @@
     a.A0x = A0x; a.A0y = A0y; a.A1y = A1y; a.pool = (const f32x4*)pool; a.prog = (const int2*)prog; a.prog_len = prog_len;
     a.consts = consts; a.z = z; a.xpad = xpad; a.ldx = ldx; a.cur = cur; a.orig = orig; a.pred = pred; a.park = pred; a.counter = counter;
     a.ncols = ncols; a.K = K; a.Tp = Tp; a.Tf2 = 2 * Tf;
-    a.dbg = nullptr; a.trace_tag = 0; a.xcd_map = 0; a.nworkers = 0; a.m_gt = nullptr; a.m_ade = a.m_fde = nullptr; a.m_scale = 1.0f;
+    a.dbg = nullptr; a.trace_tag = 0; a.xcd_map = 0; a.nworkers = 0; a.ncopy = 0; a.front = 0; a.cp_n16 = 0; a.cp_src = nullptr; a.cp_dst = nullptr; a.m_gt = nullptr; a.m_ade = a.m_fde = nullptr; a.m_scale = 1.0f;
     a.R = RoleArgs();
     a.persistent = 0;
 #if defined(C32_DIAG_STAMPS) || defined(C32_DIAG_TRACE)
@@ -1237,6 +1248,7 @@
     a.consts = W[STT_W_CHAIN_CONSTS]; a.z = z; a.xpad = ws + off[STT_B_XPAD]; a.ldx = 2 * Tp <= 16 ? 16 : 32; a.cur = ws + off[STT_B_CUR];
     a.orig = ws + off[STT_B_ORIG]; a.pred = pred; a.park = pred; a.counter = (int*)(ws + off[STT_B_QUEUE]);
     a.ncols = n * K; a.K = K; a.Tp = Tp; a.Tf2 = 2 * Tf; a.persistent = 0; a.dbg = nullptr; a.trace_tag = 0; a.xcd_map = 0; a.nworkers = 0;
+    a.ncopy = 0; a.front = 0; a.cp_n16 = 0; a.cp_src = nullptr; a.cp_dst = nullptr;
     a.m_gt = nullptr; a.m_ade = a.m_fde = nullptr; a.m_scale = 1.0f;
 #if defined(C32_DIAG_STAMPS) || defined(C32_DIAG_TRACE)
     a.dbg = g_chain_dbg;
@@ -1266,7 +1278,8 @@
 }
 
 bool stt_chain_lagged_covers(int Tp) { return Tp >= 2 && 2 * Tp <= 32; }
-int stt_chain_lagged(const float* const* W, const LagRoles& lr, const LagGroups& lg, int K, int Tp, int Tf, int prog_len, int b3, void* stream) {
+int stt_chain_lagged(const float* const* W, const LagRoles& lr, const LagGroups& lg, const LagCopy& cp, int K, int Tp, int Tf, int prog_len, int b3,
+                     void* stream) {
     float* ws_r = lr.ws; const long* off_r = lr.off; const int n_r = lr.n; const float* attn = lr.attn; const int ld_attn = lr.ld_attn;
     const float ode_time = lr.ode_time; float* zgen = lr.zgen; const unsigned long long zkey = lr.zkey; const float* past = lr.past;
     const int* scene_ptr = lr.scene_ptr; const int S = lr.S; float* r_ade = lr.ade; float* r_fde = lr.fde;
@@ -1278,6 +1291,13 @@
     a.R = RoleArgs();
     a.R32 = Role32Args();
     a.dbg = nullptr; a.trace_tag = 0; a.xcd_map = 0; a.persistent = 0; a.counter = nullptr; a.nworkers = 0;
+    a.ncopy = 0; a.front = 0; a.cp_n16 = 0; a.cp_src = nullptr; a.cp_dst = nullptr;
+    if (cp.bytes > 0) {
+        STT_REQUIRE(!b3, "stt_chain_lagged: the bf16-split launches carry no copy part");
+        STT_REQUIRE(cp.dst && cp.src && cp.bytes % 16 == 0 && ((size_t)cp.dst | (size_t)cp.src) % 16 == 0 && cp.wgs >= 1 && cp.wgs <= 256,
+                    "stt_chain_lagged: bad copy part (16-byte aligned pointers, a multiple of 16 bytes, 1 .. 256 workgroups)");
+        a.ncopy = cp.wgs; a.cp_n16 = cp.bytes / 16; a.cp_src = (const f32x4*)cp.src; a.cp_dst = (f32x4*)cp.dst;
+    }
     a.K = K; a.Tp = Tp; a.Tf2 = 2 * Tf; a.ldx = 2 * Tp <= 16 ? 16 : 32; a.ncols = 0;
     a.pool = (const f32x4*)W[b3 ? STT_W_CHAINB3_POOL : STT_W_CHAIN_POOL]; a.prog = (const int2*)W[b3 ? STT_W_CHAINB3_PROG : STT_W_CHAIN_PROG];
     a.prog_len = prog_len; a.consts = W[STT_W_CHAIN_CONSTS];
diff --git a/sttode_amd/csrc/pipeline.hip b/sttode_amd/csrc/pipeline.hip
--- a/sttode_amd/csrc/pipeline.hip
+++ b/sttode_amd/csrc/pipeline.hip
@@ -15,6 +15,8 @@
 struct LagPending { bool valid; float* ws; long off[STT_B_COUNT]; int n; const float* z; float* pred; hipStream_t s; int si;
                     const float* gt; float* ade; float* fde; float scale;
                     int one_launch; };
+
+struct CopyPending { bool valid; void* dst; const void* src; long bytes; int wgs; int si; long seq; };
 
 struct SttodeModel {
     int Tp, Tf, TPX, NOY, K;
@@ -39,6 +41,8 @@
     long lag_calls;
     LagPending lag[STT_MAX_SLOTS];
     int lag_q[4][STT_MAX_SLOTS]; int lag_qn[4];
+    CopyPending cpy[STT_MAX_SLOTS]; hipEvent_t ev_copy[STT_MAX_SLOTS]; int copy_si[STT_MAX_SLOTS]; bool slot_lagged[STT_MAX_SLOTS];
+    long copy_seq, copies_rode, copies_own_launch;
     hipStream_t sLag4;
     long acalls;
     hipEvent_t ev_call, evA_done[STT_MAX_SLOTS], evB_done[STT_MAX_SLOTS];
@@ -106,7 +110,11 @@
     m->b3 = 0;
     m->role_lead = -1;
     m->drop_tile = -1;
-    for (int p = 0; p < STT_MAX_SLOTS; ++p) { m->slot_stream[p] = nullptr; m->lag[p].valid = false; }
+    for (int p = 0; p < STT_MAX_SLOTS; ++p) {
+        m->slot_stream[p] = nullptr; m->lag[p].valid = false; m->lag[p].si = 0;
+        m->cpy[p].valid = false; m->copy_si[p] = -1; m->slot_lagged[p] = false; m->ev_copy[p] = nullptr;
+    }
+    m->copy_seq = 0; m->copies_rode = 0; m->copies_own_launch = 0;
     m->lag_streams = 3;
     m->lag_calls = 0;
     m->tmo_host = nullptr;
@@ -138,7 +146,8 @@
     if (ok) { m->tmo_host = tmo_word_take(); ok = m->tmo_host != nullptr; }
     for (int p = 0; p < STT_MAX_SLOTS && ok; ++p)
         ok = hipEventCreateWithFlags(&m->evA_done[p], hipEventDisableTiming) == hipSuccess &&
-             hipEventCreateWithFlags(&m->evB_done[p], hipEventDisableTiming) == hipSuccess;
+             hipEventCreateWithFlags(&m->evB_done[p], hipEventDisableTiming) == hipSuccess &&
+             hipEventCreateWithFlags(&m->ev_copy[p], hipEventDisableTiming) == hipSuccess;
     if (!ok) {
         tmo_word_give(m->tmo_host);
         delete m;
@@ -164,7 +173,7 @@
     for (auto e : m->pool) (void)hipEventDestroy(e);
     (void)hipEventDestroy(m->ev_fork); (void)hipEventDestroy(m->ev_join);
     (void)hipEventDestroy(m->ev_call);
-    for (int p = 0; p < STT_MAX_SLOTS; ++p) { (void)hipEventDestroy(m->evA_done[p]); (void)hipEventDestroy(m->evB_done[p]); }
+    for (int p = 0; p < STT_MAX_SLOTS; ++p) { (void)hipEventDestroy(m->evA_done[p]); (void)hipEventDestroy(m->evB_done[p]); (void)hipEventDestroy(m->ev_copy[p]); }
     tmo_word_give(m->tmo_host);
     delete m;
     if (exchanged) (void)hipThreadExchangeStreamCaptureMode(&mode);
@@ -554,6 +563,53 @@
         if (m->lag_q[si][i] != slot) m->lag_q[si][w++] = m->lag_q[si][i];
     m->lag_qn[si] = w;
 }
+static int copy_own_launch(SttodeModel* m, int slot) {
+    CopyPending& c = m->cpy[slot];
+    if (!c.valid) return 0;
+    c.valid = false;
+    hipStream_t s = lag_stream(m, c.si);
+    if (int rc = sttode_copy_to_host(c.dst, c.src, c.bytes, c.wgs, s)) return rc;
+    STT_HIP(hipEventRecord(m->ev_copy[slot], s));
+    ++m->copies_own_launch;
+    return 0;
+}
+static int copy_flush_all(SttodeModel* m) {
+    for (;;) {
+        int best = -1;
+        for (int p = 0; p < STT_MAX_SLOTS; ++p)
+            if (m->cpy[p].valid && (best < 0 || m->cpy[p].seq < m->cpy[best].seq)) best = p;
+        if (best < 0) return 0;
+        if (int rc = copy_own_launch(m, best)) return rc;
+    }
+}
+static int copy_take(SttodeModel* m, int si, LagCopy* cp, int* slot) {
+    *cp = LagCopy{nullptr, nullptr, 0, 0};
+    *slot = -1;
+    for (;;) {
+        const int keep = m->b3 ? 0 : 1;
+        int first = -1, cnt = 0;
+        for (int p = 0; p < STT_MAX_SLOTS; ++p)
+            if (m->cpy[p].valid && m->cpy[p].si == si) { ++cnt; if (first < 0 || m->cpy[p].seq < m->cpy[first].seq) first = p; }
+        if (cnt == 0) return 0;
+        if (cnt == keep) { const CopyPending& c = m->cpy[first]; *cp = LagCopy{c.dst, c.src, c.bytes, c.wgs}; *slot = first; return 0; }
+        if (int rc = copy_own_launch(m, first)) return rc;
+    }
+}
+static int copy_rode(SttodeModel* m, int slot, hipStream_t s) {
+    if (slot < 0) return 0;
+    m->cpy[slot].valid = false;
+    STT_HIP(hipEventRecord(m->ev_copy[slot], s));
+    ++m->copies_rode;
+    return 0;
+}
+static int copy_guard(SttodeModel* m, int slot, int next_si, hipStream_t writer) {
+    if (m->copy_si[slot] < 0 || m->copy_si[slot] == next_si) return 0;
+    if (int rc = copy_own_launch(m, slot)) return rc;
+    STT_HIP(hipStreamWaitEvent(writer, m->ev_copy[slot], 0));
+    m->copy_si[slot] = -1;
+    return 0;
+}
+
 static int lag_flush(SttodeModel* m, int slot) {
     LagPending& p = m->lag[slot];
     if (!p.valid) return 0;
@@ -561,14 +617,16 @@
     p.valid = false;
     LagRoles none = {};
     LagGroups lg = {p.ws, p.off, p.n, p.z, p.pred, p.gt, p.ade, p.fde, p.scale, p.one_launch};
-    RUN(STT_STAGE_FUSED, p.s, stt_chain_lagged(m->w, none, lg, m->K, m->Tp, m->Tf, m->prog_len, m->b3, p.s));
+    LagCopy cp; int cslot;
+    if (int rc = copy_take(m, p.si, &cp, &cslot)) return rc;
+    RUN(STT_STAGE_FUSED, p.s, stt_chain_lagged(m->w, none, lg, cp, m->K, m->Tp, m->Tf, m->prog_len, m->b3, p.s));
     STT_HIP(hipEventRecord(m->evB_done[slot], p.s));
-    return 0;
+    return copy_rode(m, cslot, p.s);
 }
 static int lag_flush_all(SttodeModel* m) {
     for (int p = 0; p < STT_MAX_SLOTS; ++p)
         if (int rc = lag_flush(m, p)) return rc;
-    return 0;
+    return copy_flush_all(m);
 }
 static int run_lagged(SttodeModel* m, const float* past, const int* scene_ptr, int n, int S, int G, int B, int N, const float* z, float* ws,
                       float* pred, int slot, const long* off, const SttodeAsyncOpts& o, hipStream_t s) {
@@ -578,6 +636,7 @@
     ++m->lag_calls;
     STT_HIP(hipStreamWaitEvent(sf, m->ev_call, 0));
     STT_HIP(hipStreamWaitEvent(sf, m->evB_done[slot], 0));
+    if (int rc = copy_guard(m, slot, si, sf)) return rc;
     const bool fe_role = scene_ptr != nullptr;
     const bool fe_embed = !scene_ptr && B > 1 && stt_embed_qkv_fe_covers(n, m->Tp);
     if (!fe_role && !fe_embed)
@@ -605,7 +664,10 @@
                    met ? o.ade : nullptr, met ? o.fde : nullptr};
     LagGroups lg = {};
     if (g) lg = LagGroups{g->ws, g->off, g->n, g->z, g->pred, g->gt, g->ade, g->fde, g->scale, fe_role && g->one_launch};
-    RUN(STT_STAGE_FUSED, sf, stt_chain_lagged(W, lr, lg, m->K, m->Tp, m->Tf, m->prog_len, m->b3, sf));
+    LagCopy cp; int cslot;
+    if (int rc = copy_take(m, si, &cp, &cslot)) return rc;
+    RUN(STT_STAGE_FUSED, sf, stt_chain_lagged(W, lr, lg, cp, m->K, m->Tp, m->Tf, m->prog_len, m->b3, sf));
+    if (int rc = copy_rode(m, cslot, sf)) return rc;
     if (g) {
         lag_unqueue(m, gs);
         g->valid = false;
@@ -620,6 +682,7 @@
     memcpy(p.off, off, sizeof(p.off));
     m->lag_q[si][m->lag_qn[si]++] = slot;
     m->slot_stream[slot] = sf;
+    m->slot_lagged[slot] = true;
     return 0;
 }
 
@@ -654,6 +717,8 @@
         ++m->acalls;
         STT_HIP(hipStreamWaitEvent(sf, m->ev_call, 0));
         STT_HIP(hipStreamWaitEvent(sf, m->evB_done[slot], 0));
+        if (int rc = copy_guard(m, slot, -1, sf)) return rc;
+        m->slot_lagged[slot] = false;
         const bool fe_in_role = scene_ptr != nullptr && m->fe_in_role;
         if (!fe_in_role)
             if (int rc = frontend(m, ws, off, past, scene_ptr, n, S, N, sf)) return rc;
@@ -670,6 +735,8 @@
     hipStream_t sb = (m->acalls++ & 1) ? m->sB2 : m->sB;
     STT_HIP(hipStreamWaitEvent(sb, m->ev_call, 0));
     STT_HIP(hipStreamWaitEvent(sb, m->evA_done[slot], 0));
+    if (int rc = copy_guard(m, slot, -1, sb)) return rc;
+    m->slot_lagged[slot] = false;
     if (int rc = stage_trajectories(m, ws, off, n, z, pred, sb, true)) return rc;
     STT_HIP(hipEventRecord(m->evB_done[slot], sb));
     m->slot_stream[slot] = sb;
@@ -810,6 +877,7 @@
     {
         std::lock_guard<std::mutex> lk(m->mu);
         if (int rc = lag_flush(m, slot)) return rc;
+        if (int rc = copy_flush_all(m)) return rc;
         ev = m->evB_done[slot];
     }
     STT_HIP(hipEventSynchronize(ev));
@@ -820,7 +888,46 @@
     STT_REQUIRE(m && slot >= 0 && slot < STT_MAX_SLOTS, "sttode_wait: bad arguments");
     std::lock_guard<std::mutex> lk(m->mu);
     if (int rc = lag_flush(m, slot)) return rc;
+    if (int rc = copy_flush_all(m)) return rc;
     STT_HIP(hipStreamWaitEvent((hipStream_t)stream, m->evB_done[slot], 0));
+    return 0;
+}
+
+extern "C" int sttode_async_copy_to_host(SttodeModel* m, int slot, void* dst, const void* src, long bytes, int wgs) {
+    STT_REQUIRE(m && slot >= 0 && slot < STT_MAX_SLOTS, "sttode_async_copy_to_host: bad model / slot");
+    STT_REQUIRE(dst && src && bytes > 0 && bytes % 16 == 0, "sttode_async_copy_to_host: null pointer or size not a multiple of 16 bytes");
+    STT_REQUIRE(((size_t)dst | (size_t)src) % 16 == 0, "sttode_async_copy_to_host: pointers must be 16-byte aligned");
+    std::lock_guard<std::mutex> lk(m->mu);
+    STT_REQUIRE(m->slot_stream[slot] != nullptr && m->slot_lagged[slot], "sttode_async_copy_to_host: the slot's latest call is not of the lagged form");
+    STT_REQUIRE(!m->lag[slot].valid, "sttode_async_copy_to_host: the call's trajectory groups have not been enqueued (sttode_async_enqueue)");
+    if (int rc = copy_own_launch(m, slot)) return rc;
+    if (wgs <= 0) wgs = 8;
+    if (wgs > 256) wgs = 256;
+    const int si = m->lag[slot].si;
+    m->cpy[slot] = CopyPending{true, dst, src, bytes, wgs, si, ++m->copy_seq};
+    m->copy_si[slot] = si;
+    return 0;
+}
+
+extern "C" int sttode_wait_host_copy(SttodeModel* m, int slot) {
+    STT_REQUIRE(m && slot >= 0 && slot < STT_MAX_SLOTS, "sttode_wait_host_copy: bad arguments");
+    hipEvent_t ev;
+    {
+        std::lock_guard<std::mutex> lk(m->mu);
+        if (int rc = copy_flush_all(m)) return rc;
+        ev = m->ev_copy[slot];
+    }
+    STT_HIP(hipEventSynchronize(ev));
+    return 0;
+}
+
+extern "C" int sttode_async_copy_stats(SttodeModel* m, long* rode, long* own_launch, int* pending) {
+    STT_REQUIRE(m && rode && own_launch && pending, "sttode_async_copy_stats: null pointer");
+    std::lock_guard<std::mutex> lk(m->mu);
+    *rode = m->copies_rode; *own_launch = m->copies_own_launch;
+    int n = 0;
+    for (int p = 0; p < STT_MAX_SLOTS; ++p) n += m->cpy[p].valid ? 1 : 0;
+    *pending = n;
     return 0;
 }
 
diff --git a/sttode_amd/model.py b/sttode_amd/model.py
--- a/sttode_amd/model.py
+++ b/sttode_amd/model.py
@@ -168,6 +168,7 @@
         self.ode_method, self.ode_steps = 'euler', 1
         self.mfma_mode = 'bf16x3' if os.environ.get('STTODE_BF16X3', '0') not in ('', '0') else 'f32'
         self._host_futures = {}
+        self._host_copy_refs = {}
         self.async_depth = 6
         self.device_latents = os.environ.get('STTODE_DEVICE_LATENTS', '1') != '0'
         self._async_bufs = {}
@@ -827,7 +828,7 @@
             opts.nba_groups = getattr(self, '_G', 1)
             capi.call('sttode_inference_nba_async', nat.h, self._past, self.batch_size, self._N, z, buf, pred, slot, ctypes.addressof(opts), st)
         return {'fused_metrics': fused, 'slot': slot, 'pred': pred, 'z': z, 'inputs': (self._past, getattr(self, '_scene_ptr', None)), 'metrics': mb,
-                'gt_default': self._future, 'stream': pstream}
+                'gt_default': self._future, 'stream': pstream, 'lagged': lagged}
 
     def wait(self, handle):
         if handle.get('generic'):
@@ -854,6 +855,12 @@
         nat = self.native()
         capi.call('sttode_async_enqueue', nat.h, handle['slot'])
         st = handle['stream']
+        handle['host'] = out
+        if handle.get('lagged') and st is not None and (pred.numel() * 4) % 16 == 0:
+            capi.call('sttode_async_copy_to_host', nat.h, handle['slot'], out, pred, pred.numel() * 4, int(workgroups))
+            self._host_copy_refs[handle['slot']] = (out, pred)
+            handle['host_event'] = None
+            return out
         raw = st.cuda_stream if st is not None else capi.stream_ptr()
         if st is None:
             capi.call('sttode_wait', nat.h, handle['slot'], raw)
@@ -866,13 +873,21 @@
         if ev is None:
             ev = handle['host_event'] = torch.cuda.Event()
         ev.record(st if st is not None else torch.cuda.current_stream(self.device))
-        handle['host'] = out
         return out
 
     def wait_host_copy(self, handle):
-        handle['host_event'].synchronize()
+        if handle['host_event'] is None:
+            capi.call('sttode_wait_host_copy', self.native().h, handle['slot'])
+        else:
+            handle['host_event'].synchronize()
         self.native().raise_if_timed_out()
         return handle['host'].permute(1, 0, 2, 3)
+
+    def host_copy_stats(self):
+        import ctypes
+        rode, own, pend = ctypes.c_long(0), ctypes.c_long(0), ctypes.c_int(0)
+        capi.call('sttode_async_copy_stats', self.native().h, ctypes.addressof(rode), ctypes.addressof(own), ctypes.addressof(pend))
+        return int(rode.value), int(own.value), int(pend.value)
 
     def next_async_stream(self, n):
         if self._generic:
```

New measurement: 86.78 million. No clear change (-0.1%).
